# acdha/trivy

Hardware: AMD Instinct MI355X
Metric: secret-scan GB/s (builtin rules) at 1/2/4/8 MI355X; % of HBM peak (higher is better)
Workload: dtype u8

## Files before the change

### include/trivy_secret.h

```cpp
#ifndef TRIVY_SECRET_H
#define TRIVY_SECRET_H

#include <stddef.h>
#include <stdint.h>

#ifdef __cplusplus
extern "C" {
#endif

#define TSG_OK 0
#define TSG_ERR_CONFIG -1
#define TSG_ERR_ARG -2
#define TSG_ERR_GPU -3
#define TSG_ERR_NOMEM -4
#define TSG_ERR_INTERNAL -5

typedef struct tsg_allow_rule_desc {
  const char* id;
  const char* description;
  const char* regex;
  const char* path;
} tsg_allow_rule_desc;

typedef struct tsg_rule_desc {
// ... 16 lines not shown
typedef struct tsg_result tsg_result;
typedef struct tsg_ctx tsg_ctx;

int tsg_ruleset_compile(const tsg_rule_desc* rules, uint32_t n_rules,
                        const tsg_allow_rule_desc* allow_rules, uint32_t n_allow_rules,
                        const char* const* exclude_regexes, uint32_t n_exclude_regexes,
                        tsg_ruleset** out, char* err, size_t err_len);
void tsg_ruleset_destroy(tsg_ruleset* rs);

int tsg_ruleset_allow_path(const tsg_ruleset* rs, const char* path, size_t path_len);

typedef struct tsg_ruleset_info {
  uint32_t n_rules;
  uint32_t n_keywords;
  uint32_t n_groups;
  uint32_t n_hostonly;
  uint32_t kw_states;
  uint32_t max_group_states;
  uint64_t table_bytes;
  uint32_t kw_classes;
  uint32_t k1x_literals;
} tsg_ruleset_info;
int tsg_ruleset_get_info(const tsg_ruleset* rs, tsg_ruleset_info* out);

int tsg_scan_cpu(const tsg_ruleset* rs, const char* path, size_t path_len,
                 const uint8_t* content, size_t len, tsg_result** out);

int tsg_scan_cpu_batch(const tsg_ruleset* rs, const uint8_t* data, const uint64_t* offsets,
                       uint32_t nfiles, const char* paths, const uint64_t* path_offsets,
                       int nthreads, tsg_result** out);

const uint8_t* tsg_result_data(const tsg_result* r, size_t* len);

int tsg_go_sort_perm(const uint8_t* keys, const uint64_t* key_offsets, const int64_t* secondary,
                     uint32_t n, uint32_t* perm);
void tsg_result_free(tsg_result* r);
int tsg_result_summary(const tsg_result* r, uint64_t* nfiles, uint64_t* files_with_findings,
                       uint64_t* findings);

typedef struct tsg_ctx_options {
  uint32_t chunk_bytes;
  uint32_t ext_cap;
  uint32_t cand_capacity;
  int32_t host_threads;
  uint32_t adapt_mib;
  uint32_t flags;
  uint32_t slot_mib;
  uint32_t max_slots;
} tsg_ctx_options;

#define TSG_CTX_EMULATE 1u

int tsg_ctx_create(int device, const tsg_ruleset* rs, const tsg_ctx_options* opt,
                   tsg_ctx** out);
void tsg_ctx_destroy(tsg_ctx* ctx);

typedef struct tsg_slot_view {
  uint32_t id;
  uint8_t* data;
  uint64_t data_cap;
  uint64_t* offsets;
  uint32_t files_cap;
  char* paths;
  uint64_t paths_cap;
  uint64_t* path_offsets;
} tsg_slot_view;
int tsg_slot_acquire(tsg_ctx* ctx, uint64_t data_bytes, uint32_t nfiles, uint64_t path_bytes,
                     tsg_slot_view* out);
int tsg_slot_submit(tsg_ctx* ctx, uint32_t slot_id, uint32_t nfiles, uint64_t* ticket);
int tsg_slot_release(tsg_ctx* ctx, uint32_t slot_id);

int tsg_batch_upload(tsg_ctx* ctx, const uint8_t* data, const uint64_t* offsets,
                     uint32_t nfiles, const char* paths, const uint64_t* path_offsets,
                     uint32_t* slot_id);
int tsg_batch_collect(tsg_ctx* ctx, uint64_t ticket, tsg_result** out);
int tsg_batch_pending(const tsg_ctx* ctx);
int tsg_scan_batch(tsg_ctx* ctx, const uint8_t* data, const uint64_t* offsets, uint32_t nfiles,
                   const char* paths, const uint64_t* path_offsets, tsg_result** out);
int tsg_batch_kernels(tsg_ctx* ctx, uint32_t slot_id, uint32_t nfiles, uint32_t* kw,
                      size_t kw_len, uint32_t* ev, size_t ev_len);
int tsg_batch_items(tsg_ctx* ctx, uint32_t slot_id, uint32_t* entries, size_t entries_cap,
                    uint32_t* dentries, size_t dentries_cap, uint32_t* items, size_t items_cap,
                    uint8_t* gskip, size_t gskip_len, uint64_t* n);
int tsg_batch_candidates(tsg_ctx* ctx, uint32_t slot_id, uint32_t* records, size_t records_cap,
                         uint8_t* flags, size_t flags_len, uint32_t* kw, size_t kw_len, uint64_t* n);

typedef struct tsg_adaptation_info {
  uint32_t adapted;
  uint32_t k1_filter;
  uint32_t hot_states;
  uint32_t ev_hot;
  uint64_t sample_bytes;
  uint32_t n_keywords;
  uint32_t n_groups;
  uint32_t n_literals;
  uint32_t reserved;
} tsg_adaptation_info;
int tsg_test_adaptation(tsg_ctx* ctx, tsg_adaptation_info* info, uint8_t* kw_unknown,
                        size_t kw_unknown_len, uint8_t* gate_open, size_t gate_open_len,
                        uint8_t* event_everywhere, size_t event_everywhere_len, uint32_t* hits,
                        size_t hits_len, uint8_t* quiet, size_t quiet_len);

typedef struct tsg_stats {
  double k1_ms;
  double k2_ms;
  double aux_ms;
  double resolve_ms;
  uint64_t bytes;
  uint64_t k2_bytes;
  uint64_t candidates;
  uint64_t files_resolved;
  uint32_t k2_launches;
  uint32_t overflow;
  double gate_ms;
  uint64_t k2_items;
  uint32_t k1_hot_states;
  double h2d_ms;
  uint32_t groups_skipped;
  uint64_t batches;
  uint64_t sum_bytes;
  double sum_k1_ms, sum_gate_ms, sum_k2_ms, sum_h2d_ms, sum_d2h_ms, sum_resolve_ms;
  double wait_ms;
  uint32_t k2_tail_bytes, k2_tail_max, k2_long_tails, k2_replays;
  double prep_ms, meta_ms, sum_prep_ms, sum_meta_ms;
  uint32_t k1x_records, k1x_inline;
  uint32_t k1f_listed, k1f_arrivals;
  uint32_t event_chunks;
  uint32_t k1_filter;
  double k1_clock_ms, chain_clock_ms, post_k1_clock_ms;
  double sum_k1_clock_ms, sum_chain_clock_ms, sum_post_k1_clock_ms;
  uint32_t k2_dense_entries;
  uint32_t k2_rich;
  uint32_t k1x_img_bytes;
} tsg_stats;
int tsg_ctx_get_stats(const tsg_ctx* ctx, tsg_stats* out);

int tsg_device_submit(tsg_ctx* ctx, const void* d_data, const uint64_t* offsets, uint32_t nfiles,
                      const char* paths, const uint64_t* path_offsets, uint64_t* ticket);
int tsg_scan_device(tsg_ctx* ctx, const void* d_data, const uint64_t* offsets, uint32_t nfiles,
                    const char* paths, const uint64_t* path_offsets, tsg_result** out);
typedef struct tsg_device_input_stats {
  double stage_ms;
  double fetch_ms;
  uint64_t fetched_files;
  uint64_t fetched_bytes;
  uint64_t batches, sum_bytes, sum_fetched_bytes;
  double sum_stage_ms, sum_fetch_ms;
  uint32_t whole_batch_copy;
} tsg_device_input_stats;
int tsg_ctx_get_device_input_stats(const tsg_ctx* ctx, tsg_device_input_stats* out);
int tsg_test_device_mirror(tsg_ctx* ctx, uint8_t* data, uint64_t data_cap, uint64_t* segs,
                           size_t segs_cap, uint64_t* n);

#define TSG_SPANS_BINARY_GATE 1u
int tsg_device_spans_submit(tsg_ctx* ctx, const void* d_base, uint64_t base_bytes,
                            const uint64_t* starts, const uint64_t* lengths, uint32_t nfiles,
                            const char* paths, const uint64_t* path_offsets, uint32_t flags,
                            uint8_t* kept, uint64_t* ticket);
int tsg_scan_device_spans(tsg_ctx* ctx, const void* d_base, uint64_t base_bytes,
                          const uint64_t* starts, const uint64_t* lengths, uint32_t nfiles,
                          const char* paths, const uint64_t* path_offsets, uint32_t flags,
                          uint8_t* kept, tsg_result** out);
typedef struct tsg_device_spans_stats {
  double gate_ms;
  double gather_ms;
  double wait_ms;
  uint64_t files_in, files_kept, files_dropped;
  uint64_t bytes_in, bytes_kept;
  uint64_t batches, sum_files_in, sum_files_kept, sum_files_dropped, sum_bytes_in, sum_bytes_kept;
  double sum_gate_ms, sum_gather_ms, sum_wait_ms;
} tsg_device_spans_stats;
int tsg_ctx_get_device_spans_stats(const tsg_ctx* ctx, tsg_device_spans_stats* out);

typedef struct tsg_queue tsg_queue;
int tsg_queue_create(tsg_ctx* ctx, uint32_t flush_us, tsg_queue** out);
int tsg_queue_scan(tsg_queue* q, const char* path, size_t path_len, const uint8_t* content,
                   size_t len, tsg_result** out);
int tsg_queue_flush(tsg_queue* q);
void tsg_queue_destroy(tsg_queue* q);

typedef struct tsg_multi tsg_multi;
int tsg_multi_create(const int* devices, uint32_t n, const tsg_ruleset* rs,
                     const tsg_ctx_options* opt, tsg_multi** out);
int tsg_multi_size(const tsg_multi* m);
int tsg_multi_ctx(tsg_multi* m, uint32_t i, tsg_ctx** out);
int tsg_multi_scan_batch(tsg_multi* m, const uint8_t* data, const uint64_t* offsets,
                         uint32_t nfiles, const char* paths, const uint64_t* path_offsets,
                         tsg_result** out);
int tsg_multi_get_stats(const tsg_multi* m, uint32_t i, tsg_stats* out);
void tsg_multi_destroy(tsg_multi* m);

const char* tsg_last_error(void);

int tsg_test_knob(const char* name, const char* value);

typedef struct tsg_regex tsg_regex;
int tsg_regex_compile(const char* src, tsg_regex** out, char* err, size_t err_len);
void tsg_regex_free(tsg_regex* re);
int tsg_regex_num_slots(const tsg_regex* re);
int tsg_regex_match(const tsg_regex* re, const uint8_t* text, size_t len);
int64_t tsg_regex_find_all(const tsg_regex* re, const uint8_t* text, size_t len, int submatch,
                           int64_t* out, size_t cap);
int64_t tsg_regex_find_all_engine(const tsg_regex* re, const uint8_t* text, size_t len,
                                  int submatch, int engine, int64_t* out, size_t cap);
int64_t tsg_regex_dfa_ends(const tsg_regex* re, const uint8_t* text, size_t len, uint32_t chunk,
                           int64_t* out, size_t cap);

int tsg_emulate_candidate_stats(const tsg_ruleset* rs, const uint8_t* data,
                                const uint64_t* offsets, uint32_t nfiles, uint32_t chunk,
                                uint64_t* cand_per_rule, uint64_t* gated_bytes_per_group);

int tsg_emulate_items(const tsg_ruleset* rs, const uint8_t* data, const uint64_t* offsets,
                      uint32_t nfiles, uint32_t chunk, uint32_t max_back, uint32_t* triples,
                      size_t triples_cap, uint64_t* counts, uint64_t* n_items);

int tsg_emulate_candidates(const tsg_ruleset* rs, const uint8_t* data, const uint64_t* offsets,
                           uint32_t nfiles, uint32_t chunk, uint32_t ext_cap, uint64_t items_cap,
                           uint32_t max_dense, uint32_t word_recs, uint32_t* records,
                           size_t records_cap, uint64_t* n_records);

int tsg_emulate_item_candidates(const tsg_ruleset* rs, const uint8_t* data, const uint64_t* offsets,
                                uint32_t nfiles, uint32_t chunk, uint32_t ext_cap, uint32_t* triples,
                                size_t triples_cap, uint64_t* n_triples);

int tsg_expand_candidates(const tsg_ruleset* rs, const uint8_t* data, const uint64_t* offsets,
                          uint32_t nfiles, const uint32_t* records, size_t n_records,
                          uint32_t* triples, size_t triples_cap, uint64_t* n_triples);

int tsg_layout_reference(const uint64_t* counts, uint32_t n_groups, uint64_t nchunks,
                         uint64_t items_cap, uint32_t max_dense, uint8_t* kind, uint64_t* totals);

int tsg_emulate_k1(const tsg_ruleset* rs, const uint8_t* data, const uint64_t* offsets,
                   uint32_t nfiles, uint32_t chunk, uint32_t* kw, size_t kw_len, uint32_t* ev,
                   size_t ev_len);

int tsg_emulate_k1f(const tsg_ruleset* rs, const uint8_t* data, const uint64_t* offsets,
                    uint32_t nfiles, uint32_t chunk, const uint32_t* quiet_ids, uint32_t nquiet,
                    uint32_t sample_kib, uint32_t* kw, size_t kw_len, uint32_t* ev, size_t ev_len,
                    uint64_t* stats);

int tsg_ruleset_rule_plan(const tsg_ruleset* rs, uint32_t rule, int32_t* group, int32_t* relax,
                          int64_t* max_len);

int tsg_ruleset_rule_program(const tsg_ruleset* rs, uint32_t rule, int32_t* first_atom,
                             int32_t* rule_atoms, int64_t* winback, int32_t* has_rev);

int tsg_ruleset_rule_anchor(const tsg_ruleset* rs, uint32_t rule, uint32_t* event, int64_t* evdist,
                            char* desc, size_t desc_len);

int tsg_ruleset_k1_literal(const tsg_ruleset* rs, uint32_t i, uint8_t* buf, uint32_t cap,
                           uint32_t* len, uint32_t* event);

int tsg_scan_batch_emulated(const tsg_ruleset* rs, const uint8_t* data, const uint64_t* offsets,
                            uint32_t nfiles, const char* paths, const uint64_t* path_offsets,
                            uint32_t chunk, tsg_result** out);

typedef struct tsg_layer tsg_layer;
typedef struct tsg_layer_view {
  const uint8_t* data;
  const uint64_t* offsets;
  uint32_t nfiles;
  const uint8_t* paths;
  const uint64_t* path_offsets;
  const char* opq;
  size_t opq_len;
  const char* wh;
  size_t wh_len;
  uint32_t walked;
} tsg_layer_view;
int tsg_layer_pack(const tsg_ruleset* rs, const uint8_t* tar, uint64_t tar_len,
                   const char* const* skip_files, uint32_t n_skip_files,
                   const char* const* skip_dirs, uint32_t n_skip_dirs, const char* config_path,
                   tsg_layer** out);
int tsg_layer_pack_shard(const tsg_ruleset* rs, const uint8_t* tar, uint64_t tar_len,
                         const char* const* skip_files, uint32_t n_skip_files,
                         const char* const* skip_dirs, uint32_t n_skip_dirs, const char* config_path,
                         uint32_t rank, uint32_t world, tsg_layer** out);
int tsg_layer_get(const tsg_layer* layer, tsg_layer_view* out);
typedef struct tsg_layer_range tsg_layer_range;
int tsg_layer_range_walk(const uint8_t* tar, uint64_t tar_len, uint32_t rank, uint32_t world,
                         tsg_layer_range** out, uint64_t info[4]);
int tsg_layer_range_sync(tsg_layer_range* range, uint64_t pos, uint64_t* end);
int tsg_layer_range_dirs(tsg_layer_range* range, const char* const* skip_dirs, uint32_t n_skip_dirs,
                         const char** out, uint64_t* out_len);
int tsg_layer_range_pack(const tsg_ruleset* rs, const tsg_layer_range* range,
                         const char* const* skip_files, uint32_t n_skip_files,
                         const char* const* skip_dirs, uint32_t n_skip_dirs,
                         const char* const* prior_dirs, uint32_t n_prior_dirs,
                         const char* config_path, tsg_layer** out);
void tsg_layer_range_free(tsg_layer_range* range);
int tsg_fs_pack(const tsg_ruleset* rs, const char* root, const char* const* skip_files,
                uint32_t n_skip_files, const char* const* skip_dirs, uint32_t n_skip_dirs,
                const char* config_path, tsg_layer** out);
int tsg_fs_pack_shard(const tsg_ruleset* rs, const char* root, const char* const* skip_files,
                      uint32_t n_skip_files, const char* const* skip_dirs, uint32_t n_skip_dirs,
                      const char* config_path, uint32_t rank, uint32_t world, tsg_layer** out);
int tsg_layer_pack_slot(tsg_ctx* ctx, const uint8_t* tar, uint64_t tar_len,
                        const char* const* skip_files, uint32_t n_skip_files,
                        const char* const* skip_dirs, uint32_t n_skip_dirs, const char* config_path,
                        uint32_t* slot_id, tsg_layer** out);
int tsg_layer_range_pack_slot(tsg_ctx* ctx, const tsg_layer_range* range,
                              const char* const* skip_files, uint32_t n_skip_files,
                              const char* const* skip_dirs, uint32_t n_skip_dirs,
                              const char* const* prior_dirs, uint32_t n_prior_dirs,
                              const char* config_path, uint32_t* slot_id, tsg_layer** out);
int tsg_fs_pack_slot(tsg_ctx* ctx, const char* root, const char* const* skip_files,
                     uint32_t n_skip_files, const char* const* skip_dirs, uint32_t n_skip_dirs,
                     const char* config_path, uint32_t* slot_id, tsg_layer** out);
int tsg_layer_scan(tsg_ctx* ctx, const uint8_t* tar, uint64_t tar_len,
                   const char* const* skip_files, uint32_t n_skip_files,
                   const char* const* skip_dirs, uint32_t n_skip_dirs, const char* config_path,
                   tsg_layer** layer, tsg_result** out);
int tsg_fs_scan(tsg_ctx* ctx, const char* root, const char* const* skip_files, uint32_t n_skip_files,
                const char* const* skip_dirs, uint32_t n_skip_dirs, const char* config_path,
                tsg_layer** layer, tsg_result** out);
void tsg_layer_free(tsg_layer* layer);

int tsg_device_layer_scan(tsg_ctx* ctx, const void* d_tar, uint64_t tar_len,
                          const char* const* skip_files, uint32_t n_skip_files,
                          const char* const* skip_dirs, uint32_t n_skip_dirs,
                          const char* config_path, tsg_layer** layer, tsg_result** out);
typedef struct tsg_device_layer_stats {
  double mark_ms;
  uint64_t tar_bytes;
  uint64_t blocks;
  uint64_t marked_blocks;
  uint64_t chain_entries;
  uint64_t header_bytes;
  uint64_t payloads;
  uint64_t payload_bytes;
  uint64_t payload_rounds;
// ... 18 lines not shown
```

### trivy_amd/_native.py

```python
import ctypes as C
import os

LIB_PATH = os.path.join(os.path.dirname(os.path.abspath(__file__)), "libtrivy_secret.so")
if os.environ.get("TSG_LIB_VARIANT"):
    LIB_PATH = os.path.join(os.path.dirname(os.path.abspath(__file__)),
                            "libtrivy_secret_%s.so" % os.environ["TSG_LIB_VARIANT"])

TSG_OK = 0
TSG_ERR_CONFIG = -1
TSG_ERR_ARG = -2
TSG_ERR_GPU = -3
TSG_ERR_NOMEM = -4
TSG_ERR_INTERNAL = -5


class AllowRuleDesc(C.Structure):
    _fields_ = [("id", C.c_char_p), ("description", C.c_char_p), ("regex", C.c_char_p),
                ("path", C.c_char_p)]


class RuleDesc(C.Structure):
    _fields_ = [("id", C.c_char_p), ("category", C.c_char_p), ("title", C.c_char_p),
                ("severity", C.c_char_p), ("regex", C.c_char_p),
                ("keywords", C.POINTER(C.c_char_p)), ("n_keywords", C.c_uint32),
# ... 153 lines not shown
    ("tsg_queue_destroy", None, [_P]),
    ("tsg_multi_create", C.c_int, [C.POINTER(C.c_int), C.c_uint32, _P, C.POINTER(CtxOptions),
                                   C.POINTER(_P)]),
    ("tsg_multi_size", C.c_int, [_P]),
    ("tsg_multi_ctx", C.c_int, [_P, C.c_uint32, C.POINTER(_P)]),
    ("tsg_multi_scan_batch", C.c_int, [_P, _P, _U64P, C.c_uint32, _P, _U64P, C.POINTER(_P)]),
    ("tsg_multi_get_stats", C.c_int, [_P, C.c_uint32, C.POINTER(Stats)]),
    ("tsg_multi_destroy", None, [_P]),
    ("tsg_last_error", C.c_char_p, []),
    ("tsg_test_knob", C.c_int, [C.c_char_p, C.c_char_p]),
    ("tsg_regex_compile", C.c_int, [C.c_char_p, C.POINTER(_P), C.c_char_p, C.c_size_t]),
    ("tsg_regex_free", None, [_P]),
    ("tsg_regex_num_slots", C.c_int, [_P]),
    ("tsg_regex_match", C.c_int, [_P, C.c_char_p, C.c_size_t]),
    ("tsg_regex_find_all", C.c_int64, [_P, C.c_char_p, C.c_size_t, C.c_int, _I64P, C.c_size_t]),
    ("tsg_regex_find_all_engine", C.c_int64, [_P, C.c_char_p, C.c_size_t, C.c_int, C.c_int, _I64P, C.c_size_t]),
    ("tsg_regex_dfa_ends", C.c_int64, [_P, C.c_char_p, C.c_size_t, C.c_uint32, _I64P,
                                       C.c_size_t]),
    ("tsg_scan_batch_emulated", C.c_int, [_P, _P, _U64P, C.c_uint32, _P, _U64P, C.c_uint32,
                                          C.POINTER(_P)]),
    ("tsg_emulate_candidate_stats", C.c_int, [_P, _P, _U64P, C.c_uint32, C.c_uint32, _U64P,
                                              _U64P]),
    ("tsg_emulate_items", C.c_int, [_P, _P, _U64P, C.c_uint32, C.c_uint32, C.c_uint32,
                                    C.POINTER(C.c_uint32), C.c_size_t, _U64P, _U64P]),
    ("tsg_emulate_candidates", C.c_int, [_P, _P, _U64P, C.c_uint32, C.c_uint32, C.c_uint32, C.c_uint64,
                                         C.c_uint32, C.c_uint32, C.POINTER(C.c_uint32), C.c_size_t, _U64P]),
    ("tsg_emulate_item_candidates", C.c_int, [_P, _P, _U64P, C.c_uint32, C.c_uint32, C.c_uint32,
                                              C.POINTER(C.c_uint32), C.c_size_t, _U64P]),
    ("tsg_expand_candidates", C.c_int, [_P, _P, _U64P, C.c_uint32, C.POINTER(C.c_uint32), C.c_size_t,
                                        C.POINTER(C.c_uint32), C.c_size_t, _U64P]),
    ("tsg_layout_reference", C.c_int, [_U64P, C.c_uint32, C.c_uint64, C.c_uint64, C.c_uint32,
                                       _U8P, _U64P]),
    ("tsg_ruleset_rule_plan", C.c_int, [_P, C.c_uint32, C.POINTER(C.c_int32),
                                        C.POINTER(C.c_int32), C.POINTER(C.c_int64)]),
    ("tsg_ruleset_rule_program", C.c_int, [_P, C.c_uint32, C.POINTER(C.c_int32), C.POINTER(C.c_int32),
                                           C.POINTER(C.c_int64), C.POINTER(C.c_int32)]),
    ("tsg_emulate_k1", C.c_int, [_P, _P, _U64P, C.c_uint32, C.c_uint32, C.POINTER(C.c_uint32),
                                 C.c_size_t, C.POINTER(C.c_uint32), C.c_size_t]),
    ("tsg_layer_pack", C.c_int, [_P, _P, C.c_uint64, C.POINTER(C.c_char_p), C.c_uint32,
                                 C.POINTER(C.c_char_p), C.c_uint32, C.c_char_p, C.POINTER(_P)]),
    ("tsg_layer_pack_shard", C.c_int, [_P, _P, C.c_uint64, C.POINTER(C.c_char_p), C.c_uint32,
                                       C.POINTER(C.c_char_p), C.c_uint32, C.c_char_p, C.c_uint32,
                                       C.c_uint32, C.POINTER(_P)]),
    ("tsg_layer_get", C.c_int, [_P, C.POINTER(LayerView)]),
    ("tsg_layer_range_walk", C.c_int, [_P, C.c_uint64, C.c_uint32, C.c_uint32, C.POINTER(_P),
                                       _U64P]),
    ("tsg_layer_range_sync", C.c_int, [_P, C.c_uint64, _U64P]),
    ("tsg_layer_range_dirs", C.c_int, [_P, C.POINTER(C.c_char_p), C.c_uint32,
                                       C.POINTER(C.c_void_p), _U64P]),
    ("tsg_layer_range_pack", C.c_int, [_P, _P, C.POINTER(C.c_char_p), C.c_uint32,
                                       C.POINTER(C.c_char_p), C.c_uint32, C.POINTER(C.c_char_p),
                                       C.c_uint32, C.c_char_p, C.POINTER(_P)]),
    ("tsg_layer_range_free", None, [_P]),
    ("tsg_fs_pack", C.c_int, [_P, C.c_char_p, C.POINTER(C.c_char_p), C.c_uint32,
                              C.POINTER(C.c_char_p), C.c_uint32, C.c_char_p, C.POINTER(_P)]),
    ("tsg_fs_pack_shard", C.c_int, [_P, C.c_char_p, C.POINTER(C.c_char_p), C.c_uint32,
                                    C.POINTER(C.c_char_p), C.c_uint32, C.c_char_p, C.c_uint32,
                                    C.c_uint32, C.POINTER(_P)]),
    ("tsg_layer_pack_slot", C.c_int, [_P, _P, C.c_uint64, C.POINTER(C.c_char_p), C.c_uint32,
                                      C.POINTER(C.c_char_p), C.c_uint32, C.c_char_p,
                                      C.POINTER(C.c_uint32), C.POINTER(_P)]),
    ("tsg_layer_range_pack_slot", C.c_int, [_P, _P, C.POINTER(C.c_char_p), C.c_uint32,
                                            C.POINTER(C.c_char_p), C.c_uint32,
                                            C.POINTER(C.c_char_p), C.c_uint32, C.c_char_p,
                                            C.POINTER(C.c_uint32), C.POINTER(_P)]),
    ("tsg_fs_pack_slot", C.c_int, [_P, C.c_char_p, C.POINTER(C.c_char_p), C.c_uint32,
                                   C.POINTER(C.c_char_p), C.c_uint32, C.c_char_p,
                                   C.POINTER(C.c_uint32), C.POINTER(_P)]),
    ("tsg_layer_scan", C.c_int, [_P, _P, C.c_uint64, C.POINTER(C.c_char_p), C.c_uint32,
                                 C.POINTER(C.c_char_p), C.c_uint32, C.c_char_p, C.POINTER(_P),
                                 C.POINTER(_P)]),
    ("tsg_fs_scan", C.c_int, [_P, C.c_char_p, C.POINTER(C.c_char_p), C.c_uint32,
                              C.POINTER(C.c_char_p), C.c_uint32, C.c_char_p, C.POINTER(_P),
                              C.POINTER(_P)]),
    ("tsg_layer_free", None, [_P]),
    ("tsg_go_sort_perm", C.c_int, [_P, _U64P, _I64P, C.c_uint32, C.POINTER(C.c_uint32)]),
    ("tsg_ruleset_rule_anchor", C.c_int, [_P, C.c_uint32, C.POINTER(C.c_uint32),
                                          C.POINTER(C.c_int64), C.c_char_p, C.c_size_t]),
    ("tsg_emulate_k1f", C.c_int, [_P, _P, _U64P, C.c_uint32, C.c_uint32, C.POINTER(C.c_uint32),
                                  C.c_uint32, C.c_uint32, C.POINTER(C.c_uint32), C.c_size_t,
                                  C.POINTER(C.c_uint32), C.c_size_t, C.POINTER(C.c_uint64)]),
    ("tsg_ruleset_k1_literal", C.c_int, [_P, C.c_uint32, C.c_char_p, C.c_uint32,
                                         C.POINTER(C.c_uint32), C.POINTER(C.c_uint32)]),
]

_lib = None


def lib():
    global _lib
    if _lib is None:
        if not os.path.exists(LIB_PATH):
            raise ImportError("libtrivy_secret.so is not built; run `python -m trivy_amd.build` "
                              "(expected at %s)" % LIB_PATH)
        L = C.CDLL(LIB_PATH)
        for name, res, args in SIGNATURES:
            fn = getattr(L, name)
            fn.restype = res
            fn.argtypes = args
        _lib = L
    return _lib


class NativeError(RuntimeError):
    def __init__(self, code, msg):
        super().__init__("%s (code %d)" % (msg, code))
        self.code = code


def knob(name, value=None):
    check(lib().tsg_test_knob(name.encode(), None if value is None else str(value).encode()))


def check(rc):
    if rc != TSG_OK:
        raise NativeError(rc, lib().tsg_last_error().decode("utf-8", "replace"))
    return rc
```

### trivy_amd/csrc/capi.cpp

```cpp
#include <chrono>
#include <cstdio>
#include <cstdlib>
#include <cstring>
#include <exception>
#include <thread>

#include "internal.hpp"
#include "k1f.hpp"

namespace tsg {

static thread_local std::string g_last_error;

void set_error(const std::string& msg) { g_last_error = msg; }
int fail(int code, const std::string& msg) {
  g_last_error = msg;
  return code;
}

static void copy_err(const std::string& m, char* err, size_t len) {
  if (!err || len == 0) return;
  size_t n = std::min(len - 1, m.size());
  std::memcpy(err, m.data(), n);
  err[n] = 0;
// ... 363 lines not shown
  try {
    std::vector<uint64_t> poff(nfiles + 1, 0);
    BatchView b{data, offsets, nfiles, "", poff.data()};
    std::vector<uint32_t> k, e;
    k1_reference(*rs->plan, b, chunk, &k, &e);
    if (kw) std::memcpy(kw, k.data(), sizeof(uint32_t) * std::min(kw_len, k.size()));
    if (ev) std::memcpy(ev, e.data(), sizeof(uint32_t) * std::min(ev_len, e.size()));
    return TSG_OK;
  } catch (const std::bad_alloc&) {
    return fail(TSG_ERR_NOMEM, "out of memory");
  } catch (const std::exception& ex) {
    return fail(TSG_ERR_INTERNAL, ex.what());
  }
}

int tsg_emulate_k1f(const tsg_ruleset* rs, const uint8_t* data, const uint64_t* offsets,
                    uint32_t nfiles, uint32_t chunk, const uint32_t* quiet_ids, uint32_t nquiet,
                    uint32_t sample_kib, uint32_t* kw, size_t kw_len, uint32_t* ev, size_t ev_len,
                    uint64_t* stats) {
  if (!rs || !offsets || chunk == 0 || (nquiet && !quiet_ids)) return fail(TSG_ERR_ARG, "bad argument");
  try {
    const Plan& p = *rs->plan;
    std::vector<uint8_t> quiet(p.n_lit, 0);
    for (uint32_t i = 0; i < nquiet; i++) {
      if (quiet_ids[i] >= (uint32_t)p.n_lit) return fail(TSG_ERR_ARG, "no such K1 literal");
      quiet[quiet_ids[i]] = 1;
    }
    K1FTables t;
    std::string why;
    const size_t smp = std::min<uint64_t>((uint64_t)sample_kib << 10, offsets[nfiles]);
    if (!k1f_build(p, quiet, &t, &why, smp ? data : nullptr, smp)) return fail(TSG_ERR_CONFIG, "K1F does not apply: " + why);
    std::vector<uint64_t> poff(nfiles + 1, 0);
    BatchView b{data, offsets, nfiles, "", poff.data()};
    std::vector<uint32_t> k, e;
    uint64_t st[2];
    k1f_emulate(p, t, b, chunk, &k, &e, st);
    if (kw) std::memcpy(kw, k.data(), sizeof(uint32_t) * std::min(kw_len, k.size()));
    if (ev) std::memcpy(ev, e.data(), sizeof(uint32_t) * std::min(ev_len, e.size()));
    if (stats) {
      stats[0] = st[0];
      stats[1] = st[1];
      stats[2] = t.nlit;
      stats[3] = 0;
    }
    return TSG_OK;
  } catch (const std::bad_alloc&) {
    return fail(TSG_ERR_NOMEM, "out of memory");
  } catch (const std::exception& ex) {
    return fail(TSG_ERR_INTERNAL, ex.what());
  }
}

int tsg_ruleset_rule_plan(const tsg_ruleset* rs, uint32_t rule, int32_t* group, int32_t* relax,
                          int64_t* max_len) {
  if (!rs || rule >= rs->rs.rules.size()) return fail(TSG_ERR_ARG, "bad argument");
  const Plan& p = *rs->plan;
  if (group) *group = p.rule_hostonly[rule] ? -1 : p.rule_group[rule];
  if (relax) *relax = p.rule_relax[rule];
  if (max_len) *max_len = p.rule_maxlen[rule];
  return TSG_OK;
}

int tsg_ruleset_rule_program(const tsg_ruleset* rs, uint32_t rule, int32_t* first_atom, int32_t* rule_atoms,
                             int64_t* winback, int32_t* has_rev) {
  if (!rs || rule >= rs->rs.rules.size()) return fail(TSG_ERR_ARG, "bad argument");
  const Plan& p = *rs->plan;
  if (first_atom) *first_atom = p.rule_first_atom[rule];
  if (rule_atoms) *rule_atoms = p.rule_atoms[rule];
  if (winback) *winback = p.rule_winback[rule];
  if (has_rev) *has_rev = p.rule_rev[rule] ? 1 : 0;
  return TSG_OK;
}

int tsg_ruleset_rule_anchor(const tsg_ruleset* rs, uint32_t rule, uint32_t* event, int64_t* evdist,
                            char* desc, size_t desc_len) {
  if (!rs || rule >= rs->rs.rules.size()) return fail(TSG_ERR_ARG, "bad argument");
  const Plan& p = *rs->plan;
  if (event) *event = p.rule_event[rule];
  if (evdist) *evdist = p.rule_evdist[rule];
  copy_err(p.rule_anchor[rule], desc, desc_len);
  return TSG_OK;
}

int tsg_ruleset_k1_literal(const tsg_ruleset* rs, uint32_t i, uint8_t* buf, uint32_t cap,
                           uint32_t* len, uint32_t* event) {
  if (!rs || (!buf && cap)) return fail(TSG_ERR_ARG, "bad argument");
  const Plan& p = *rs->plan;
  if (i >= p.k1_lits.size()) return fail(TSG_ERR_ARG, "no such K1 literal");
  const std::string& s = p.k1_lits[i];
  if (buf) std::memcpy(buf, s.data(), std::min<size_t>(cap, s.size()));
  if (len) *len = (uint32_t)s.size();
  if (event) *event = p.lit_event[i];
  return TSG_OK;
}

int tsg_go_sort_perm(const uint8_t* keys, const uint64_t* key_offsets, const int64_t* secondary,
                     uint32_t n, uint32_t* perm) {
  if ((n && (!keys || !key_offsets || !perm))) return fail(TSG_ERR_ARG, "bad argument");
  try {
    go_sort_perm(keys, key_offsets, secondary, n, perm);
    return TSG_OK;
  } catch (const std::bad_alloc&) {
    return fail(TSG_ERR_NOMEM, "out of memory");
  }
}

const uint8_t* tsg_result_data(const tsg_result* r, size_t* len) {
  if (!r) {
    if (len) *len = 0;
    return nullptr;
  }
  if (len) *len = r->buf.size();
  return (const uint8_t*)r->buf.data();
}

void tsg_result_free(tsg_result* r) { delete r; }

int tsg_result_summary(const tsg_result* r, uint64_t* nfiles, uint64_t* files_with_findings,
                       uint64_t* findings) {
  if (!r) return fail(TSG_ERR_ARG, "bad argument");
  try {
    std::vector<size_t> rec;
    result_record_spans(r->buf, &rec);
    uint64_t ff = 0, nf = 0;
    for (size_t i = 0; i + 1 < rec.size(); i++) {
      uint32_t k;
      std::memcpy(&k, r->buf.data() + rec[i] + 1, 4);
      ff += k > 0;
      nf += k;
    }
    if (nfiles) *nfiles = rec.size() - 1;
    if (files_with_findings) *files_with_findings = ff;
    if (findings) *findings = nf;
    return TSG_OK;
  } catch (const std::exception& ex) {
    return fail(TSG_ERR_ARG, ex.what());
  }
}

struct tsg_regex {
  std::shared_ptr<Regexp> re;
};

int tsg_regex_compile(const char* src, tsg_regex** out, char* err, size_t err_len) {
  if (!src || !out) return fail(TSG_ERR_ARG, "bad argument");
  std::string e;
  auto re = Regexp::Compile(src, &e);
  if (!re) {
    copy_err(e, err, err_len);
    return fail(TSG_ERR_CONFIG, e);
  }
  *out = new tsg_regex{re};
  return TSG_OK;
}

void tsg_regex_free(tsg_regex* re) { delete re; }

int tsg_regex_num_slots(const tsg_regex* re) { return re ? re->re->NumSlots() : TSG_ERR_ARG; }

int tsg_regex_match(const tsg_regex* re, const uint8_t* text, size_t len) {
  if (!re) return fail(TSG_ERR_ARG, "bad argument");
  return re->re->Match(text, len) ? 1 : 0;
}

int64_t tsg_regex_find_all(const tsg_regex* re, const uint8_t* text, size_t len, int submatch,
                           int64_t* out, size_t cap) {
// ... 51 lines not shown
```

### trivy_amd/csrc/device.hpp

```cpp
#pragma once
#include <hip/hip_runtime_api.h>

#include <cstdint>
#include <memory>
#include <vector>

#include "plan.hpp"

namespace tsg {

struct DeviceRules;

enum BatchEvent : int { kEvH2D = 0, kEvMeta, kEvPrep, kEvWait, kEvK1, kEvGates, kEvK2, kEvOut, kEvDone };

struct HostOut {
  uint8_t* blk = nullptr;
  uint8_t* blk_dev = nullptr;
  uint32_t* kw = nullptr;
  uint8_t* ovf = nullptr;
  uint8_t* gskip = nullptr;
  Candidate* cand = nullptr;
  Candidate* cand_dev = nullptr;
  uint32_t* counts = nullptr;
  uint32_t files_cap = 0, cand_cap = 0, groups = 0, kw_words = 0;
// ... 17 lines not shown
  kCntK1FSample = 24,
  kCntClk = 32,
  kCounts = 48,
};
enum LayoutStat : uint32_t { kLayItems = 1, kLayEntries = 2, kLaySkipped = 3 };
enum ClkStamp : uint32_t { kClkK1FStart = 0, kClkK1FEnd = 1, kClkGatesStart = 2, kClkK2End = 3, kClkStamps = 4 };
static_assert(kCntDenseEntries < kCntLayout && kCntLayout + kLayItems == kCntItems &&
                  kCntLayout + kLayEntries == kCntEntries && kCntLayout + kLaySkipped == kCntSkipped,
              "the layout's stats are slots 5..7");
static_assert(kCntSkipped < kCntK2Diag && kCntK2Diag + 4 <= kCntK2Claim && kCntK2Claim + 2 <= kCntK1X &&
                  kCntK1X + 2 <= kCntK1F && kCntK1F + 2 <= kCntK1FSample && kCntK1FSample + 2 <= kCntClk,
              "counter ranges overlap");
static_assert(kCntClk % 2 == 0 && kCntClk + 2 * kClkStamps <= kCounts, "clock stamps: 8-byte aligned, inside the block");

struct K2Diag {
  unsigned long long tail_bytes, tail_max, long_tails, replays;
};

struct GatherSeg {
  uint64_t src, dst, len;
};

enum class ScanSource {
  kHostSlot,
  kPackedHbm,
  kHbmSpans,
};

struct ScanInput {
  ScanSource kind;
  const uint64_t* off;
  uint32_t nfiles;
  uint64_t total;
  const uint8_t* data = nullptr;
  uint8_t* room = nullptr;
  uint64_t room_bytes = 0;
  const uint8_t* dev_src = nullptr;
  uint64_t src_bytes = 0;
  const GatherSeg* gather = nullptr;
  const GatherSeg* gather_dev = nullptr;
  uint32_t ngather = 0;
};

inline uint64_t slot_room_bytes(uint32_t files_cap) { return (128u << 10) + 8ull * ((uint64_t)files_cap + 1) + 64; }

struct ScanTimes {
  float h2d = 0, meta = 0, wait = 0, prep = 0, k1 = 0, gates = 0, k2 = 0, out = 0;
  float k1_clk = 0, chain_clk = 0, post_k1_clk = 0;
};

struct LaneState;

int device_rules_create(int device, const Plan& plan, uint32_t chunk, uint32_t ext_cap,
                        uint32_t adapt_mib, DeviceRules** out);
void device_rules_destroy(DeviceRules* d);
std::shared_ptr<const std::vector<uint8_t>> device_rules_kw_unknown(const DeviceRules* d);
uint32_t device_rules_hot_states(const DeviceRules* d);
struct AdaptationView {
  bool adapted = false, k1_filter = false;
  uint32_t hot_states = 0, ev_hot = 0;
  uint64_t sample_bytes = 0;
  std::vector<uint8_t> kw_unknown;
  std::vector<uint8_t> gate_open;
  std::vector<uint8_t> event_everywhere;
  std::vector<uint32_t> hits;
  std::vector<uint8_t> quiet;
};
int device_rules_adaptation(const DeviceRules* d, AdaptationView* out);
bool device_rules_k1_filter(const DeviceRules* d);
bool device_rules_k2_rich(const DeviceRules* d);
uint32_t device_rules_k1x_img_bytes(const DeviceRules* d);

int lane_create(DeviceRules* d, LaneState** out);
void lane_destroy(LaneState* l);
hipStream_t lane_stream(LaneState* l);

int host_out_alloc(const DeviceRules* d, uint32_t files_cap, uint32_t cand_cap, HostOut* out);
void host_out_free(HostOut* o);

int enqueue_scan(DeviceRules* d, LaneState* l, const ScanInput& in, HostOut* out);
int batch_times(const HostOut* out, ScanTimes* t);
int lane_kw(LaneState* l, uint32_t* kw, size_t n);
int lane_events(LaneState* l, uint32_t* ev, size_t n);
struct LaneItems {
  std::vector<uint32_t> entries, dentries, items;
  std::vector<uint8_t> gskip;
  uint64_t extent = 0;
};
int lane_items(LaneState* l, LaneItems* out);
int lane_k2_trace(LaneState* l, std::vector<unsigned long long>* out);
int lane_k1f_trace(LaneState* l, std::vector<unsigned long long>* out);

constexpr uint64_t kGatherSegBytes = 64u << 10;
struct DeviceFetch;
int fetch_create(DeviceRules* d, DeviceFetch** out);
void fetch_destroy(DeviceFetch* f);
int fetch_segments(DeviceFetch* f, const uint8_t* d_src, uint64_t total, uint8_t* host_dst,
                   const GatherSeg* segs, size_t nsegs, float* ms);
int gate_spans(DeviceFetch* f, const uint8_t* d_base, uint64_t base_bytes, const uint64_t* starts_dev,
               const uint64_t* lengths_dev, uint8_t* flags_dev, uint32_t nfiles, float* ms);
int fetch_gather(DeviceFetch* f, const uint8_t* d_base, uint64_t base_bytes, uint8_t* host_dst, uint64_t dst_bytes,
                 const GatherSeg* segs, size_t nsegs, float* ms);
int mark_tar(DeviceFetch* f, const uint8_t* d_tar, uint64_t tar_len, uint64_t* marks, float* ms);
int fetch_whole(DeviceFetch* f, const uint8_t* d_src, uint64_t total, uint8_t* host_dst, float* ms);

}
```

### trivy_amd/csrc/internal.hpp

```cpp
#pragma once
#include <algorithm>
#include <atomic>
#include <cstdint>
#include <memory>
#include <mutex>
#include <string>
#include <utility>

#include "../../include/trivy_secret.h"
#include "plan.hpp"
#include "scanner.hpp"

struct tsg_ruleset {
  tsg::Ruleset rs;
  std::unique_ptr<tsg::Plan> plan;
};

struct tsg_result {
  std::string buf;
};

namespace tsg {
void set_error(const std::string& msg);
int fail(int code, const std::string& msg);
const tsg_ruleset* ctx_ruleset(const tsg_ctx* c);
uint64_t ctx_slot_bytes(const tsg_ctx* c);
bool is_binary_head(const uint8_t* p, uint64_t n);


void tar_block_marks(const uint8_t* block, bool* header, bool* zero);
int ctx_tar_marks(tsg_ctx* c, const void* d_tar, uint64_t tar_len, uint64_t* marks, double* ms);
struct PinBuf {
  uint8_t* p = nullptr;
  uint64_t cap = 0;
};
void ctx_pin_give(tsg_ctx* c, PinBuf* b);
int ctx_fetch_ranges(tsg_ctx* c, const void* d_base, uint64_t base_bytes,
                     const std::pair<uint64_t, uint64_t>* ranges, size_t n, PinBuf* dst);
int ctx_collect_device(tsg_ctx* c, uint64_t ticket, tsg_result** out, uint64_t* fetched_bytes);
void ctx_device_layer_done(tsg_ctx* c, const tsg_device_layer_stats& last);

struct Knobs {
  std::atomic<int64_t> tar_range_kib{0}, piece_mib{0}, pike_only{0}, no_k1x{0}, emu_wordrec{0},
      x_step{0}, k1_automaton{0}, group_states{0}, group_table_kib{0}, k1f_grid{0},
      k1f_list{0}, k2_items_cap{0}, k2_max_dense{0}, k2_no_word_recs{0}, device_poison{0}, grid_cap{0};
  std::mutex m;
  std::string emu_kw_unknown;
};
Knobs& knobs();
std::string knob_kw_unknown();

inline int capped_grid(uint64_t grid, int64_t cap) {
  return (int)(cap > 0 ? std::min<uint64_t>(grid, (uint64_t)cap) : grid);
}

inline uint64_t k2_items_cap(uint64_t nchunks) {
  const int64_t k = knobs().k2_items_cap.load();
  return k > 0 ? (uint64_t)k : std::max<uint64_t>(2 * nchunks, 1u << 16);
}
inline uint32_t k2_max_dense() {
  const int64_t k = knobs().k2_max_dense.load();
  return k > 0 ? (uint32_t)k : 16u;
}
}
```

### trivy_amd/csrc/kernels.hip

```cpp
#include <hip/hip_runtime.h>

#include <algorithm>
#include <map>
#include <cstdlib>
#include <cstring>
#include <memory>
#include <vector>

#include "device.hpp"
#include "internal.hpp"
#include "k1f.hpp"

namespace tsg {

#define HIP_TRY(x)                                                                    \
  do {                                                                                \
    hipError_t e_ = (x);                                                              \
    if (e_ != hipSuccess)                                                             \
      return fail(TSG_ERR_GPU, std::string(#x) + ": " + hipGetErrorString(e_));       \
  } while (0)

constexpr int kStreams = 4;
constexpr int kK1Chains = 2;
constexpr int kK1Unroll = 8;
// ... 1301 lines not shown
  if (threadIdx.x == 0) {
    const uint32_t n = *s_n, kept = min(n, slice);
    A.count[blockIdx.x] = kept;
    atomicAdd(&A.stats[0], kept);
    if (n > kept) atomicAdd(&A.stats[1], n - kept);
  }
}

static const void* k1x_fn(uint32_t step) {
  if (step == 4) return (const void*)k1x_kernel<4>;
  if (step == 2) return (const void*)k1x_kernel<2>;
  return (const void*)k1x_kernel<1>;
}

constexpr int kXVerifyBlock = 1024;
template <bool LDS>
__global__ void __launch_bounds__(kXVerifyBlock) k1x_verify_kernel(DevK1X x, K1XArgs A, uint32_t nblocks) {
  extern __shared__ __attribute__((aligned(16))) uint8_t x_img[];
  const uint32_t b = blockIdx.x;
  const uint32_t n = A.count[b];
  if (n == 0) return;
  DevK1X y = x;
  if constexpr (LDS) {
    stage16(x_img, x.img, x.img_bytes / 16 * 16);
    __syncthreads();
    auto rebase = [&](auto* p) { return (decltype(p))(x_img + ((const uint8_t*)p - x.img)); };
    y.slots = rebase(x.slots);
    y.lits = rebase(x.lits);
    y.off = rebase(x.off);
    y.len = rebase(x.len);
    y.kwid = rebase(x.kwid);
    y.ev = rebase(x.ev);
    y.bytes = rebase(x.bytes);
  }
  const uint32_t slice = A.cap / nblocks;
  for (uint32_t j = threadIdx.x; j < n; j += blockDim.x) {
    const uint2 r = A.list[(size_t)b * slice + j];
    const uint64_t p0 = (uint64_t)r.x * 16;
    for (uint32_t t = r.y; t; t &= t - 1) {
      const uint64_t p = p0 + __builtin_ctz(t);
      const uint32_t w = x_low_byte(A.data[p]) | x_low_byte(A.data[p + 1]) << 8 | x_low_byte(A.data[p + 2]) << 16 |
                         x_low_byte(A.data[p + 3]) << 24;
      k1x_verify_at(y, A, p, w);
    }
  }
}

__device__ __forceinline__ bool group_gated(const uint32_t* __restrict__ kwf, const uint32_t* __restrict__ gm,
                                            uint32_t W, uint32_t always) {
  if (always) return true;
  for (uint32_t w = 0; w < W; w++)
    if (kwf[w] & gm[w]) return true;
  return false;
}

__device__ __forceinline__ void ggate_file(uint32_t f, const uint32_t* __restrict__ kw, uint32_t F, uint32_t W,
                                           const unsigned long long* __restrict__ kwg,
                                           const unsigned long long* __restrict__ galw, uint32_t GW,
                                           unsigned long long* __restrict__ ggate) {
  if (f >= F) return;
  const uint32_t* kwf = kw + (size_t)f * W;
  for (uint32_t w0 = 0; w0 < GW; w0 += 8) {
    const uint32_t n = min(8u, GW - w0);
    unsigned long long acc[8];
#pragma unroll
    for (uint32_t j = 0; j < 8; j++) acc[j] = j < n ? galw[w0 + j] : 0ull;
    for (uint32_t i = 0; i < W; i++)
      for (uint32_t bits = kwf[i]; bits; bits &= bits - 1) {
        const unsigned long long* row = kwg + (size_t)(i * 32 + __builtin_ctz(bits)) * GW + w0;
#pragma unroll
        for (uint32_t j = 0; j < 8; j++)
          if (j < n) acc[j] |= row[j];
      }
#pragma unroll
    for (uint32_t j = 0; j < 8; j++)
      if (j < n) ggate[(size_t)f * GW + w0 + j] = acc[j];
  }
}

struct ItemArgs {
  const uint64_t* off;
  const uint32_t* cf;
  const uint32_t* ev;
  const uint32_t* evlist;
  const uint32_t* nev;
  uint32_t evcap;
  const unsigned long long* ggate;
  const unsigned long long* gofbit;
  const uint32_t* gevents;
  const uint32_t* gback;
  uint64_t nchunks;
  uint32_t F, G, GW, chunk, maxback;
  uint32_t* count;
  uint32_t* bcount;
  uint32_t* cursor;
  uint2* items;
  const uint32_t* kw;
  uint32_t W;
  const unsigned long long* kwg;
  const unsigned long long* galw;
  unsigned long long* clk;
  uint32_t kwg_lds;
};

constexpr uint32_t kEvPer = 32;
__device__ __forceinline__ void ev_compact_block(const uint32_t* __restrict__ ev, uint64_t nchunks,
                                                 uint32_t* __restrict__ list, uint32_t* __restrict__ count,
                                                 uint32_t bid, uint32_t nblocks) {
  __shared__ uint32_t s_wave[kBlock / 64];
  __shared__ uint32_t s_base;
  const uint32_t lane = threadIdx.x & 63, wave = threadIdx.x >> 6;
  constexpr uint64_t kPer = (uint64_t)kEvPer * kBlock;
  for (uint64_t c0 = (uint64_t)bid * kPer; c0 < nchunks; c0 += (uint64_t)nblocks * kPer) {
    const uint64_t c = c0 + (uint64_t)threadIdx.x * kEvPer;
    uint32_t has = 0;
    if (c + kEvPer <= nchunks) {
      uint4 v[kEvPer / 4];
#pragma unroll
      for (uint32_t i = 0; i < kEvPer / 4; i++) v[i] = *(const uint4*)(ev + c + 4 * i);
#pragma unroll
      for (uint32_t i = 0; i < kEvPer / 4; i++)
        has |= ((v[i].x & ~kEvAlways) != 0 ? 1u : 0u) << (4 * i) | ((v[i].y & ~kEvAlways) != 0 ? 2u : 0u) << (4 * i) |
               ((v[i].z & ~kEvAlways) != 0 ? 4u : 0u) << (4 * i) | ((v[i].w & ~kEvAlways) != 0 ? 8u : 0u) << (4 * i);
    } else {
      for (uint32_t i = 0; i < kEvPer && c + i < nchunks; i++) has |= ((ev[c + i] & ~kEvAlways) != 0 ? 1u : 0u) << i;
    }
    const uint32_t n = __popc(has);
    uint32_t inc = n;
#pragma unroll
    for (int o = 1; o < 64; o <<= 1) {
      const uint32_t t = __shfl_up(inc, o);
      if (lane >= (uint32_t)o) inc += t;
    }
    if (lane == 63) s_wave[wave] = inc;
    __syncthreads();
    if (threadIdx.x == 0) {
      uint32_t tot = 0;
      for (uint32_t w = 0; w < kBlock / 64; w++) tot += s_wave[w];
      s_base = tot ? atomicAdd(count, tot) : 0;
    }
    __syncthreads();
    uint32_t at = s_base + inc - n;
    for (uint32_t w = 0; w < wave; w++) at += s_wave[w];
    for (uint32_t t = has; t; t &= t - 1) list[at++] = (uint32_t)(c + __builtin_ctz(t));
    __syncthreads();
  }
}

struct GateArgs {
  const uint32_t* ev;
  uint64_t nchunks;
  uint32_t* evlist;
  uint32_t* nev;
  uint32_t ev_blocks;
  const uint32_t* kw;
  uint32_t F, W, GW;
  const unsigned long long* kwg;
  const unsigned long long* galw;
  unsigned long long* ggate;
  unsigned long long* clk;
  uint32_t kwg_lds;
};
constexpr uint32_t kKwgLdsMax = 48 * 1024;
__global__ void __launch_bounds__(kBlock) gates_kernel(GateArgs A) {
  extern __shared__ __attribute__((aligned(16))) uint8_t smem[];
  if (threadIdx.x == 0 && blockIdx.x < kStampBlocks)
    atomicMax(&A.clk[kClkGatesStart], ~(unsigned long long)wall_clock64());
  if (blockIdx.x < A.ev_blocks) {
    ev_compact_block(A.ev, A.nchunks, A.evlist, A.nev, blockIdx.x, A.ev_blocks);
  } else {
    const unsigned long long* kwg = A.kwg;
    if (A.kwg_lds) {
      stage16(smem, A.kwg, A.kwg_lds);
      __syncthreads();
      kwg = (const unsigned long long*)smem;
    }
    ggate_file((blockIdx.x - A.ev_blocks) * blockDim.x + threadIdx.x, A.kw, A.F, A.W, kwg, A.galw, A.GW, A.ggate);
  }
}

static inline size_t item_lds_host(uint32_t G, uint32_t GW) { return 256 * (size_t)GW + 8 * (size_t)G; }
constexpr uint32_t kItemKwgLdsMax = 16 * 1024;
struct ItemLds {
  const unsigned long long* gofbit;
  const uint32_t* gback;
  const uint32_t* gevents;
  const unsigned long long* kwg;
};
__device__ __forceinline__ uint32_t item_lds_bytes(const ItemArgs& A) { return 256 * A.GW + 8 * A.G + A.kwg_lds; }
__device__ __forceinline__ ItemLds item_lds_load(const ItemArgs& A, uint8_t* smem) {
  unsigned long long* gofbit = (unsigned long long*)smem;
  uint32_t* gback = (uint32_t*)(gofbit + 32 * A.GW);
  uint32_t* gevents = gback + A.G;
  for (uint32_t i = threadIdx.x; i < 32 * A.GW; i += blockDim.x) gofbit[i] = A.gofbit[i];
  for (uint32_t i = threadIdx.x; i < A.G; i += blockDim.x) {
    gback[i] = A.gback[i];
    gevents[i] = A.gevents[i];
  }
  const unsigned long long* kwg = A.kwg;
  if (A.kwg_lds) {
    unsigned long long* k = (unsigned long long*)(gevents + A.G);
    for (uint32_t i = threadIdx.x; i < A.kwg_lds / 8; i += blockDim.x) k[i] = A.kwg[i];
    kwg = k;
  }
  return ItemLds{gofbit, gback, gevents, kwg};
}

__device__ __forceinline__ unsigned long long file_gate(const ItemArgs& A, const ItemLds& T, uint32_t f, uint32_t w) {
  if (A.ggate) return A.ggate[(size_t)f * A.GW + w];
  const uint32_t* kwf = A.kw + (size_t)f * A.W;
  unsigned long long acc = A.galw[w];
  for (uint32_t i = 0; i < A.W; i++)
    for (uint32_t bits = kwf[i]; bits; bits &= bits - 1) acc |= T.kwg[(size_t)(i * 32 + __builtin_ctz(bits)) * A.GW + w];
  return acc;
}

template <class V>
__device__ __forceinline__ void gen_items(const ItemArgs& A, const ItemLds& T, uint64_t t, V visit) {
  const uint32_t ev_t = t < A.evcap ? A.evlist[t] : 0u;
  const uint32_t nev = min(*A.nev, A.evcap);
  const uint32_t C = A.chunk;
  if (t < nev) {
    const uint64_t e = ev_t;
    const uint32_t evb = A.ev[e] & ~kEvAlways;
    const uint64_t ce = (e + 1) * C;
    uint32_t pw[kMaxBack];
    if (e >= (uint64_t)kMaxBack) {
      const uint64_t b0 = (e - kMaxBack) & ~3ull;
      const uint32_t sh = (uint32_t)(e - kMaxBack - b0);
      uint32_t x[20];
#pragma unroll
      for (int j = 0; j < 5; j++) {
        const uint4 q = *(const uint4*)(A.ev + b0 + 4 * j);
        x[4 * j] = q.x;
        x[4 * j + 1] = q.y;
        x[4 * j + 2] = q.z;
        x[4 * j + 3] = q.w;
      }
#pragma unroll
      for (int i = 0; i < kMaxBack; i++) {
        const int k = kMaxBack - 1 - i;
        pw[i] = sh == 0 ? x[k] : sh == 1 ? x[k + 1] : sh == 2 ? x[k + 2] : x[k + 3];
      }
    } else {
#pragma unroll
      for (int i = 0; i < kMaxBack; i++) pw[i] = e > (uint64_t)i ? A.ev[e - 1 - i] : 0u;
    }
    for (uint32_t f = file_of(A.cf, A.off, A.F, e * C); f < A.F && A.off[f] < ce; f++) {
      const uint64_t fs = A.off[f], fe = A.off[f + 1];
      if (fe == fs) continue;
      const uint64_t fc0 = fs / C;
      for (uint32_t w = 0; w < A.GW; w++) {
        unsigned long long cand = 0;
        for (uint32_t bits = evb; bits; bits &= bits - 1) cand |= T.gofbit[__builtin_ctz(bits) * A.GW + w];
        cand &= file_gate(A, T, f, w) & ~T.gofbit[31 * A.GW + w];
        while (cand) {
          const uint32_t g = w * 64 + __builtin_ctzll(cand);
          cand &= cand - 1;
          const uint32_t back = T.gback[g], gev = T.gevents[g];
          const uint64_t lo0 = e > fc0 + back ? e - back : fc0;
          const uint32_t lim = (uint32_t)(e - lo0);
          uint32_t m = 0;
#pragma unroll
          for (int i = 0; i < kMaxBack; i++) m |= ((pw[i] & gev) != 0 && (uint32_t)i < lim ? 1u : 0u) << i;
          visit(f, g, m ? e - __builtin_ctz(m) : lo0, e);
        }
      }
    }
  } else if (t < (uint64_t)nev + A.F) {
    const uint32_t f = (uint32_t)(t - nev);
    const uint64_t fs = A.off[f], fe = A.off[f + 1];
    if (fe == fs) return;
    for (uint32_t w = 0; w < A.GW; w++) {
      unsigned long long cand = file_gate(A, T, f, w) & T.gofbit[31 * A.GW + w];
      while (cand) {
        const uint32_t g = w * 64 + __builtin_ctzll(cand);
        cand &= cand - 1;
        visit(f, g, fs / C, (fe - 1) / C);
      }
    }
  }
}

__global__ void __launch_bounds__(kBlock) items_count_kernel(ItemArgs A) {
  extern __shared__ __attribute__((aligned(16))) uint8_t smem[];
  if (!A.ggate && threadIdx.x == 0 && blockIdx.x < kStampBlocks)
    atomicMax(&A.clk[kClkGatesStart], ~(unsigned long long)wall_clock64());
  const ItemLds T = item_lds_load(A, smem);
  uint32_t* s_count = (uint32_t*)(smem + item_lds_bytes(A));
  for (uint32_t g = threadIdx.x; g < A.G; g += blockDim.x) s_count[g] = 0;
  __syncthreads();
  const uint64_t nt = (uint64_t)min(*A.nev, A.evcap) + A.F, stride = (uint64_t)gridDim.x * blockDim.x;
  for (uint64_t t = (uint64_t)blockIdx.x * blockDim.x + threadIdx.x; t < nt; t += stride)
    gen_items(A, T, t, [&](uint32_t, uint32_t g, uint64_t lo, uint64_t hi) { atomicAdd(&s_count[g], (uint32_t)(hi - lo + 1)); });
  __syncthreads();
  for (uint32_t g = threadIdx.x; g < A.G; g += blockDim.x)
    A.bcount[(size_t)blockIdx.x * A.G + g] = s_count[g] ? atomicAdd(&A.count[g], s_count[g]) : 0u;
}

struct LayoutArgs {
  const uint32_t* gcount;
  uint32_t G;
  uint64_t nchunks, items_cap;
  uint32_t max_dense;
  uint4* entries;
  uint32_t* nentries;
  uint4* dentries;
  uint32_t* ndentries;
  uint8_t* gskip;
  uint32_t* stats;
};

constexpr int kK2Block = 256;
constexpr uint32_t kEntryItems = 2 * kK2Block;
constexpr uint32_t kEntryChunks = kStreams * kBlock;
static_assert(kEntryItems == kK2EntryItems && kEntryChunks == kK2EntryChunks, "layout_reference restates these");

template <int N>
__device__ void block_exclusive_scan_n(const unsigned long long (&v)[N], unsigned long long (&out)[N],
                                       unsigned long long (&tot)[N], unsigned long long* s_wave) {
  const uint32_t lane = threadIdx.x & 63, wave = threadIdx.x >> 6, nw = blockDim.x >> 6;
  unsigned long long x[N];
#pragma unroll
  for (int k = 0; k < N; k++) x[k] = v[k];
  for (int o = 1; o < 64; o <<= 1) {
#pragma unroll
    for (int k = 0; k < N; k++) {
      const unsigned long long y = __shfl_up(x[k], o);
      if (lane >= (uint32_t)o) x[k] += y;
    }
  }
  if (lane == 63)
#pragma unroll
    for (int k = 0; k < N; k++) s_wave[k * nw + wave] = x[k];
  __syncthreads();
#pragma unroll
  for (int k = 0; k < N; k++) {
    unsigned long long before = 0, total = 0;
    for (uint32_t w = 0; w < nw; w++) {
      const unsigned long long t = s_wave[k * nw + w];
      before += w < wave ? t : 0;
      total += t;
    }
    out[k] = before + x[k] - v[k];
    tot[k] = total;
  }
  __syncthreads();
// ... 947 lines not shown
  v.ns = (uint32_t)d.nstates;
  v.nmasks = (uint32_t)d.masks.size();
  v.mw = mw;
  v.kw_words = W;
  v.warm = (uint32_t)p.warm;
  v.kU = (uint32_t)p.run_k[0];
  v.kD = v.packed ? (uint32_t)p.run_k[1] : (uint32_t)p.run_k[1] << 8;
  std::vector<uint16_t> kwlen((size_t)W * 32, 0);
  v.kw_maxlen = 1;
  for (int k = 0; k < p.n_kw; k++) {
    kwlen[k] = p.kw_len[k];
    v.kw_maxlen = std::max<uint32_t>(v.kw_maxlen, p.kw_len[k]);
  }
  if ((rc = upload_vec(kwlen, &v.kw_len, allocs))) return rc;
  host->masks = masks;
  const int lc = k1_lds_class(host->tab.size() * 2);
  v.lds_class = (uint32_t)(lc >> 1);
  v.rep = (uint32_t)(lc & 1);
  if (!v.packed && v.lds_class > 2) return fail(TSG_ERR_INTERNAL, "keyword automaton exceeds LDS");
  return TSG_OK;
}

template <class T>
struct DevBuf {
  T* p = nullptr;
  size_t cap = 0;
  DevBuf() = default;
  DevBuf(const DevBuf&) = delete;
  DevBuf& operator=(const DevBuf&) = delete;
  ~DevBuf() { (void)hipFree(p); }
  operator T*() const { return p; }
  int ensure(size_t n, bool exact = false) {
    if (cap >= n && p) return TSG_OK;
    if (p) HIP_TRY(hipFree(p));
    p = nullptr;
    cap = 0;
    const size_t alloc = exact ? n : std::max<size_t>(n + n / 8, 16);
    HIP_TRY(hipMalloc((void**)&p, exact ? alloc * sizeof(T) : (alloc * sizeof(T) + 15) & ~(size_t)15));
    cap = alloc;
    return TSG_OK;
  }
};

struct DeviceRules {
  uint32_t all_kw_rows = 0;
  int device = 0;
  const Plan* plan = nullptr;
  uint32_t chunk = 256, ext_cap = 1u << 16, adapt_mib = 0;
  int grid = 0;
  int cus = 0;
  int k2_grid = 0, k2_dense_grid = 0;
  bool k2_rich = false;
  hipEvent_t kernels_done = nullptr;
  bool kernels_done_valid = false;
  std::vector<void*> tables;
  DevK1 k1{};
  K1Host k1h;
  DevK1X k1x{};
  bool has_k1x = false;
  bool use_k1f = false;
  uint32_t k1f_maxlen = 4;
  DevK1F k1f{};
  K1FTables k1ft;
  DevBuf<uint32_t> d_fhits;
  DevBuf<uint32_t> d_hits;
  bool adapted = false;
  uint32_t hot_states = 0;
  uint32_t ev_hot = 0;
  uint64_t sample_bytes = 0;
  std::vector<uint32_t> lit_hits;
  std::vector<uint8_t> lit_quiet;
  std::shared_ptr<const std::vector<uint8_t>> kw_unknown;
  std::vector<uint32_t> h_galways, h_gevents;
  std::vector<unsigned long long> h_gofbit;
  std::vector<DevDFA> groups;
  DevDFA* d_groups = nullptr;
  uint32_t* d_gmask = nullptr;
  uint32_t* d_galways = nullptr;
  unsigned long long* d_kwg = nullptr;
  unsigned long long* d_galw = nullptr;
  uint32_t* d_gevents = nullptr;
  uint32_t* d_gback = nullptr;
  unsigned long long* d_gofbit = nullptr;
  std::vector<uint32_t> gback;
  uint32_t GW = 1, maxback = 0, max_lds = 0;
  ~DeviceRules() {
    (void)hipSetDevice(device);
    if (kernels_done) (void)hipEventDestroy(kernels_done);
    for (auto* p : tables) (void)hipFree(p);
  }
};

struct LaneState {
  DeviceRules* d = nullptr;
  hipStream_t st = nullptr;
  DevBuf<uint8_t> data_alloc;
  DevBuf<uint8_t> meta;
  const uint64_t* off = nullptr;
  DevBuf<uint32_t> cf;
  DevBuf<uint32_t> ev_bits;
  DevBuf<uint2> xlist;
  DevBuf<uint32_t> xcount;
  DevBuf<uint32_t> evlist;
  DevBuf<uint32_t> zclaim;
  DevBuf<unsigned long long> wtrace;
  size_t wtrace_n = 0;
  DevBuf<uint32_t> kw;
  DevBuf<unsigned long long> ggate;
  DevBuf<uint8_t> ovf;
  DevBuf<uint8_t> hascand;
  DevBuf<uint2> items;
  DevBuf<uint4> entries;
  DevBuf<uint4> dentries;
  DevBuf<DevCand> cand;
  DevBuf<uint32_t> counts;
  DevBuf<uint32_t> gcount;
  DevBuf<uint32_t> bcount;
  DevBuf<uint32_t> cursor;
  DevBuf<uint8_t> gskip;
  DevBuf<unsigned long long> etrace;
  uint64_t nchunks = 0;
  uint8_t* data() const { return data_alloc.p + kPad; }
  ~LaneState() {
    if (!d) return;
    (void)hipSetDevice(d->device);
    if (st) (void)hipStreamSynchronize(st);
    if (st) (void)hipStreamDestroy(st);
  }
};

template <bool PACKED, int LDSK, bool REP, int TPB>
static const void* k1_fn_w(uint32_t kw_words) {
  if (kw_words <= 1) return (const void*)k1_kernel<1, PACKED, LDSK, REP, TPB>;
  if (kw_words <= 2) return (const void*)k1_kernel<2, PACKED, LDSK, REP, TPB>;
  if (kw_words <= 4) return (const void*)k1_kernel<4, PACKED, LDSK, REP, TPB>;
  return (const void*)k1_kernel<8, PACKED, LDSK, REP, TPB>;
}

static const void* k1_fn(const DevK1& k, int* threads, int* per_cu) {
  if (k.packed) {
    *threads = 1024;
    *per_cu = 1;
    return k1_fn_w<true, kK1PLdsK, true, 1024>(k.kw_words);
  }
  const uint32_t lc = std::min<uint32_t>(k.lds_class, 2);
  *threads = k1_threads(kK1Lds[lc]);
  *per_cu = kK1BlocksPerCU[lc];
  switch (lc) {
    case 0: return k1_fn_w<false, kK1Lds[0], true, k1_threads(kK1Lds[0])>(k.kw_words);
    case 1: return k1_fn_w<false, kK1Lds[1], true, k1_threads(kK1Lds[1])>(k.kw_words);
    default:
      return k.rep ? k1_fn_w<false, kK1Lds[2], true, k1_threads(kK1Lds[2])>(k.kw_words)
                   : k1_fn_w<false, kK1Lds[2], false, k1_threads(kK1Lds[2])>(k.kw_words);
  }
}

static int launch_k1(DeviceRules* r, const K1Args& A, int64_t grid_cap, hipStream_t st) {
  int threads = 0, per_cu = 0;
  const void* fn = k1_fn(r->k1, &threads, &per_cu);
  const uint64_t cap = (uint64_t)r->cus * per_cu;
  const int grid = capped_grid(std::min<uint64_t>((A.nitems + threads - 1) / threads, cap), grid_cap);
  DevK1 d = r->k1;
  K1Args a = A;
  void* args[] = {&d, &a};
  HIP_TRY(hipLaunchKernel(fn, dim3(grid), dim3(threads), args, 0, st));
  HIP_TRY(hipGetLastError());
  return TSG_OK;
}

template <class Exact>
static std::vector<uint32_t> hottest_over_budget(const std::vector<uint32_t>& hits, uint64_t sample_bytes, Exact exact) {
  uint64_t tot = 0;
  std::vector<uint32_t> order, drop;
  for (uint32_t i = 0; i < hits.size(); i++)
    if (hits[i]) {
      tot += hits[i];
      order.push_back(i);
    }
  std::sort(order.begin(), order.end(), [&](uint32_t a, uint32_t b) { return hits[a] > hits[b]; });
  const uint64_t budget = sample_bytes / 4096;
  for (uint32_t i : order) {
    if (tot <= budget) break;
    if (exact(i)) continue;
// ... 176 lines not shown
}

int device_rules_create(int device, const Plan& p, uint32_t chunk, uint32_t ext_cap, uint32_t adapt_mib,
                        DeviceRules** out) {
  int ndev = 0;
  HIP_TRY(hipGetDeviceCount(&ndev));
  if (device < 0 || device >= ndev) return fail(TSG_ERR_GPU, "no such HIP device");
  HIP_TRY(hipSetDevice(device));
  auto r = std::make_unique<DeviceRules>();
  r->device = device;
  r->plan = &p;
  r->chunk = chunk;
  r->ext_cap = ext_cap;
  r->adapt_mib = adapt_mib;
  if (p.warm > kPad) return fail(TSG_ERR_CONFIG, "a keyword is longer than the K1 warm-up window");
  int rc;
  if ((rc = make_device_k1(p, &r->k1, &r->tables, &r->k1h))) return rc;
  if ((rc = make_device_k1x(p, &r->k1x, &r->tables))) return rc;
  r->has_k1x = !p.x_lits.empty();
  if (!knobs().k1_automaton.load() && k1f_build(p, {}, &r->k1ft, nullptr)) {
    void* ent = nullptr;
    void* img = nullptr;
    HIP_TRY(hipMalloc(&ent, 256 * 16));
    r->tables.push_back(ent);
    HIP_TRY(hipMalloc(&img, kFImgMax));
    r->tables.push_back(img);
    r->k1f.ent = (const uint4*)ent;
    r->k1f.img = (const uint8_t*)img;
    r->k1f.kw_words = (uint32_t)p.kw_words;
    if ((rc = upload_k1f(r.get()))) return rc;
    if ((rc = r->d_fhits.ensure(std::max(1, p.n_lit), true))) return rc;
    r->use_k1f = true;
  }
  for (uint8_t h : p.rule_hostonly) r->all_kw_rows |= h;
  if (r->has_k1x)
    HIP_TRY(hipFuncSetAttribute(k1x_fn(r->k1x.step), hipFuncAttributeMaxDynamicSharedMemorySize,
                                kXDwords * 4 + 16));
  if (r->has_k1x && r->k1x.img_bytes <= kXImgLds)
    HIP_TRY(hipFuncSetAttribute((const void*)k1x_verify_kernel<true>, hipFuncAttributeMaxDynamicSharedMemorySize,
                                r->k1x.img_bytes));
  if ((rc = r->d_hits.ensure(r->k1.ns, true))) return rc;
  const uint32_t G = (uint32_t)p.groups.size();
  if (G > 0x7FFF) return fail(TSG_ERR_INTERNAL, "more K2 groups than transition records can name");
  r->GW = std::max<uint32_t>(1, (G + 63) / 64);
  std::vector<uint32_t> gmask, galways, gevents;
  std::vector<unsigned long long> gofbit(32 * r->GW, 0);
  for (uint32_t g = 0; g < G; g++) {
    const auto& gp = p.groups[g];
    DevDFA dd{};
    if ((rc = make_device_dfa(*gp.dfa, gp.rules, &dd, &r->tables))) return rc;
    r->max_lds = std::max(r->max_lds, dd.lds_bytes);
    r->groups.push_back(dd);
    gmask.insert(gmask.end(), gp.kwmask.begin(), gp.kwmask.end());
    galways.push_back(gp.always ? 1 : 0);
    gevents.push_back(gp.events);
    uint32_t back = group_back(gp, chunk);
    if (back > (uint32_t)kMaxBack) back = kMaxBack + 1;
    r->gback.push_back(back);
    if (back <= (uint32_t)kMaxBack) r->maxback = std::max(r->maxback, back);
    for (int b = 0; b < 32; b++)
      if (((gp.events >> b) & 1) || back > (uint32_t)kMaxBack) gofbit[b * r->GW + g / 64] |= 1ull << (g % 64);
  }
  r->max_lds = std::max<uint32_t>(r->max_lds, 16);
  {
    const size_t emit_lds = item_lds_host(G, r->GW) + kItemKwgLdsMax + 13 * (size_t)G + 16;
    if (emit_lds > 160 * 1024) return fail(TSG_ERR_INTERNAL, "too many rule groups for the item passes");
    if (emit_lds > 64 * 1024) {
      HIP_TRY(hipFuncSetAttribute((const void*)items_emit_kernel, hipFuncAttributeMaxDynamicSharedMemorySize, (int)emit_lds));
      HIP_TRY(hipFuncSetAttribute((const void*)items_count_kernel, hipFuncAttributeMaxDynamicSharedMemorySize, (int)emit_lds));
    }
  }
  if (r->max_lds > 64 * 1024) {
    HIP_TRY(hipFuncSetAttribute((const void*)k2_kernel, hipFuncAttributeMaxDynamicSharedMemorySize, (int)r->max_lds));
    HIP_TRY(hipFuncSetAttribute((const void*)k2_kernel_rich, hipFuncAttributeMaxDynamicSharedMemorySize, (int)r->max_lds));
    HIP_TRY(hipFuncSetAttribute((const void*)k2_dense_kernel, hipFuncAttributeMaxDynamicSharedMemorySize,
                                (int)r->max_lds));
  }
  if ((rc = upload_vec(gmask, &r->d_gmask, &r->tables))) return rc;
  if ((rc = upload_vec(galways, &r->d_galways, &r->tables))) return rc;
  if ((rc = upload_vec(gevents, &r->d_gevents, &r->tables))) return rc;
  if ((rc = upload_vec(r->gback, &r->d_gback, &r->tables))) return rc;
  if ((rc = upload_vec(gofbit, &r->d_gofbit, &r->tables))) return rc;
  {
    const uint32_t nkw = (uint32_t)p.kw_words * 32;
    std::vector<unsigned long long> kwg((size_t)nkw * r->GW, 0), galw(r->GW, 0);
    for (uint32_t g = 0; g < G; g++) {
      for (uint32_t k = 0; k < nkw; k++)
        if ((gmask[(size_t)g * p.kw_words + k / 32] >> (k % 32)) & 1) kwg[(size_t)k * r->GW + g / 64] |= 1ull << (g % 64);
      if (galways[g]) galw[g / 64] |= 1ull << (g % 64);
    }
    if ((rc = upload_vec(kwg, &r->d_kwg, &r->tables))) return rc;
    if ((rc = upload_vec(galw, &r->d_galw, &r->tables))) return rc;
  }
  r->h_galways = galways;
  r->h_gevents = gevents;
  r->h_gofbit = gofbit;
  if ((rc = upload_vec(r->groups, &r->d_groups, &r->tables))) return rc;
  hipDeviceProp_t prop;
  HIP_TRY(hipGetDeviceProperties(&prop, device));
  r->cus = prop.multiProcessorCount;
  r->grid = prop.multiProcessorCount * 8;
  HIP_TRY(hipEventCreateWithFlags(&r->kernels_done, hipEventDisableTiming | hipEventReleaseToDevice));
  int occ = 0;
  HIP_TRY(hipOccupancyMaxActiveBlocksPerMultiprocessor(&occ, (const void*)k2_kernel, kK2Block, r->max_lds));
  r->k2_grid = r->cus * std::max(occ, 1);
  {
    int occ_rich = 0;
    HIP_TRY(hipOccupancyMaxActiveBlocksPerMultiprocessor(&occ_rich, (const void*)k2_kernel_rich, kK2Block, r->max_lds));
    r->k2_rich = occ_rich >= 1 && occ_rich >= occ;
  }
  HIP_TRY(hipOccupancyMaxActiveBlocksPerMultiprocessor(&occ, (const void*)k2_dense_kernel, kBlock, r->max_lds));
  r->k2_dense_grid = r->cus * std::max(occ, 1);
  *out = r.release();
  return TSG_OK;
}

void device_rules_destroy(DeviceRules* d) { delete d; }

std::shared_ptr<const std::vector<uint8_t>> device_rules_kw_unknown(const DeviceRules* d) { return d->kw_unknown; }
uint32_t device_rules_hot_states(const DeviceRules* d) { return d->hot_states; }
int device_rules_adaptation(const DeviceRules* d, AdaptationView* out) {
  const Plan& p = *d->plan;
  out->adapted = d->adapted;
  out->k1_filter = d->use_k1f;
  out->hot_states = d->hot_states;
  out->ev_hot = d->ev_hot;
  out->sample_bytes = d->sample_bytes;
  if (d->kw_unknown) out->kw_unknown = *d->kw_unknown;
  else out->kw_unknown.assign(p.n_kw, 0);
  const size_t G = d->groups.size();
  std::vector<uint32_t> ga(G), ge(G);
  if (G) {
    HIP_TRY(hipSetDevice(d->device));
    HIP_TRY(hipMemcpy(ga.data(), d->d_galways, sizeof(uint32_t) * G, hipMemcpyDeviceToHost));
    HIP_TRY(hipMemcpy(ge.data(), d->d_gevents, sizeof(uint32_t) * G, hipMemcpyDeviceToHost));
  }
  out->gate_open.assign(G, 0);
  out->event_everywhere.assign(G, 0);
  for (size_t g = 0; g < G; g++) {
    out->gate_open[g] = ga[g] ? 1 : 0;
    out->event_everywhere[g] = (ge[g] & kEvAlways) ? 1 : 0;
  }
  out->hits = d->lit_hits;
  out->quiet = d->lit_quiet;
  return TSG_OK;
}
bool device_rules_k1_filter(const DeviceRules* d) { return d->use_k1f; }
bool device_rules_k2_rich(const DeviceRules* d) { return d->k2_rich; }
uint32_t device_rules_k1x_img_bytes(const DeviceRules* d) { return d->has_k1x ? d->k1x.img_bytes : 0u; }

int lane_create(DeviceRules* d, LaneState** out) {
  HIP_TRY(hipSetDevice(d->device));
  auto l = std::make_unique<LaneState>();
  l->d = d;
  HIP_TRY(hipStreamCreateWithFlags(&l->st, hipStreamNonBlocking));
  const uint32_t G = std::max<uint32_t>(1, (uint32_t)d->groups.size());
  int rc;
  if ((rc = l->counts.ensure(kCounts, true))) return rc;
  if ((rc = l->gcount.ensure(G, true))) return rc;
  if ((rc = l->bcount.ensure(G * (size_t)d->grid, true))) return rc;
  if ((rc = l->cursor.ensure(G, true))) return rc;
  if ((rc = l->gskip.ensure(G, true))) return rc;
  *out = l.release();
  return TSG_OK;
}

void lane_destroy(LaneState* l) { delete l; }
hipStream_t lane_stream(LaneState* l) { return l->st; }

static size_t al256(size_t x) { return (x + 255) & ~(size_t)255; }

void host_out_free(HostOut* o) {
  void* ps[] = {o->blk, o->cand};
  for (void* p : ps)
    if (p) (void)hipHostFree(p);
  for (auto& e : o->ev)
    if (e) (void)hipEventDestroy(e);
  *o = HostOut{};
}

int host_out_alloc(const DeviceRules* d, uint32_t files_cap, uint32_t cand_cap, HostOut* o) {
  HIP_TRY(hipSetDevice(d->device));
  HostOut h;
  h.files_cap = std::max<uint32_t>(files_cap, 1);
  h.cand_cap = std::max<uint32_t>(cand_cap, 1);
  h.groups = std::max<uint32_t>(1, (uint32_t)d->groups.size());
  h.kw_words = (uint32_t)d->plan->kw_words;
  const size_t o_gskip = 256, o_ovf = o_gskip + al256(h.groups), o_kw = o_ovf + al256(h.files_cap),
               bytes = o_kw + al256(sizeof(uint32_t) * (size_t)h.files_cap * h.kw_words);
  auto fail_free = [&](hipError_t e, const char* what) {
    host_out_free(&h);
    return fail(TSG_ERR_GPU, std::string(what) + ": " + hipGetErrorString(e));
  };
  hipError_t e;
  if ((e = hipHostMalloc((void**)&h.blk, bytes, hipHostMallocMapped)) != hipSuccess) return fail_free(e, "hipHostMalloc");
  if ((e = hipHostGetDevicePointer((void**)&h.blk_dev, h.blk, 0)) != hipSuccess) return fail_free(e, "hipHostGetDevicePointer");
  h.counts = (uint32_t*)h.blk;
  {
    int khz = 0;
    if (hipDeviceGetAttribute(&khz, hipDeviceAttributeWallClockRate, d->device) == hipSuccess && khz > 0)
      h.wall_khz = (uint32_t)khz;
  }
  h.gskip = h.blk + o_gskip;
  h.ovf = h.blk + o_ovf;
  h.kw = (uint32_t*)(h.blk + o_kw);
  if ((e = hipHostMalloc((void**)&h.cand, sizeof(Candidate) * (size_t)h.cand_cap, hipHostMallocMapped)) != hipSuccess)
    return fail_free(e, "hipHostMalloc");
  if ((e = hipHostGetDevicePointer((void**)&h.cand_dev, h.cand, 0)) != hipSuccess) return fail_free(e, "hipHostGetDevicePointer");
  for (int k = 0; k <= kEvDone; k++)
    if ((e = k < kEvDone ? hipEventCreateWithFlags(&h.ev[k], hipEventDisableSystemFence) : hipEventCreate(&h.ev[k])) !=
        hipSuccess)
      return fail_free(e, "hipEventCreate");
  *o = h;
  return TSG_OK;
}

struct BatchShape {
  uint32_t W, C, F, G;
  uint64_t total, nchunks, nchunks_pad, ncf;
  size_t tail, o_off, meta_bytes;
  bool one_copy;
  bool k1f;
  uint64_t k1_items;
  uint32_t k1f_tiles;
  uint64_t items_cap;
  uint32_t max_dense;
  uint64_t entries_cap, dentries_cap, zclaim_words;
  bool work;
  uint32_t kwg_bytes;
  int64_t grid_cap;
};

static int batch_shape(const DeviceRules* r, const ScanInput& in, const HostOut* out, BatchShape* s) {
  const uint32_t C = s->C = r->chunk;
  const uint64_t total = s->total = in.total;
  s->W = (uint32_t)r->plan->kw_words;
  s->F = in.nfiles;
  s->G = (uint32_t)r->groups.size();
  if (s->F > out->files_cap) return fail(TSG_ERR_ARG, "batch has more files than its output buffers");
  if (total / C >= (1ull << 32) - 2) return fail(TSG_ERR_ARG, "batch too large for u32 chunk ids");
  const bool spans = in.kind == ScanSource::kHbmSpans;
  for (uint32_t k = 0; spans && k < in.ngather; k++) {
    const GatherSeg& g = in.gather[k];
    if (g.src > in.src_bytes || g.len > in.src_bytes - g.src || g.dst > total || g.len > total - g.dst)
      return fail(TSG_ERR_INTERNAL, "gather segment outside its buffers");
  }
  if (spans && in.ngather && (!in.dev_src || !in.gather_dev)) return fail(TSG_ERR_INTERNAL, "gather without a source");
  s->nchunks = (total + C - 1) / C;
  s->k1f = r->use_k1f && total + (1u << 16) < (1ull << 32);
  s->tail = std::max<size_t>((size_t)kK1Chains * kK1Seg * C + kPad, 8192);
  s->meta_bytes = sizeof(uint64_t) * ((size_t)s->F + 1);
  s->o_off = ((size_t)total + s->tail + 15) & ~(size_t)15;
  s->one_copy = in.kind == ScanSource::kHostSlot && in.room == in.data && in.room_bytes >= s->o_off + s->meta_bytes;
  const uint64_t k1_item_chunks = (uint64_t)kK1Chains * kK1Seg;
  s->k1_items = (s->nchunks + k1_item_chunks - 1) / k1_item_chunks;
  s->nchunks_pad = s->k1_items * k1_item_chunks + 1;
  s->ncf = (total >> kCfShift) + 2;
  s->k1f_tiles = (uint32_t)((total + kFTile - 1) / kFTile);
  s->zclaim_words = s->nchunks_pad / 32 + 2;
  s->items_cap = k2_items_cap(s->nchunks);
  s->max_dense = k2_max_dense();
  s->entries_cap = s->items_cap / kEntryItems + s->G + 1;
  s->dentries_cap = (uint64_t)s->max_dense * ((s->nchunks + kEntryChunks - 1) / kEntryChunks + 1);
  s->work = s->F && s->G && s->nchunks;
  s->kwg_bytes = (uint32_t)(32ull * s->W * r->GW * 8);
  s->grid_cap = knobs().grid_cap.load();
  return TSG_OK;
}

int enqueue_scan(DeviceRules* r, LaneState* l, const ScanInput& in, HostOut* out) {
  const Plan& p = *r->plan;
  HIP_TRY(hipSetDevice(r->device));
  hipStream_t st = l->st;
  BatchShape s;
  int rc;
  if ((rc = batch_shape(r, in, out, &s))) return rc;
  const uint64_t total = s.total;
  l->nchunks = s.nchunks;
  if ((rc = l->data_alloc.ensure(kPad + s.o_off + s.meta_bytes))) return rc;
  uint8_t* data = l->data();
  if (s.one_copy) {
    l->off = (const uint64_t*)(data + s.o_off);
  } else {
    if ((rc = l->meta.ensure(s.meta_bytes))) return rc;
    l->off = (const uint64_t*)l->meta.p;
  }
  if ((rc = l->cf.ensure((size_t)s.ncf))) return rc;
  if ((rc = l->ev_bits.ensure((size_t)s.nchunks_pad + 4))) return rc;
  if (r->has_k1x && (rc = l->xlist.ensure((size_t)(total / 256 + 65536)))) return rc;
  if (r->has_k1x && (rc = l->xcount.ensure((size_t)std::max(r->cus, 1)))) return rc;
  if ((rc = l->evlist.ensure((size_t)s.nchunks_pad))) return rc;
  if (s.k1f && (rc = l->zclaim.ensure((size_t)s.zclaim_words))) return rc;
  if ((rc = l->kw.ensure((size_t)s.F * s.W + 1))) return rc;
  if ((rc = l->ggate.ensure((size_t)s.F * r->GW + 1))) return rc;
  if ((rc = l->ovf.ensure((size_t)s.F + 1))) return rc;
  if ((rc = l->hascand.ensure((size_t)s.F + 1))) return rc;
  if ((rc = l->items.ensure((size_t)s.items_cap))) return rc;
  if ((rc = l->entries.ensure((size_t)s.entries_cap))) return rc;
  if ((rc = l->dentries.ensure((size_t)s.dentries_cap))) return rc;
  if ((rc = l->cand.ensure(out->cand_cap, true))) return rc;
  HIP_TRY(hipEventRecord(out->ev[kEvH2D], st));
  if (s.one_copy) {
    std::memset(in.room + total, 0, s.o_off - total);
    std::memcpy(in.room + s.o_off, in.off, s.meta_bytes);
    HIP_TRY(hipMemcpyAsync(data, in.room, s.o_off + s.meta_bytes, hipMemcpyHostToDevice, st));
    HIP_TRY(hipEventRecord(out->ev[kEvMeta], st));
  } else {
    switch (in.kind) {
      case ScanSource::kHbmSpans:
        if (in.ngather) {
          GatherArgs GA{in.dev_src, in.src_bytes, data, total, in.gather_dev, in.ngather};
          const int ggrid = capped_grid(std::min<uint64_t>(in.ngather, (uint64_t)std::max(r->grid, 1)), s.grid_cap);
          gather_kernel<true><<<ggrid, 256, 0, st>>>(GA);
          HIP_TRY(hipGetLastError());
        }
        break;
      case ScanSource::kPackedHbm:
        if (total) {
          const uint64_t words = (total + 15) / 16;
          const int sgrid =
              capped_grid(std::max<uint64_t>(1, std::min<uint64_t>((words + 255) / 256, (uint64_t)r->grid)), s.grid_cap);
          stage_kernel<<<sgrid, 256, 0, st>>>(data, in.dev_src, total);
          HIP_TRY(hipGetLastError());
        }
        break;
      case ScanSource::kHostSlot:
        if (total) HIP_TRY(hipMemcpyAsync(data, in.data, total, hipMemcpyHostToDevice, st));
        break;
    }
    HIP_TRY(hipEventRecord(out->ev[kEvMeta], st));
    HIP_TRY(hipMemcpyAsync(l->meta, in.off, s.meta_bytes, hipMemcpyHostToDevice, st));
  }
  HIP_TRY(hipEventRecord(out->ev[kEvPrep], st));
  {
    PrepArgs PA{};
    PA.off = l->off;
    PA.nfiles = s.F;
    PA.ncf = s.F ? s.ncf : 0;
    PA.cf = l->cf;
    bool too_many = false;
    auto zero = [&](void* ptr, uint64_t n) {
      if (!n) return;
      if (PA.nz == (uint32_t)kPrepZeros) {
        too_many = true;
        return;
      }
      PA.zp[PA.nz] = (uint8_t*)ptr;
      PA.zn[PA.nz++] = n;
    };
    zero(l->data_alloc, kPad);
    if (!s.one_copy) zero(data + total, s.tail);
    zero(l->kw, sizeof(uint32_t) * (uint64_t)s.F * s.W);
    zero(l->ovf, s.F);
    zero(l->hascand, s.F);
    zero(l->counts, sizeof(uint32_t) * kCounts);
    if (s.k1f) zero(l->ev_bits, sizeof(uint32_t) * s.nchunks_pad);
    if (s.k1f) zero(l->zclaim, sizeof(uint32_t) * s.zclaim_words);
    zero(l->gcount, sizeof(uint32_t) * s.G);
    zero(l->cursor, sizeof(uint32_t) * s.G);
    zero(l->gskip, s.G);
    if (too_many) return fail(TSG_ERR_INTERNAL, "more zero fills than the prep kernel takes");
    const uint64_t work = std::max<uint64_t>(
        {PA.ncf, (uint64_t)s.F * s.W / 4, s.one_copy ? 1 : s.tail / 16, s.k1f ? s.nchunks_pad / 4 : 1, 1});
    const int pgrid = capped_grid(std::min<uint64_t>((work + 255) / 256, (uint64_t)r->grid), s.grid_cap);
    prep_kernel<<<pgrid, 256, 0, st>>>(PA);
    HIP_TRY(hipGetLastError());
  }
  HIP_TRY(hipEventRecord(out->ev[kEvWait], st));
  if (r->kernels_done_valid) HIP_TRY(hipStreamWaitEvent(st, r->kernels_done, 0));
  HIP_TRY(hipEventRecord(out->ev[kEvK1], st));

  const uint64_t adapt_bytes = r->adapt_mib == 0xFFFFFFFFu ? ~0ull : (uint64_t)(r->adapt_mib ? r->adapt_mib : 16) << 20;
  const bool k1f_list = s.k1f && total && !r->has_k1x && knobs().k1f_list.load() && k1f_lists(r, s.k1f_tiles, s.C, s.grid_cap);
  if (s.k1f) {
    K1FArgs A{data, l->off, l->cf, (uint32_t)total, s.C, s.F, s.k1f_tiles, s.F ? (uint32_t)s.ncf : 0u,
              l->kw, l->ev_bits, nullptr, l->counts + kCntK1F, (unsigned long long*)(l->counts + kCntClk),
              nullptr, nullptr, r->k1f_maxlen, 0, nullptr, nullptr};
    if (!r->adapted && total >= adapt_bytes &&
        (rc = adapt_k1f(r, l, A, in.data, sizeof(uint32_t) * (uint64_t)s.F * s.W, sizeof(uint32_t) * s.nchunks_pad,
                        s.grid_cap)))
      return rc;
    if (k1f_list) {
      A.evlist = l->evlist;
      A.nev = l->counts + kCntEvChunks;
      A.evcap = (uint32_t)std::min<size_t>(l->evlist.cap, 0xFFFFFFFFu);
      A.zone = r->k1f_maxlen;
      A.claim = l->zclaim;
    }
    static const bool wtrace = getenv("TSG_K1F_TRACE") != nullptr;
    if (wtrace && total) {
      const size_t nw = (size_t)k1f_grid(r, s.k1f_tiles, s.grid_cap) * (kFThreads / 64);
      if ((rc = l->wtrace.ensure(4 * nw))) return rc;
      HIP_TRY(hipMemsetAsync(l->wtrace, 0, sizeof(unsigned long long) * 4 * nw, st));
      A.wtrace = l->wtrace;
      l->wtrace_n = 4 * nw;
    }
    if (total && (rc = launch_k1f(r, A, s.grid_cap, st))) return rc;
  } else if (!r->adapted && s.k1_items >= 64 && total >= adapt_bytes) {
    if ((rc = adapt_k1(r, l, total, s.F, s.nchunks, s.k1_items, s.grid_cap))) return rc;
  }
  if (!s.k1f && s.k1_items) {
    K1Args A{data, l->off, l->cf, total, s.nchunks, s.k1_items, 1, s.C, s.F, l->kw, l->ev_bits, nullptr, (uint32_t)kK1Seg};
    if ((rc = launch_k1(r, A, s.grid_cap, st))) return rc;
  }
  if (r->has_k1x && total) {
    const int xg = capped_grid(
        std::max<uint64_t>(1, std::min<uint64_t>((total / 16 + kK1XBlock - 1) / kK1XBlock, (uint64_t)r->cus)), s.grid_cap);
    K1XArgs X{data, l->off, l->cf, total, s.C, s.F, l->kw, l->ev_bits, l->xlist, l->xcount,
              (uint32_t)std::min<size_t>(l->xlist.cap, 0xFFFFFFFFu), l->counts + kCntK1X};
    void* xa[] = {(void*)&r->k1x, (void*)&X};
    HIP_TRY(hipLaunchKernel(k1x_fn(r->k1x.step), dim3(xg), dim3(kK1XBlock), xa, kXDwords * 4 + 16, st));
    if (r->k1x.img_bytes <= kXImgLds)
      k1x_verify_kernel<true><<<xg, kXVerifyBlock, r->k1x.img_bytes, st>>>(r->k1x, X, (uint32_t)xg);
    else
      k1x_verify_kernel<false><<<xg, kXVerifyBlock, 0, st>>>(r->k1x, X, (uint32_t)xg);
    HIP_TRY(hipGetLastError());
  }
  HIP_TRY(hipEventRecord(out->ev[kEvGates], st));

  ItemArgs IA{};
  IA.off = l->off;
  IA.cf = l->cf;
  IA.ev = l->ev_bits;
  IA.ggate = l->ggate;
  IA.gofbit = r->d_gofbit;
  IA.gevents = r->d_gevents;
  IA.gback = r->d_gback;
  IA.nchunks = s.nchunks;
  IA.F = s.F;
  IA.G = s.G;
  IA.GW = r->GW;
  IA.chunk = s.C;
  IA.maxback = r->maxback;
  IA.count = l->gcount;
  IA.bcount = l->bcount;
  IA.cursor = l->cursor;
  IA.evlist = l->evlist;
  IA.nev = l->counts + kCntEvChunks;
  IA.evcap = (uint32_t)std::min<size_t>(l->evlist.cap, 0xFFFFFFFFu);
  IA.items = l->items;
  IA.kw = l->kw;
  IA.W = s.W;
  IA.kwg = r->d_kwg;
  IA.galw = r->d_galw;
  IA.clk = (unsigned long long*)(l->counts + kCntClk);
  if (s.work && k1f_list) {
    IA.ggate = nullptr;
  } else if (s.work) {
    const uint32_t cgrid = (uint32_t)capped_grid(
        std::min<uint64_t>((s.nchunks + kEvPer * kBlock - 1) / (kEvPer * kBlock), (uint64_t)r->grid), s.grid_cap);
    GateArgs GA{l->ev_bits, s.nchunks, l->evlist, l->counts + kCntEvChunks, cgrid, l->kw, s.F, s.W, r->GW, r->d_kwg, r->d_galw, l->ggate,
                (unsigned long long*)(l->counts + kCntClk), s.kwg_bytes <= kKwgLdsMax ? s.kwg_bytes : 0u};
    gates_kernel<<<cgrid + (s.F + kBlock - 1) / kBlock, kBlock, GA.kwg_lds, st>>>(GA);
    HIP_TRY(hipGetLastError());
  }
  if (s.work) {
    const int igrid = capped_grid((uint64_t)std::min(r->grid, r->cus * kItemsBpc), s.grid_cap);
    IA.kwg_lds = !IA.ggate && s.kwg_bytes <= kItemKwgLdsMax ? s.kwg_bytes : 0u;
    const size_t ilds = item_lds_host(s.G, r->GW) + IA.kwg_lds;
    hipLaunchKernelGGL(items_count_kernel, dim3(igrid), dim3(kBlock), ilds + s.G * sizeof(uint32_t) + 16, st, IA);
    HIP_TRY(hipGetLastError());
    LayoutArgs LA{l->gcount, s.G, s.nchunks, s.items_cap, s.max_dense, l->entries, l->counts + kCntListEntries,
                  l->dentries, l->counts + kCntDenseEntries, l->gskip, l->counts + kCntLayout};
    hipLaunchKernelGGL(items_emit_kernel, dim3(igrid), dim3(kBlock), ilds + 3 * s.G * sizeof(uint32_t) + s.G + 16, st, IA, LA);
    HIP_TRY(hipGetLastError());
  }
  HIP_TRY(hipEventRecord(out->ev[kEvK2], st));

  if (s.work) {
    K2Args A{};
    A.data = data;
    A.off = l->off;
    A.cf = l->cf;
    A.total = total;
    A.nchunks = s.nchunks;
    A.chunk = s.C;
    A.ext_cap = r->ext_cap;
    A.nfiles = s.F;
    A.kw = l->kw;
    A.kw_words = s.W;
    A.gmask = r->d_gmask;
    A.galways = r->d_galways;
    A.items = l->items;
    A.entries = l->entries;
    A.nentries = l->counts + kCntListEntries;
    A.dentries = l->dentries;
    A.ndentries = l->counts + kCntDenseEntries;
    A.cand = l->cand;
    A.cand_count = l->counts + kCntCand;
    A.cand_cap = out->cand_cap;
    A.ovf = l->ovf;
    A.hascand = l->hascand;
    static const bool diag = getenv("TSG_K2_DIAG") != nullptr;
    A.diag = diag ? l->counts + kCntK2Diag : nullptr;
    A.claim = l->counts + kCntK2Claim;
    A.word_recs = s.G <= 0x3FFF && !knobs().k2_no_word_recs.load();
    static const bool trace = getenv("TSG_K2_TRACE") != nullptr;
    if (trace && (rc = l->etrace.ensure((size_t)s.entries_cap * kTraceW))) return rc;
    if (trace) HIP_TRY(hipMemsetAsync(l->etrace, 0, sizeof(unsigned long long) * s.entries_cap * kTraceW, st));
    A.etrace = trace ? l->etrace.p : nullptr;
    A.clk = (unsigned long long*)(l->counts + kCntClk);
    const int k2g = capped_grid((uint64_t)r->k2_grid, s.grid_cap), k2dg = capped_grid((uint64_t)r->k2_dense_grid, s.grid_cap);
    if (r->k2_rich)
      hipLaunchKernelGGL(k2_kernel_rich, dim3(k2g), dim3(kK2Block), r->max_lds, st, (const DevDFA*)r->d_groups, A);
    else
      hipLaunchKernelGGL(k2_kernel, dim3(k2g), dim3(kK2Block), r->max_lds, st, (const DevDFA*)r->d_groups, A);
    HIP_TRY(hipGetLastError());
    hipLaunchKernelGGL(k2_dense_kernel, dim3(k2dg), dim3(kBlock), r->max_lds, st,
                       (const DevDFA*)r->d_groups, A);
    HIP_TRY(hipGetLastError());
  }
  HIP_TRY(hipEventRecord(out->ev[kEvOut], st));
  HIP_TRY(hipEventRecord(r->kernels_done, st));
  r->kernels_done_valid = true;

  {
    OutArgs OA{};
    OA.count = l->counts;
    OA.cand_cap = out->cand_cap;
    OA.cand = (const uint8_t*)l->cand.p;
    OA.cand_host = (uint8_t*)out->cand_dev;
    auto copy = [&](void* host, const void* dev, uint64_t n) {
      if (n) {
        OA.dst[OA.nc] = out->blk_dev + ((uint8_t*)host - out->blk);
        OA.src[OA.nc] = (const uint8_t*)dev;
        OA.n[OA.nc++] = n;
      }
    };
    copy(out->counts, l->counts, sizeof(uint32_t) * kCounts);
    copy(out->gskip, l->gskip, s.G);
    OA.kw = l->kw;
    OA.kw_host = (uint32_t*)(out->blk_dev + ((uint8_t*)out->kw - out->blk));
    OA.ovf = l->ovf;
    OA.hascand = l->hascand;
    OA.flags_host = out->blk_dev + (out->ovf - out->blk);
    OA.F = s.F;
    OA.W = s.W;
    OA.fb_lo = (uint32_t)p.fb_kw0;
    OA.fb_hi = (uint32_t)p.n_kw;
    OA.all_rows = r->all_kw_rows;
    outputs_kernel<<<capped_grid(128, s.grid_cap), 256, 0, st>>>(OA);
    HIP_TRY(hipGetLastError());
  }
  HIP_TRY(hipEventRecord(out->ev[kEvDone], st));
  return TSG_OK;
}

int batch_times(const HostOut* o, ScanTimes* t) {
  auto between = [&](BatchEvent a, BatchEvent b, float* ms) { return hipEventElapsedTime(ms, o->ev[a], o->ev[b]); };
  HIP_TRY(between(kEvH2D, kEvMeta, &t->h2d));
  HIP_TRY(between(kEvMeta, kEvPrep, &t->meta));
  HIP_TRY(between(kEvPrep, kEvWait, &t->prep));
  HIP_TRY(between(kEvWait, kEvK1, &t->wait));
  HIP_TRY(between(kEvK1, kEvGates, &t->k1));
  HIP_TRY(between(kEvGates, kEvK2, &t->gates));
  HIP_TRY(between(kEvK2, kEvOut, &t->k2));
  HIP_TRY(between(kEvOut, kEvDone, &t->out));
  const unsigned long long* c = (const unsigned long long*)(o->counts + kCntClk);
  const double per_ms = o->wall_khz ? (double)o->wall_khz : 100000.0;
  const unsigned long long k1s = ~c[kClkK1FStart], k1e = c[kClkK1FEnd], gs = ~c[kClkGatesStart], k2e = c[kClkK2End];
  t->k1_clk = c[kClkK1FStart] && k1e > k1s ? (float)((k1e - k1s) / per_ms) : 0.f;
  t->chain_clk = c[kClkK1FStart] && k2e > k1s ? (float)((k2e - k1s) / per_ms) : 0.f;
  t->post_k1_clk = c[kClkGatesStart] && k2e > gs ? (float)((k2e - gs) / per_ms) : 0.f;
  return TSG_OK;
}

static int lane_sync(LaneState* l) {
  HIP_TRY(hipSetDevice(l->d->device));
  HIP_TRY(hipStreamSynchronize(l->st));
  return TSG_OK;
}

int lane_k2_trace(LaneState* l, std::vector<unsigned long long>* out) {
  if (int rc = lane_sync(l)) return rc;
  out->clear();
  if (!l->etrace) return TSG_OK;
  uint32_t nent = 0;
  HIP_TRY(hipMemcpy(&nent, l->counts + kCntListEntries, sizeof(nent), hipMemcpyDeviceToHost));
  const size_t n = std::min<size_t>((size_t)nent * kTraceW, l->etrace.cap);
  out->resize(n);
  if (n) HIP_TRY(hipMemcpy(out->data(), l->etrace, n * sizeof(unsigned long long), hipMemcpyDeviceToHost));
  return TSG_OK;
}

int lane_k1f_trace(LaneState* l, std::vector<unsigned long long>* out) {
  if (int rc = lane_sync(l)) return rc;
  out->assign(l->wtrace ? l->wtrace_n : 0, 0);
  if (!out->empty()) HIP_TRY(hipMemcpy(out->data(), l->wtrace, out->size() * sizeof(unsigned long long), hipMemcpyDeviceToHost));
  return TSG_OK;
}

int lane_kw(LaneState* l, uint32_t* kw, size_t n) {
  if (int rc = lane_sync(l)) return rc;
  if (n) HIP_TRY(hipMemcpy(kw, l->kw, sizeof(uint32_t) * n, hipMemcpyDeviceToHost));
  return TSG_OK;
}

int lane_items(LaneState* l, LaneItems* out) {
  if (int rc = lane_sync(l)) return rc;
  uint32_t nent = 0, ndent = 0, nitems = 0;
  HIP_TRY(hipMemcpy(&nent, l->counts + kCntListEntries, sizeof(nent), hipMemcpyDeviceToHost));
  HIP_TRY(hipMemcpy(&ndent, l->counts + kCntDenseEntries, sizeof(ndent), hipMemcpyDeviceToHost));
  HIP_TRY(hipMemcpy(&nitems, l->counts + kCntItems, sizeof(nitems), hipMemcpyDeviceToHost));
  const size_t ne = std::min<size_t>(nent, l->entries.cap), nd = std::min<size_t>(ndent, l->dentries.cap),
               ni = std::min<size_t>(nitems, l->items.cap), G = l->d->groups.size();
  out->entries.assign(4 * ne, 0);
  out->dentries.assign(4 * nd, 0);
  out->items.assign(2 * ni, 0);
  out->gskip.assign(G, 0);
  out->extent = nitems;
  if (ne) HIP_TRY(hipMemcpy(out->entries.data(), l->entries, sizeof(uint4) * ne, hipMemcpyDeviceToHost));
  if (nd) HIP_TRY(hipMemcpy(out->dentries.data(), l->dentries, sizeof(uint4) * nd, hipMemcpyDeviceToHost));
  if (ni) HIP_TRY(hipMemcpy(out->items.data(), l->items, sizeof(uint2) * ni, hipMemcpyDeviceToHost));
  if (G) HIP_TRY(hipMemcpy(out->gskip.data(), l->gskip, G, hipMemcpyDeviceToHost));
  return TSG_OK;
}

int lane_events(LaneState* l, uint32_t* ev, size_t n) {
  if (int rc = lane_sync(l)) return rc;
  if (n && l->nchunks)
    HIP_TRY(hipMemcpy(ev, l->ev_bits, sizeof(uint32_t) * std::min<uint64_t>(n, l->nchunks), hipMemcpyDeviceToHost));
  return TSG_OK;
}

struct DeviceFetch {
  DeviceRules* d = nullptr;
  std::mutex m;
  hipStream_t st = nullptr;
  hipEvent_t ev[2] = {};
  FetchSeg* segs = nullptr;
  FetchSeg* segs_dev = nullptr;
  size_t segs_cap = 0;
  GatherSeg* gsegs = nullptr;
  GatherSeg* gsegs_dev = nullptr;
  size_t gsegs_cap = 0;
  uint64_t* marks = nullptr;
  uint64_t marks_cap = 0;
  ~DeviceFetch() {
    if (!d) return;
    (void)hipSetDevice(d->device);
    if (st) (void)hipStreamSynchronize(st);
    if (segs) (void)hipHostFree(segs);
    if (gsegs) (void)hipHostFree(gsegs);
    if (marks) (void)hipFree(marks);
    for (auto& e : ev)
      if (e) (void)hipEventDestroy(e);
    if (st) (void)hipStreamDestroy(st);
  }
};

int fetch_create(DeviceRules* d, DeviceFetch** out) {
  HIP_TRY(hipSetDevice(d->device));
  auto f = std::make_unique<DeviceFetch>();
  f->d = d;
  HIP_TRY(hipStreamCreateWithFlags(&f->st, hipStreamNonBlocking));
  for (auto& e : f->ev) HIP_TRY(hipEventCreate(&e));
  *out = f.release();
  return TSG_OK;
}

void fetch_destroy(DeviceFetch* f) { delete f; }

struct FetchCall {
  std::lock_guard<std::mutex> g;
  int rc;
  explicit FetchCall(DeviceFetch* f)
      : g(f->m), rc(hipSetDevice(f->d->device) == hipSuccess ? TSG_OK : fail(TSG_ERR_GPU, "hipSetDevice failed")) {}
};

template <class Work, class Behind>
int fetch_run(DeviceFetch* f, float* ms, Work work, Behind behind) {
  HIP_TRY(hipEventRecord(f->ev[0], f->st));
  if (int rc = work()) return rc;
  HIP_TRY(hipEventRecord(f->ev[1], f->st));
  if (int rc = behind()) return rc;
  HIP_TRY(hipEventSynchronize(f->ev[1]));
  HIP_TRY(hipEventElapsedTime(ms, f->ev[0], f->ev[1]));
  return TSG_OK;
}
template <class Work>
int fetch_run(DeviceFetch* f, float* ms, Work work) {
  return fetch_run(f, ms, work, [] { return (int)TSG_OK; });
}

int fetch_segments(DeviceFetch* f, const uint8_t* d_src, uint64_t total, uint8_t* host_dst, const GatherSeg* segs,
                   size_t nsegs, float* ms) {
  *ms = 0;
  if (!nsegs) return TSG_OK;
  if (nsegs > 0xFFFFFFFFu) return fail(TSG_ERR_INTERNAL, "too many fetch segments");
  for (size_t k = 0; k < nsegs; k++)
    if (segs[k].src != segs[k].dst || segs[k].dst > total || segs[k].len > total - segs[k].dst)
      return fail(TSG_ERR_INTERNAL, "fetch segment outside the batch");
  FetchCall call(f);
  if (call.rc) return call.rc;
  if (f->segs_cap < nsegs) {
    if (f->segs) HIP_TRY(hipHostFree(f->segs));
    f->segs = nullptr;
    f->segs_cap = 0;
    const size_t cap = nsegs + nsegs / 2 + 1024;
    HIP_TRY(hipHostMalloc((void**)&f->segs, sizeof(FetchSeg) * cap, hipHostMallocMapped));
// ... 106 lines not shown
```

### trivy_amd/csrc/knobs.cpp

```cpp
#include <cstdlib>
#include <cstring>
#include <mutex>
#include <string>

#include "internal.hpp"

namespace tsg {

Knobs& knobs() {
  static Knobs k;
  return k;
}

std::string knob_kw_unknown() {
  Knobs& k = knobs();
  std::lock_guard<std::mutex> g(k.m);
  return k.emu_kw_unknown;
}

}

extern "C" int tsg_test_knob(const char* name, const char* value) {
  using namespace tsg;
  if (!name) return fail(TSG_ERR_ARG, "bad argument");
  const std::string v = value ? value : "";
  const long long x = v.empty() ? 0 : strtoll(v.c_str(), nullptr, 10);
  Knobs& k = knobs();
  if (!strcmp(name, "tar_range_kib")) k.tar_range_kib = x;
  else if (!strcmp(name, "piece_mib")) k.piece_mib = x;
  else if (!strcmp(name, "pike_only")) k.pike_only = x;
  else if (!strcmp(name, "no_k1x")) k.no_k1x = x;
  else if (!strcmp(name, "emu_wordrec")) k.emu_wordrec = x;
  else if (!strcmp(name, "k1_automaton")) k.k1_automaton = x;
  else if (!strcmp(name, "group_states")) k.group_states = x;
  else if (!strcmp(name, "k1f_list")) k.k1f_list = x;
  else if (!strcmp(name, "k1f_grid")) {
    if (x < 0) return fail(TSG_ERR_ARG, "k1f_grid must be >= 0");
    k.k1f_grid = x;
  }
  else if (!strcmp(name, "grid_cap")) {
    if (x < 0) return fail(TSG_ERR_ARG, "grid_cap must be >= 0");
    k.grid_cap = x;
  }
  else if (!strcmp(name, "device_poison")) k.device_poison = x;
  else if (!strcmp(name, "k2_no_word_recs")) k.k2_no_word_recs = x;
  else if (!strcmp(name, "k2_items_cap")) {
    if (x < 0 || x > 0x7FFFFFFF) return fail(TSG_ERR_ARG, "k2_items_cap must be 0..2^31-1");
    k.k2_items_cap = x;
  }
  else if (!strcmp(name, "k2_max_dense")) {
    if (x < 0 || x > 16) return fail(TSG_ERR_ARG, "k2_max_dense must be 0..16");
    k.k2_max_dense = x;
  }
  else if (!strcmp(name, "group_table_kib")) {
    if (x < 0 || x > 64) return fail(TSG_ERR_ARG, "group_table_kib must be 0..64");
    k.group_table_kib = x;
  }
  else if (!strcmp(name, "x_step")) {
    if (x != 0 && x != 1 && x != 2 && x != 4) return fail(TSG_ERR_ARG, "x_step must be 0, 1, 2 or 4");
    k.x_step = x;
  }
  else if (!strcmp(name, "emu_kw_unknown")) {
    std::lock_guard<std::mutex> g(k.m);
    k.emu_kw_unknown = v;
  } else {
    return fail(TSG_ERR_ARG, std::string("unknown knob: ") + name);
  }
  return TSG_OK;
}
```

### trivy_amd/csrc/pipeline.cpp

```cpp
#include <hip/hip_runtime_api.h>
#include <malloc.h>

#include <algorithm>
#include <chrono>
#include <condition_variable>
#include <cstdio>
#include <cstdlib>
#include <cstring>
#include <deque>
#include <functional>
#include <map>
#include <set>
#include <memory>
#include <mutex>
#include <thread>
#include <vector>

#include "device.hpp"
#include "internal.hpp"

namespace tsg {

#define HIP_TRY(x)                                                                    \
  do {                                                                                \
// ... 1247 lines not shown
  if (!c) return fail(TSG_ERR_ARG, "bad argument");
  return guard([&]() -> int {
    std::lock_guard<std::mutex> g(c->m);
    if (slot_id >= c->slots.size() || c->slots[slot_id]->owner != kCaller) return fail(TSG_ERR_ARG, "not an acquired slot");
    Slot& s = *c->slots[slot_id];
    int rc = check_layout(s, nfiles);
    if (rc) return rc;
    const size_t W = (size_t)c->rs->plan->kw_words;
    BatchView view{s.data, s.off, nfiles, s.paths, s.poff};
    if (c->emulate) {
      std::vector<uint32_t> kwv, evv;
      k1_reference(*c->rs->plan, view, c->opt.chunk_bytes, &kwv, &evv);
      if (kw) std::memcpy(kw, kwv.data(), sizeof(uint32_t) * std::min(kw_len, kwv.size()));
      if (ev) std::memcpy(ev, evv.data(), sizeof(uint32_t) * std::min(ev_len, evv.size()));
      return TSG_OK;
    }
    int oi;
    if ((rc = out_take(c, nfiles, &oi))) return rc;
    LaneState* l = c->lanes[c->seq++ % c->lanes.size()];
    const ScanInput in = slot_input(s, nfiles);
    if ((rc = enqueue_scan(c->dr, l, in, &c->outs[oi]))) {
      c->out_busy[oi] = 0;
      return rc;
    }
    HostOut ho = c->outs[oi];
    hipError_t e = hipEventSynchronize(ho.ev[kEvDone]);
    if (e == hipSuccess) {
      Batch b;
      (void)batch_times(&ho, &b.t);
      std::memcpy(b.counts, ho.counts, sizeof(b.counts));
      b.bytes = s.off[nfiles];
      b.cand_cap = ho.cand_cap;
      update_stats(c, b);
      c->kernels_lane = l;
      c->kernels_slot = slot_id;
      c->kernels_seq = c->seq;
      c->kernels_out = oi;
      c->kernels_nfiles = nfiles;
      if (kw) rc = lane_kw(l, kw, std::min(kw_len, W * nfiles));
      if (ev && !rc) rc = lane_events(l, ev, ev_len);
      if (const char* tp = getenv("TSG_K1F_TRACE")) {
        std::vector<unsigned long long> tr;
        if (!rc) rc = lane_k1f_trace(l, &tr);
        if (FILE* f = tr.empty() ? nullptr : fopen(tp, "ab")) {
          fwrite(tr.data(), sizeof(unsigned long long), tr.size(), f);
          fclose(f);
        }
      }
      if (const char* tp = getenv("TSG_K2_TRACE")) {
        std::vector<unsigned long long> tr;
        if (!rc) rc = lane_k2_trace(l, &tr);
        if (FILE* f = tr.empty() ? nullptr : fopen(tp, "ab")) {
          fwrite(tr.data(), sizeof(unsigned long long), tr.size(), f);
          fclose(f);
        }
      }
    }
    c->out_busy[oi] = 0;
    if (e != hipSuccess) return fail(TSG_ERR_GPU, std::string("tsg_batch_kernels: ") + hipGetErrorString(e));
    return rc;
  });
}

int tsg_batch_items(tsg_ctx* c, uint32_t slot_id, uint32_t* entries, size_t entries_cap, uint32_t* dentries,
                    size_t dentries_cap, uint32_t* items, size_t items_cap, uint8_t* gskip, size_t gskip_len,
                    uint64_t* n) {
  if (!c || !n) return fail(TSG_ERR_ARG, "bad argument");
  return guard([&]() -> int {
    std::lock_guard<std::mutex> g(c->m);
    if (c->emulate) return fail(TSG_ERR_ARG, "an emulated context has no device work lists");
    if (!c->kernels_lane || c->kernels_slot != slot_id || c->kernels_seq != c->seq)
      return fail(TSG_ERR_ARG, "tsg_batch_items follows tsg_batch_kernels on the same slot");
    LaneItems li;
    int rc = lane_items(c->kernels_lane, &li);
    if (rc) return rc;
    n[0] = li.entries.size() / 4;
    n[1] = li.dentries.size() / 4;
    n[2] = li.extent;
    if (entries) std::memcpy(entries, li.entries.data(), 16 * std::min<size_t>(entries_cap, n[0]));
    if (dentries) std::memcpy(dentries, li.dentries.data(), 16 * std::min<size_t>(dentries_cap, n[1]));
    if (items) std::memcpy(items, li.items.data(), 8 * std::min<size_t>(items_cap, li.items.size() / 2));
    if (gskip) std::memcpy(gskip, li.gskip.data(), std::min(gskip_len, li.gskip.size()));
    return TSG_OK;
  });
}

int tsg_batch_candidates(tsg_ctx* c, uint32_t slot_id, uint32_t* records, size_t records_cap, uint8_t* flags,
                         size_t flags_len, uint32_t* kw, size_t kw_len, uint64_t* n) {
  if (!c || !n) return fail(TSG_ERR_ARG, "bad argument");
  return guard([&]() -> int {
    std::lock_guard<std::mutex> g(c->m);
    if (c->emulate) return fail(TSG_ERR_ARG, "an emulated context has no device output block");
    if (!c->kernels_lane || c->kernels_slot != slot_id || c->kernels_seq != c->seq || c->kernels_out < 0)
      return fail(TSG_ERR_ARG, "tsg_batch_candidates follows tsg_batch_kernels on the same slot");
    const HostOut& ho = c->outs[c->kernels_out];
    const uint32_t F = c->kernels_nfiles;
    if (!ho.blk || ho.files_cap < F) return fail(TSG_ERR_INTERNAL, "the output block of the last tsg_batch_kernels is gone");
    const size_t W = ho.kw_words;
    const uint32_t nrec = std::min<uint32_t>(ho.counts[kCntCand], ho.cand_cap);
    n[0] = ho.counts[kCntCand];
    n[1] = nrec;
    n[2] = F;
    n[3] = ho.cand_cap;
    if (records) std::memcpy(records, ho.cand, sizeof(Candidate) * std::min<size_t>(records_cap, nrec));
    if (flags) std::memcpy(flags, ho.ovf, std::min<size_t>(flags_len, F));
    if (kw)
      for (uint32_t f = 0; f < F && (size_t)(f + 1) * W <= kw_len; f++) {
        if (ho.ovf[f] & 4) std::memcpy(kw + (size_t)f * W, ho.kw + (size_t)f * W, sizeof(uint32_t) * W);
        else std::memset(kw + (size_t)f * W, 0, sizeof(uint32_t) * W);
      }
    return TSG_OK;
  });
}

int tsg_test_adaptation(tsg_ctx* c, tsg_adaptation_info* info, uint8_t* kw_unknown, size_t kw_unknown_len,
                        uint8_t* gate_open, size_t gate_open_len, uint8_t* event_everywhere,
                        size_t event_everywhere_len, uint32_t* hits, size_t hits_len, uint8_t* quiet, size_t quiet_len) {
  if (!c || !info) return fail(TSG_ERR_ARG, "bad argument");
  return guard([&]() -> int {
    std::lock_guard<std::mutex> g(c->m);
    const Plan& p = *c->rs->plan;
    AdaptationView v;
    if (c->emulate || !c->dr) {
      v.kw_unknown.assign(p.n_kw, 0);
      for (const auto& gp : p.groups) {
        v.gate_open.push_back(gp.always ? 1 : 0);
        v.event_everywhere.push_back((gp.events & kEvAlways) ? 1 : 0);
      }
    } else if (int rc = device_rules_adaptation(c->dr, &v)) {
      return rc;
    }
    std::memset(info, 0, sizeof(*info));
    info->adapted = v.adapted;
    info->k1_filter = v.k1_filter;
    info->hot_states = v.hot_states;
    info->ev_hot = v.ev_hot;
    info->sample_bytes = v.sample_bytes;
    info->n_keywords = (uint32_t)v.kw_unknown.size();
    info->n_groups = (uint32_t)v.gate_open.size();
    info->n_literals = (uint32_t)v.hits.size();
    auto give = [](auto* dst, size_t cap, const auto& src) {
      if (dst && !src.empty()) std::memcpy(dst, src.data(), sizeof(src[0]) * std::min(cap, src.size()));
    };
    give(kw_unknown, kw_unknown_len, v.kw_unknown);
    give(gate_open, gate_open_len, v.gate_open);
    give(event_everywhere, event_everywhere_len, v.event_everywhere);
    give(hits, hits_len, v.hits);
    give(quiet, quiet_len, v.quiet);
    return TSG_OK;
  });
}

int tsg_ctx_get_stats(const tsg_ctx* c, tsg_stats* out) {
  if (!c || !out) return fail(TSG_ERR_ARG, "bad argument");
  std::lock_guard<std::mutex> g(c->m);
  *out = c->stats;
  return TSG_OK;
}

int tsg_queue_create(tsg_ctx* c, uint32_t flush_us, tsg_queue** out) {
  if (!c || !out) return fail(TSG_ERR_ARG, "bad argument");
  return guard([&]() -> int {
    auto q = std::make_unique<tsg_queue>();
    q->c = c;
    q->flush_us = flush_us ? flush_us : 2000;
    q->slot_bytes = (uint64_t)(c->opt.slot_mib ? c->opt.slot_mib : 256) << 20;
// ... 128 lines not shown
```

### trivy_amd/csrc/plan.cpp

```cpp
#include "plan.hpp"
#include "internal.hpp"
#include <deque>
#include <condition_variable>
#include <mutex>
#include <functional>

#include <algorithm>
#include <chrono>
#include <cstdio>
#include <cstdlib>
#include <atomic>
#include <map>
#include <unordered_map>
#include <unordered_set>
#include <set>
#include <thread>
#include <x86intrin.h>

namespace tsg {

static std::string ascii_lower(std::string s) {
  for (char& c : s)
    if (c >= 'A' && c <= 'Z') c = (char)(c + 32);
  return s;
}

static bool is_ascii(const std::string& s) {
  for (unsigned char c : s)
    if (c >= 0x80) return false;
  return true;
}

static const std::unordered_set<uint32_t>& common4() {
  static const std::unordered_set<uint32_t> set = [] {
    static const char kCommon4[][5] = {
#include "common4.inc"
    };
    std::unordered_set<uint32_t> s;
    for (const auto& g : kCommon4) s.insert(x_prefix4((const uint8_t*)g));
    return s;
  }();
  return set;
}

static void x_place_windows(Plan* p, int step) {
  std::unordered_map<uint32_t, uint32_t> mult;
  for (const auto& l : p->x_lits) {
    std::unordered_set<uint32_t> mine;
    for (size_t j = 0; j + 4 <= l.size(); j++) mine.insert(x_prefix4((const uint8_t*)l.data() + j));
    for (uint32_t g : mine) mult[g]++;
  }
  p->x_j0.assign(p->x_lits.size(), 0);
  for (size_t i = 0; i < p->x_lits.size(); i++) {
    const std::string& l = p->x_lits[i];
    const size_t last = std::min(l.size() - 3 - (size_t)step, (size_t)256 - (size_t)step);
    uint64_t best = UINT64_MAX;
    for (size_t j = 0; j <= last; j++) {
      uint64_t c = 0;
      for (size_t t = j; t < j + (size_t)step; t++) {
        const uint32_t g = x_prefix4((const uint8_t*)l.data() + t);
        c += (common4().count(g) ? 1000000u : 0u) + mult[g];
      }
      if (c < best) {
        best = c;
        p->x_j0[i] = (uint8_t)j;
      }
    }
  }
}

static int x_pick(const std::string& l, int step, uint32_t* j0) {
  if (l.size() < (size_t)step + 3) return -1;
  const size_t last = std::min(l.size() - 3 - (size_t)step, (size_t)256 - (size_t)step);
  int best = -1;
  for (size_t j = 0; j <= last && best != 0; j++) {
    int c = 0;
    for (size_t t = j; t < j + (size_t)step; t++) c += common4().count(x_prefix4((const uint8_t*)l.data() + t)) ? 1 : 0;
    if (best < 0 || c < best) {
      best = c;
      *j0 = (uint32_t)j;
    }
  }
  return best;
}

namespace {

bool in_set(const uint64_t* set, const uint8_t* cls, int bit) {
  for (int c = 0; c < 128; c++)
    if (((set[c >> 6] >> (c & 63)) & 1) && !((cls[c] >> bit) & 1)) return false;
  return true;
}

struct Anchor {
  uint32_t kind = kEvAlways;
  std::string lit;
  int first_atom = 0;
  int64_t evdist = 0;
  std::string desc = "none";
};

Anchor choose_anchor(const Regexp& re, const Plan& p, bool literal_first) {
  const std::vector<AtomInfo> at = re.Atoms();
  const int n = (int)at.size();
  std::vector<int64_t> B(n + 1, 0);
  for (int i = 0; i < n; i++)
    B[i + 1] = (B[i] < 0 || at[i].max_bytes < 0) ? -1 : B[i] + at[i].max_bytes;
  Anchor best;
  auto take = [&](uint32_t kind, int t, int64_t len, const std::string& lit, const char* what) {
    Anchor a;
    a.kind = kind;
    a.lit = lit;
    if (B[t] >= 0) {
      a.first_atom = 0;
      a.evdist = B[t] + len - 1;
    } else {
      a.first_atom = t;
      a.evdist = len - 1;
    }
    a.desc = std::string(what) + (lit.empty() ? "" : " '" + lit + "'") + " at atom " +
             std::to_string(t) + (a.first_atom ? " (suffix)" : "");
    return a;
  };
  double best_score = 0;
  auto best_literal = [&]() {
    for (int i = 0; i < n;) {
      if (at[i].lit < 0) {
        i++;
        continue;
      }
      int j = i;
      std::string s;
      double score = 0;
      while (j < n && at[j].lit >= 0) {
        int c = at[j].lit;
        if (s.size() < 24) {
          s.push_back((char)c);
          score += (c >= 'a' && c <= 'z') ? 1.0 : (c >= '0' && c <= '9') ? 1.3 : 1.6;
        }
        j++;
      }
      if (score >= 3.0 && score > best_score) {
        best_score = score;
        best = take(1u << kEvLit0, i, (int64_t)s.size(), s, "literal");
      }
      i = j;
    }
  };
  if (literal_first) {
    best_literal();
    if (best_score >= 6.0) return best;
    best = Anchor();
    best_score = 0;
  }
  for (int bit = 0; bit < 2; bit++) {
    const int k = p.run_k[bit];
    for (int i = 0; i < n;) {
      if (!(at[i].ascii_only && in_set(at[i].set, p.run_cls, bit))) {
        i++;
        continue;
      }
      int j = i;
      int64_t run = 0;
      while (j < n && at[j].ascii_only && in_set(at[j].set, p.run_cls, bit)) run += at[j++].min_bytes;
      if (run >= k) return take(bit == 0 ? kEvRunU : kEvRunD, i, k, "", bit == 0 ? "run U" : "run D");
      i = j;
    }
  }
  best_literal();
  return best;
}

size_t product_states(const DFA& a, const DFA& b, size_t cap) {
  std::vector<uint8_t> seen((size_t)a.nstates * b.nstates, 0);
  std::vector<std::pair<uint32_t, uint32_t>> stack;
  uint16_t pcls[256][2];
  int np = 0;
  {
    std::map<std::pair<int, int>, int> idx;
    for (int c = 0; c < 256; c++) {
      auto k = std::make_pair((int)a.cls[c], (int)b.cls[c]);
      if (!idx.count(k)) idx[k] = np++;
      pcls[c][0] = (uint16_t)a.cls[c];
      pcls[c][1] = (uint16_t)b.cls[c];
    }
  }
  std::vector<int> rep;
  {
    std::set<std::pair<int, int>> done;
    for (int c = 0; c < 256; c++)
      if (done.insert({pcls[c][0], pcls[c][1]}).second) rep.push_back(c);
  }
  size_t n = 0;
  auto push = [&](uint32_t x, uint32_t y) {
    uint8_t& v = seen[(size_t)x * b.nstates + y];
    if (v) return;
    v = 1;
    n++;
    stack.push_back({x, y});
  };
  for (int c = 0; c < 4; c++) push(a.start[c], b.start[c]);
  while (!stack.empty() && n <= cap) {
    auto [x, y] = stack.back();
    stack.pop_back();
    for (int c : rep) push(a.next[(size_t)x * a.nclasses + pcls[c][0]], b.next[(size_t)y * b.nclasses + pcls[c][1]]);
  }
  return n;
}

}

std::unique_ptr<Plan> build_plan(const Ruleset& rs, const PlanOptions& opt, std::string* err) {
  auto p = std::make_unique<Plan>();
  const size_t R = rs.rules.size();
  p->rule_kw_mode.assign(R, kKwAlways);
  p->rule_kws.assign(R, {});
  p->rule_group.assign(R, -1);
  p->rule_hostonly.assign(R, 0);
  p->rule_maxlen.assign(R, -1);
  p->rule_event.assign(R, kEvAlways);
  p->rule_evdist.assign(R, 0);
  p->rule_first_atom.assign(R, 0);
  p->rule_anchor.assign(R, "none");
  for (int c = 0; c < 256; c++) {
    bool u = (c >= 'A' && c <= 'Z') || (c >= 'a' && c <= 'z') || (c >= '0' && c <= '9') ||
             c == '+' || c == '/' || c == '=' || c == '_' || c == '.' || c == '-';
    bool d = (c >= '0' && c <= '9') || c == '-';
    p->run_cls[c] = (uint8_t)((u ? 1 : 0) | (d ? 2 : 0));
  }

  std::map<std::string, uint32_t> kwid;
  std::vector<std::string> kws;
  for (size_t r = 0; r < R; r++) {
    const RuleC& rule = rs.rules[r];
    if (rule.kw_lower.empty()) continue;
    bool ascii = true;
    for (const auto& k : rule.kw_lower) ascii &= is_ascii(k);
    if (!ascii) {
      p->rule_kw_mode[r] = kKwUnknown;
      continue;
    }
    p->rule_kw_mode[r] = kKwBits;
    for (const auto& k : rule.kw_lower) {
      auto it = kwid.find(k);
      uint32_t id;
      if (it == kwid.end()) {
        id = (uint32_t)kws.size();
        kwid[k] = id;
        kws.push_back(k);
      } else {
        id = it->second;
      }
      p->rule_kws[r].push_back(id);
    }
  }
  p->fb_kw0 = (int)kws.size();
  kws.push_back("\xc4\xb0");
  kws.push_back("\xe2\x84\xaa");
  kws.push_back("\xc5\xbf");
  p->n_kw = (int)kws.size();
  p->kw_words = (p->n_kw + 31) / 32;
  for (const auto& k : kws) p->kw_len.push_back((uint16_t)std::min<size_t>(k.size(), 0xFFFF));

  DFAOptions one;
  one.max_states = opt.max_group_states;
  auto fits = [&](const DFA& d, size_t nrules) {
    return d.nstates <= opt.max_group_states &&
           (size_t)d.nstates * d.nclasses * 2 <= (size_t)opt.max_group_table_bytes &&
           (int)nrules <= opt.max_rules_per_group;
  };
  p->rule_relax.assign(R, -1);
  p->rule_atoms.assign(R, -1);
  p->rule_winback.assign(R, -1);
  p->rule_prog.assign(R, Prog{});
  std::vector<std::unique_ptr<DFA>> single(R);
  const auto t_rules0 = std::chrono::steady_clock::now();
  std::vector<Anchor> anchor(R);
  const int plan_threads = (int)std::max(1u, std::min(16u, std::thread::hardware_concurrency()));
  pool_for(R, plan_threads, [&](size_t r) {
    const RuleC& rule = rs.rules[r];
    if (!rule.regex) return;
    p->rule_maxlen[r] = max_match_len(rule.regex->prog());
    if (opt.anchors) anchor[r] = choose_anchor(*rule.regex, *p, rule.kw_lower.empty());
    const int fa = anchor[r].first_atom;
    for (int k : {-1, 32, 16, 8, 4, 2, 1, 0}) {
      Prog pr = (k < 0 && fa == 0) ? rule.regex->prog() : rule.regex->RelaxedProg(k, -1, fa);
      std::string e;
      auto d = build_dfa({&pr}, one, &e);
      if (d && fits(*d, 1)) {
        single[r] = std::move(d);
        p->rule_relax[r] = k;
        p->rule_prog[r] = std::move(pr);
        break;
      }
    }
    for (int t = rule.regex->NumAtoms() - fa - 1; !single[r] && t >= 1; t--) {
      for (int k : {8, 2, 0}) {
        Prog pr = rule.regex->RelaxedProg(k, t, fa);
        std::string e;
        auto d = build_dfa({&pr}, one, &e);
        if (d && fits(*d, 1)) {
          single[r] = std::move(d);
          p->rule_relax[r] = k;
          p->rule_atoms[r] = t;
          p->rule_prog[r] = std::move(pr);
          break;
        }
      }
    }
    if (!single[r]) {
      p->rule_hostonly[r] = 1;
      return;
    }
    if (fa > 0) {
      p->rule_winback[r] = -1;
    } else if (p->rule_atoms[r] >= 0) {
      p->rule_winback[r] = max_match_len(rule.regex->RelaxedProg(-1, p->rule_atoms[r]));
    } else {
      p->rule_winback[r] = p->rule_maxlen[r];
    }
    p->rule_event[r] = anchor[r].kind;
    p->rule_evdist[r] = anchor[r].evdist;
    p->rule_first_atom[r] = fa;
    p->rule_anchor[r] = anchor[r].desc;
  }, 1);

  const bool tprof = getenv("TSG_PROF") != nullptr;
  auto tnow = [] { return std::chrono::steady_clock::now(); };
  auto tms = [](std::chrono::steady_clock::time_point a) {
    return std::chrono::duration<double, std::milli>(std::chrono::steady_clock::now() - a).count();
  };
  auto tp = tnow();
  if (tprof) fprintf(stderr, "plan: per-rule DFAs %.1f ms\n", tms(t_rules0));
  auto group_kwmask = [&](GroupPlan& g) {
    g.kwmask.assign(p->kw_words, 0);
    for (uint32_t r : g.rules) {
      if (p->rule_kw_mode[r] != kKwBits) {
        g.always = true;
        continue;
      }
      for (uint32_t k : p->rule_kws[r]) g.kwmask[k / 32] |= 1u << (k % 32);
    }
  };
  for (uint32_t kind : {kEvRunU, kEvRunD, 1u << kEvLit0, kEvAlways}) {
    std::vector<uint32_t> cur;
    std::unique_ptr<DFA> cur_dfa;
    auto flush = [&]() {
      if (cur.empty()) return;
      GroupPlan g;
      g.dfa = std::move(cur_dfa);
      g.rules = cur;
      group_kwmask(g);
      g.events = kind;
      g.evdist = 0;
      for (uint32_t r : cur) {
        p->rule_group[r] = (int)p->groups.size();
        g.evdist = std::max(g.evdist, p->rule_evdist[r]);
      }
      p->groups.push_back(std::move(g));
      cur.clear();
    };
    for (size_t r = 0; r < R; r++) {
      if (!single[r] || p->rule_event[r] != kind) continue;
      if (cur.empty()) {
        cur.push_back((uint32_t)r);
        cur_dfa = std::move(single[r]);
        continue;
      }
      if (cur_dfa->nstates + single[r]->nstates > opt.max_group_states ||
          product_states(*cur_dfa, *single[r], opt.max_group_states) > (size_t)opt.max_group_states) {
        flush();
        cur.push_back((uint32_t)r);
        cur_dfa = std::move(single[r]);
        continue;
      }
      std::vector<const Prog*> progs;
      for (uint32_t q : cur) progs.push_back(&p->rule_prog[q]);
      progs.push_back(&p->rule_prog[r]);
      std::string e;
      auto merged = build_dfa(progs, one, &e);
      if (getenv("TSG_PROF2"))
        fprintf(stderr, "merge %d+%d (nc %d,%d) -> %d %s\n", cur_dfa->nstates, single[r]->nstates,
                cur_dfa->nclasses, single[r]->nclasses, merged ? merged->nstates : -1,
                merged && fits(*merged, cur.size() + 1) ? "ok" : "FAIL");
      if (merged && fits(*merged, cur.size() + 1)) {
        cur.push_back((uint32_t)r);
        cur_dfa = std::move(merged);
      } else {
        flush();
        cur.push_back((uint32_t)r);
        cur_dfa = std::move(single[r]);
      }
    }
    flush();
  }

  if (tprof) {
    fprintf(stderr, "plan: grouping %.1f ms (%zu groups)\n", tms(tp), p->groups.size());
    for (size_t g = 0; g < p->groups.size(); g++)
      fprintf(stderr, "plan: group %zu: %zu rules, %d states x %d classes (%zu table bytes), events %#x\n", g,
              p->groups[g].rules.size(), p->groups[g].dfa->nstates, p->groups[g].dfa->nclasses,
              (size_t)p->groups[g].dfa->nstates * p->groups[g].dfa->nclasses * 2, p->groups[g].events);
  }
  tp = tnow();
  std::vector<char> litg(p->groups.size(), 0);
  for (size_t g = 0; g < p->groups.size(); g++) litg[g] = p->groups[g].events == (1u << kEvLit0);
  std::vector<char> kw_dropped(kws.size(), 0);
  std::vector<char> kw_hashed(kws.size(), 0), anchor_hashed(R, 0);
  auto build_k1 = [&](bool with_anchors) -> bool {
    std::vector<std::string> lits = kws;
    for (size_t k = 0; k < lits.size(); k++)
      if (kw_dropped[k] || kw_hashed[k]) lits[k] = never_literal();
    std::map<std::string, std::pair<int32_t, uint32_t>> xl;
    for (size_t k = 0; k < kws.size(); k++)
      if (kw_hashed[k]) xl[ascii_lower(kws[k])] = {(int32_t)k, 0u};
    std::vector<uint32_t> lit_event(lits.size(), 0);
    std::map<std::string, uint32_t> lid;
    for (size_t i = 0; i < lits.size(); i++) lid.emplace(lits[i], (uint32_t)i);
    int nlitgroups = 0;
    for (size_t gi = 0; gi < p->groups.size(); gi++) {
      GroupPlan& g = p->groups[gi];
      if (!litg[gi]) continue;
      if (!with_anchors) {
        g.events = kEvAlways;
        for (uint32_t r : g.rules) p->rule_event[r] = kEvAlways;
        continue;
      }
      const uint32_t bit = 1u << (kEvLit0 + (nlitgroups++ % kEvLitBits));
      g.events = bit;
      for (uint32_t r : g.rules) {
        p->rule_event[r] = bit;
        const std::string& s = anchor[r].lit;
        if (anchor_hashed[r]) {
          auto xi = xl.find(ascii_lower(s));
          if (xi == xl.end()) xl[ascii_lower(s)] = {-1, bit};
          else xi->second.second |= bit;
          continue;
        }
        auto it = lid.find(s);
        uint32_t id;
// ... 877 lines not shown
    (*ev)[p / chunk] |= e;
  }
  k1x_reference(plan, bv, chunk, kw, ev);
}

void k1x_reference(const Plan& plan, const BatchView& bv, uint32_t chunk, std::vector<uint32_t>* kw,
                   std::vector<uint32_t>* ev) {
  if (plan.x_lits.empty()) return;
  const uint64_t total = bv.offsets[bv.nfiles];
  std::unordered_map<uint32_t, std::vector<uint32_t>> by4;
  for (size_t i = 0; i < plan.x_lits.size(); i++) by4[x_prefix4((const uint8_t*)plan.x_lits[i].data())].push_back((uint32_t)i);
  auto low = [](uint8_t c) -> uint8_t { return (c >= 'A' && c <= 'Z') ? (uint8_t)(c + 32) : c; };
  for (uint64_t p = 0; p + 4 <= total; p++) {
    const uint8_t b4[4] = {low(bv.data[p]), low(bv.data[p + 1]), low(bv.data[p + 2]), low(bv.data[p + 3])};
    auto it = by4.find(x_prefix4(b4));
    if (it == by4.end()) continue;
    for (uint32_t i : it->second) {
      const std::string& L = plan.x_lits[i];
      if (p + L.size() > total) continue;
      size_t t = 4;
      while (t < L.size() && low(bv.data[p + t]) == (uint8_t)L[t]) t++;
      if (t < L.size()) continue;
      const uint64_t q = p + L.size() - 1;
      (*ev)[q / chunk] |= plan.x_event[i];
      if (plan.x_kw[i] >= 0) {
        const uint32_t f = (uint32_t)(std::upper_bound(bv.offsets, bv.offsets + bv.nfiles + 1, q) - bv.offsets) - 1;
        if (p >= bv.offsets[f]) (*kw)[(size_t)f * plan.kw_words + plan.x_kw[i] / 32] |= 1u << (plan.x_kw[i] % 32);
      }
    }
  }
}

static void emulate_records(const DFA& d, uint32_t gi, const std::vector<uint32_t>& rules, const uint8_t* data,
                            uint32_t f, uint64_t fs, uint64_t fe, uint64_t a, uint64_t b, uint32_t ext_cap,
                            bool body_words, bool tail_words, std::vector<Candidate>* out) {
  const uint32_t nc = (uint32_t)d.nclasses, ncd = std::max<uint32_t>(2, nc);
  auto eot = [&](uint32_t s) {
    if (!d.eot_acc[s]) return;
    const auto& m = d.masks[d.eot_acc[s]];
    for (size_t k = 0; k < rules.size(); k++)
      if ((m[k / 64] >> (k % 64)) & 1) out->push_back({f, rules[k], (uint32_t)(fe - fs)});
  };
  auto step = [&](uint32_t& s, uint64_t p, uint64_t e, bool words) {
    const uint32_t s0 = s;
    const uint64_t p0 = p;
    bool acc = false;
    for (; p < e; p++) {
      const uint32_t c = d.cls[data[p]];
      const size_t x = (size_t)s * nc + c;
      if (d.acc[x] && !words) out->push_back({f, kCandTrans | (gi << 16) | (s * ncd + c), (uint32_t)(p - fs)});
      acc |= d.acc[x] != 0;
      s = d.next[x];
    }
    if (acc && words) out->push_back({f, kCandTrans | kCandWord | (gi << 16) | (s0 * ncd), (uint32_t)(p0 - fs)});
  };
  uint32_t s = (a == fs) ? d.start[kCtxBOT] : d.start[DFA::ctx_of(data[a - 1], d)];
  for (uint64_t p = a; p < b;) {
    const uint64_t e = std::min<uint64_t>(b, (p | 15) + 1);
    step(s, p, e, body_words);
    p = e;
  }
  if (b >= fe) {
    eot(s);
    return;
  }
  s = d.to_noinject[s];
  uint64_t q = b;
  while (q < fe && !d.dead[s]) {
    if (q - b >= ext_cap || (s < d.immortal.size() && d.immortal[s])) {
      for (uint32_t r : rules) out->push_back({f, r, kCandWhole});
      return;
    }
    const uint64_t e = std::min<uint64_t>(fe, (q | 15) + 1);
    step(s, q, e, tail_words);
    q = e;
  }
  if (q >= fe && !d.dead[s]) eot(s);
}

void emulate_items(const Plan& plan, const BatchView& bv, uint32_t chunk, const uint32_t* kwbits,
                   const std::vector<uint32_t>& ev, uint32_t max_back,
                   const std::function<void(uint32_t g, uint32_t f, uint64_t c)>& visit) {
  const uint32_t F = bv.nfiles;
  for (size_t gi = 0; gi < plan.groups.size(); gi++) {
    const GroupPlan& g = plan.groups[gi];
    const uint32_t back = group_back(g, chunk);
    const bool every = (g.events & kEvAlways) != 0 || back > max_back;
    for (uint32_t f = 0; f < F; f++) {
      const uint64_t fs = bv.offsets[f], fe = bv.offsets[f + 1];
      if (fe == fs) continue;
      const uint32_t* kw = kwbits + (size_t)f * plan.kw_words;
      bool gate = g.always;
      for (int w = 0; w < plan.kw_words && !gate; w++) gate = (kw[w] & g.kwmask[w]) != 0;
      if (!gate) continue;
      const uint64_t c0 = fs / chunk, c1 = (fe - 1) / chunk;
      for (uint64_t c = c0; c <= c1; c++) {
        bool need = every;
        for (uint64_t q = c; q <= std::min<uint64_t>(c + back, c1) && !need; q++) need = (ev[q] & g.events) != 0;
        if (need) visit((uint32_t)gi, f, c);
      }
    }
  }
}

void layout_reference(const uint64_t* counts, uint32_t ngroups, uint64_t nchunks, uint64_t items_cap,
                      uint32_t max_dense, uint8_t* kind, LayoutTotals* totals) {
  LayoutTotals t;
  const uint64_t dense_all = (nchunks + kK2EntryChunks - 1) / kK2EntryChunks;
  uint64_t dense_wanted = 0;
  for (uint32_t g = 0; g < ngroups; g++) {
    const uint64_t cnt = counts[g];
    uint8_t k = kGroupNone;
    if (cnt * 2 > nchunks) {
      k = dense_wanted++ < max_dense ? kGroupDense : kGroupSkip;
      if (k == kGroupDense) t.dense_entries += dense_all;
    } else if (cnt) {
      k = t.extent + cnt <= items_cap ? kGroupList : kGroupSkip;
      if (k == kGroupList) t.entries += (cnt + kK2EntryItems - 1) / kK2EntryItems;
      t.extent += cnt;
    }
    t.skipped += k == kGroupSkip;
    if (kind) kind[g] = k;
  }
  if (totals) *totals = t;
}

void emulate_kernels(const Plan& plan, const BatchView& bv, uint32_t chunk, uint32_t ext_cap,
                     KernelOutput* ko, std::vector<uint64_t>* group_item_bytes, const EmuOptions* opt,
                     EmuStats* st) {
  const uint32_t F = bv.nfiles;
  const size_t G = plan.groups.size();
  const bool word_recs = knobs().emu_wordrec.load() && !knobs().k2_no_word_recs.load() && G <= 0x3FFF;
  const uint32_t max_back = opt ? opt->max_back : 0xFFFFFFFFu;
  std::vector<uint32_t> ev;
  k1_reference(plan, bv, chunk, &ko->kw, &ev);
  ko->cand.clear();
  ko->overflow.assign(F, 0);
  ko->group_skipped.clear();
  if (group_item_bytes) group_item_bytes->assign(G, 0);
  std::vector<uint8_t> kind;
  EmuStats es;
  if (opt && opt->layout) {
    std::vector<uint64_t> counts(G, 0);
    emulate_items(plan, bv, chunk, ko->kw.data(), ev, max_back, [&](uint32_t g, uint32_t, uint64_t) { counts[g]++; });
    kind.resize(G);
    layout_reference(counts.data(), (uint32_t)G, ev.size(), opt->items_cap, opt->max_dense, kind.data(), &es.layout);
    if (es.layout.skipped) {
      ko->group_skipped.assign(G, 0);
      for (size_t g = 0; g < G; g++) ko->group_skipped[g] = kind[g] == kGroupSkip;
    }
  }
  emulate_items(plan, bv, chunk, ko->kw.data(), ev, max_back, [&](uint32_t gi, uint32_t f, uint64_t c) {
    if (!kind.empty() && kind[gi] == kGroupSkip) return;
    const GroupPlan& g = plan.groups[gi];
    const DFA& d = *g.dfa;
    const uint64_t fs = bv.offsets[f], fe = bv.offsets[f + 1];
    const uint64_t a = std::max<uint64_t>(fs, c * chunk), b = std::min<uint64_t>(fe, (c + 1) * chunk);
    if (group_item_bytes) (*group_item_bytes)[gi] += b - a;
    if (word_recs) {
      emulate_records(d, gi, g.rules, bv.data, f, fs, fe, a, b, ext_cap, true, true, &ko->cand);
      return;
    }
    bool o = run_segment(d, bv.data, fs, fe, a, b, ext_cap, [&](uint32_t mi, uint64_t pos) {
      const auto& m = d.masks[mi];
      for (size_t k = 0; k < g.rules.size(); k++)
        if ((m[k / 64] >> (k % 64)) & 1) ko->cand.push_back({f, g.rules[k], (uint32_t)pos});
    });
    if (o)
      for (uint32_t r : g.rules) ko->cand.push_back({f, r, kCandWhole});
  });
  es.candidates = ko->cand.size();
  if (opt && ko->cand.size() > opt->cand_cap) {
    for (size_t i = (size_t)opt->cand_cap; i < ko->cand.size(); i++) ko->overflow[ko->cand[i].file] = 1;
    ko->cand.resize((size_t)opt->cand_cap);
  }
  if (st) *st = es;
}

void emulate_candidates(const Plan& plan, const BatchView& bv, uint32_t chunk, uint32_t ext_cap, uint64_t items_cap,
                        uint32_t max_dense, bool word_recs, std::vector<Candidate>* out) {
  const uint32_t F = bv.nfiles;
  const size_t G = plan.groups.size();
  const uint64_t total = bv.offsets[F];
  const bool words = word_recs && G <= 0x3FFF;
// ... 51 lines not shown
```

### trivy_amd/csrc/plan.hpp

```cpp
#pragma once
#include <cstdint>
#include <functional>
#include <memory>
#include <string>
#include <vector>

#include "dfa.hpp"
#include "scanner.hpp"

namespace tsg {

enum KwMode : uint8_t { kKwAlways = 0, kKwBits = 1, kKwUnknown = 2 };

constexpr uint32_t kEvRunU = 1u;
constexpr uint32_t kEvRunD = 2u;
constexpr int kEvLit0 = 2;
constexpr int kEvLitBits = 29;
constexpr uint32_t kEvAlways = 1u << 31;

struct GroupPlan {
  std::unique_ptr<DFA> dfa;
  std::vector<uint32_t> rules;
  std::vector<uint32_t> kwmask;
  bool always = false;
  uint32_t events = kEvAlways;
  int64_t evdist = 0;
};

struct Plan {
  std::unique_ptr<DFA> kw_dfa;
  int n_kw = 0;
  int n_lit = 0;
  int kw_words = 1;
  int fb_kw0 = 0;
  std::vector<uint32_t> kw_mask_events;
  std::vector<uint32_t> lit_event;
  std::vector<std::string> k1_lits;
  std::vector<uint16_t> kw_len;
  std::vector<std::string> x_lits;
  std::vector<int32_t> x_kw;
  std::vector<uint32_t> x_event;
  int x_step = 1;
  std::vector<uint8_t> x_j0;
  uint8_t run_cls[256] = {0};
  int run_k[2] = {32, 12};
  int warm = 32;
  std::vector<uint32_t> rule_event;
  std::vector<int64_t> rule_evdist;
  std::vector<int> rule_first_atom;
  std::vector<std::string> rule_anchor;
  std::vector<uint8_t> rule_kw_mode;
  std::vector<std::vector<uint32_t>> rule_kws;
  std::vector<GroupPlan> groups;
  std::vector<int> rule_group;
  std::vector<uint8_t> rule_hostonly;
  std::vector<int64_t> rule_maxlen;
  std::vector<int> rule_relax;
  std::vector<int> rule_atoms;
  std::vector<int64_t> rule_winback;
  std::vector<Prog> rule_prog;
  std::vector<std::unique_ptr<DFA>> rule_rev;
  std::vector<std::unique_ptr<DFA>> rule_fold_dfa;
  std::unique_ptr<DFA> fold_all_dfa;
  std::vector<uint32_t> fold_rules;
  std::unique_ptr<DFA> allow_path_dfa;
};

struct PlanOptions {
  int max_group_states = 1024;
  int max_group_table_bytes = 48 * 1024;
  int max_rules_per_group = 64;
  int max_kw_table_bytes = 96 * 1024;
  bool anchors = true;
};

std::unique_ptr<Plan> build_plan(const Ruleset& rs, const PlanOptions& opt, std::string* err);

constexpr uint32_t kCandWhole = 0xFFFFFFFFu;
constexpr uint32_t kCandTrans = 0x80000000u;
constexpr uint32_t kCandWord = 0x40000000u;
struct Candidate {
  uint32_t file;
  uint32_t rule;
  uint32_t end;
};

struct KernelOutputView {
  const uint32_t* kw = nullptr;
  const Candidate* cand = nullptr;
  size_t ncand = 0;
  const uint8_t* overflow = nullptr;
  bool sparse_kw = false;
  const uint8_t* kw_unknown = nullptr;
  const uint8_t* path_ok = nullptr;
  const uint8_t* group_skipped = nullptr;
};

enum : uint8_t { kGroupNone = 0, kGroupList = 1, kGroupDense = 2, kGroupSkip = 3 };
constexpr uint32_t kMaxBackChunks = 16;
constexpr uint32_t kK2EntryItems = 512;
constexpr uint32_t kK2EntryChunks = 1024;

struct LayoutTotals {
  uint64_t extent = 0;
  uint64_t entries = 0;
  uint64_t dense_entries = 0;
  uint64_t skipped = 0;
};
void layout_reference(const uint64_t* counts, uint32_t ngroups, uint64_t nchunks, uint64_t items_cap,
                      uint32_t max_dense, uint8_t* kind, LayoutTotals* totals);

struct KernelOutput {
  std::vector<uint32_t> kw;
  std::vector<Candidate> cand;
  std::vector<uint8_t> overflow;
  std::vector<uint8_t> kw_unknown;
  std::vector<uint8_t> path_ok;
  std::vector<uint8_t> group_skipped;
  KernelOutputView view() const {
    KernelOutputView v;
    v.kw = kw.data();
    v.cand = cand.data();
    v.ncand = cand.size();
    v.overflow = overflow.empty() ? nullptr : overflow.data();
    v.kw_unknown = kw_unknown.empty() ? nullptr : kw_unknown.data();
    v.path_ok = path_ok.empty() ? nullptr : path_ok.data();
    v.group_skipped = group_skipped.empty() ? nullptr : group_skipped.data();
    return v;
  }
};

struct BatchView {
  const uint8_t* data;
  const uint64_t* offsets;
  uint32_t nfiles;
  const char* paths;
  const uint64_t* path_offsets;
};

std::vector<uint32_t> host_rules(const Plan& plan, const KernelOutputView& ko);

inline bool file_needs_scan(const Plan& plan, const KernelOutputView& ko, uint32_t f, bool has_cand, bool empty,
                            bool any_host) {
  if (has_cand || empty || (ko.overflow && (ko.overflow[f] & 1)) || any_host) return true;
  if (ko.sparse_kw) return (ko.overflow[f] & 2) != 0;
  const uint32_t* kw = ko.kw + (size_t)f * plan.kw_words;
  for (int k = plan.fb_kw0; k < plan.n_kw; k++)
    if ((kw[k / 32] >> (k % 32)) & 1) return true;
  return false;
}

void fold_rune_positions(const uint8_t* s, int64_t n, uint32_t which, std::vector<int64_t>* out);

void resolve_batch(const Ruleset& rs, const Plan& plan, const BatchView& b,
                   const KernelOutputView& ko, int nthreads, BatchResult* out);

void scan_batch_cpu(const Ruleset& rs, const BatchView& b, int nthreads,
                    std::vector<FileResult>* out);

struct EmuOptions {
  uint32_t max_back = 0xFFFFFFFFu;
  bool layout = false;
  uint64_t items_cap = 0;
  uint32_t max_dense = 0;
  uint64_t cand_cap = ~0ull;
};
struct EmuStats {
  uint64_t candidates = 0;
  LayoutTotals layout;
};
void emulate_kernels(const Plan& plan, const BatchView& b, uint32_t chunk, uint32_t ext_cap,
                     KernelOutput* ko, std::vector<uint64_t>* group_item_bytes = nullptr,
                     const EmuOptions* opt = nullptr, EmuStats* st = nullptr);

void emulate_candidates(const Plan& plan, const BatchView& b, uint32_t chunk, uint32_t ext_cap, uint64_t items_cap,
                        uint32_t max_dense, bool word_recs, std::vector<Candidate>* out);

void expand_candidate(const Plan& plan, const BatchView& b, const Candidate& c, std::vector<Candidate>* out);

void emulate_items(const Plan& plan, const BatchView& b, uint32_t chunk, const uint32_t* kw,
                   const std::vector<uint32_t>& ev, uint32_t max_back,
                   const std::function<void(uint32_t g, uint32_t f, uint64_t c)>& visit);

void k1_reference(const Plan& plan, const BatchView& b, uint32_t chunk,
                  std::vector<uint32_t>* kw, std::vector<uint32_t>* ev);
void k1x_reference(const Plan& plan, const BatchView& b, uint32_t chunk,
                   std::vector<uint32_t>* kw, std::vector<uint32_t>* ev);

inline uint32_t x_prefix4(const uint8_t* b) {
  return (uint32_t)b[0] | (uint32_t)b[1] << 8 | (uint32_t)b[2] << 16 | (uint32_t)b[3] << 24;
}
constexpr int kXDwordBits = 15;
constexpr uint32_t kXDwords = 1u << kXDwordBits;
constexpr uint32_t kXFold = 0x20202020u;
inline uint32_t x_fold(uint32_t w) { return w | kXFold; }
inline uint32_t x_hash(uint32_t w) { return w * 2654435761u; }
inline uint32_t x_dword(uint32_t h) { return h >> (32 - kXDwordBits); }
inline uint32_t x_bits(uint32_t h) { return 1u << ((h >> 12) & 31) | 1u << ((h >> 7) & 31); }

inline uint32_t group_back(const GroupPlan& g, uint32_t chunk) {
  return (uint32_t)((g.evdist + chunk - 1) / chunk);
}

}
```

### trivy_amd/secret.py

```python
import ctypes as C
import json
import os
import struct
from dataclasses import dataclass, field
from typing import List, Optional

import numpy as np
import yaml

from . import _native as N

_RULES_JSON = os.path.join(os.path.dirname(os.path.abspath(__file__)), "rules",
                           "builtin_rules.json")


class ConfigError(ValueError):
    """secrets config decode / regexp compile error (scanner.go:74-77, 286-288)."""


def _check_regex(src):
    h = C.c_void_p()
    err = C.create_string_buffer(512)
    rc = N.lib().tsg_regex_compile(src.encode("utf-8", "surrogateescape"), C.byref(h), err, 512)
    if rc != N.TSG_OK:
# ... 239 lines not shown
        import numpy as np
        W = (self.info()["n_keywords"] + 31) // 32
        kw = np.zeros(batch.nfiles * W, dtype=np.uint32)
        ev = np.zeros((int(batch.offsets[-1]) + chunk - 1) // chunk, dtype=np.uint32)
        u32p = C.POINTER(C.c_uint32)
        N.check(N.lib().tsg_emulate_k1(self.handle, C.c_void_p(batch.data.ctypes.data),
                                       batch.offsets.ctypes.data_as(C.POINTER(C.c_uint64)),
                                       batch.nfiles, chunk, kw.ctypes.data_as(u32p), kw.size,
                                       ev.ctypes.data_as(u32p), ev.size))
        return kw.reshape(batch.nfiles, W), ev

    def emulate_items(self, batch, chunk, max_back=16):
        G = self.info()["n_groups"]
        counts = np.zeros(max(G, 1), dtype=np.uint64)
        n = C.c_uint64()
        u64p = C.POINTER(C.c_uint64)
        args = (self.handle, C.c_void_p(batch.data.ctypes.data), batch.offsets.ctypes.data_as(u64p),
                batch.nfiles, chunk, max_back)
        N.check(N.lib().tsg_emulate_items(*args, None, 0, counts.ctypes.data_as(u64p), C.byref(n)))
        tri = np.zeros((max(n.value, 1), 3), dtype=np.uint32)
        N.check(N.lib().tsg_emulate_items(*args, tri.ctypes.data_as(C.POINTER(C.c_uint32)), n.value,
                                          None, None))
        return tri[:n.value], counts[:G]

    def emulate_candidates(self, batch, chunk, ext_cap=DEFAULT_EXT_CAP, items_cap=None, max_dense=16,
                           word_recs=True):
        if items_cap is None:
            items_cap = default_items_cap((int(batch.offsets[-1]) + chunk - 1) // chunk)
        u64p, u32p = C.POINTER(C.c_uint64), C.POINTER(C.c_uint32)
        args = (self.handle, C.c_void_p(batch.data.ctypes.data), batch.offsets.ctypes.data_as(u64p),
                batch.nfiles, chunk, int(ext_cap), int(items_cap), int(max_dense), 1 if word_recs else 0)
        n = C.c_uint64()
        N.check(N.lib().tsg_emulate_candidates(*args, None, 0, C.byref(n)))
        rec = np.zeros((max(n.value, 1), 3), dtype=np.uint32)
        N.check(N.lib().tsg_emulate_candidates(*args, rec.ctypes.data_as(u32p), n.value, None))
        return rec[:n.value]

    def emulate_item_candidates(self, batch, chunk, ext_cap=DEFAULT_EXT_CAP):
        u64p, u32p = C.POINTER(C.c_uint64), C.POINTER(C.c_uint32)
        args = (self.handle, C.c_void_p(batch.data.ctypes.data), batch.offsets.ctypes.data_as(u64p),
                batch.nfiles, chunk, int(ext_cap))
        n = C.c_uint64()
        N.check(N.lib().tsg_emulate_item_candidates(*args, None, 0, C.byref(n)))
        tri = np.zeros((max(n.value, 1), 3), dtype=np.uint32)
        N.check(N.lib().tsg_emulate_item_candidates(*args, tri.ctypes.data_as(u32p), n.value, None))
        return tri[:n.value]

    def expand_candidates(self, batch, records):
        rec = np.ascontiguousarray(records, dtype=np.uint32).reshape(-1, 3)
        u64p, u32p = C.POINTER(C.c_uint64), C.POINTER(C.c_uint32)
        args = (self.handle, C.c_void_p(batch.data.ctypes.data), batch.offsets.ctypes.data_as(u64p),
                batch.nfiles, rec.ctypes.data_as(u32p), len(rec))
        n = C.c_uint64()
        N.check(N.lib().tsg_expand_candidates(*args, None, 0, C.byref(n)))
        tri = np.zeros((max(n.value, 1), 3), dtype=np.uint32)
        N.check(N.lib().tsg_expand_candidates(*args, tri.ctypes.data_as(u32p), n.value, None))
        return tri[:n.value]

    def candidate_stats(self, batch, chunk):
        per_rule = np.zeros(max(len(self.Rules), 1), dtype=np.uint64)
        per_group = np.zeros(max(self.info()["n_groups"], 1), dtype=np.uint64)
        u64p = C.POINTER(C.c_uint64)
        N.check(N.lib().tsg_emulate_candidate_stats(
            self.handle, C.c_void_p(batch.data.ctypes.data), batch.offsets.ctypes.data_as(u64p),
            batch.nfiles, chunk, per_rule.ctypes.data_as(u64p), per_group.ctypes.data_as(u64p)))
        return per_rule[:len(self.Rules)], per_group[:self.info()["n_groups"]]

    def rule_group(self, rule):
        g, relax, ml = C.c_int32(), C.c_int32(), C.c_int64()
        N.check(N.lib().tsg_ruleset_rule_plan(self.handle, rule, C.byref(g), C.byref(relax), C.byref(ml)))
        return g.value

    def rule_plan(self, rule):
        g, relax, ml = C.c_int32(), C.c_int32(), C.c_int64()
        N.check(N.lib().tsg_ruleset_rule_plan(self.handle, rule, C.byref(g), C.byref(relax), C.byref(ml)))
        return {"group": g.value, "relax": relax.value, "maxlen": ml.value}

    def rule_program(self, rule):
        fa, at, wb, rev = C.c_int32(), C.c_int32(), C.c_int64(), C.c_int32()
        N.check(N.lib().tsg_ruleset_rule_program(self.handle, rule, C.byref(fa), C.byref(at), C.byref(wb),
                                                 C.byref(rev)))
        return {"first_atom": fa.value, "rule_atoms": at.value, "rule_winback": wb.value,
                "rule_rev": bool(rev.value)}

    def k1_literals(self):
        out = []
        buf = C.create_string_buffer(1 << 16)
        n, ev = C.c_uint32(), C.c_uint32()
        while N.lib().tsg_ruleset_k1_literal(self._h, len(out), buf, len(buf), C.byref(n), C.byref(ev)) == 0:
            out.append((buf.raw[:n.value], ev.value))
        return out

    def k1f_emulate(self, batch, chunk, quiet=(), sample_kib=0):
        import numpy as np
        W = (self.info()["n_keywords"] + 31) // 32
        kw = np.zeros(batch.nfiles * W, dtype=np.uint32)
        ev = np.zeros((int(batch.offsets[-1]) + chunk - 1) // chunk, dtype=np.uint32)
        q = np.array(list(quiet) or [0], dtype=np.uint32)
        st = np.zeros(4, dtype=np.uint64)
        u32p = C.POINTER(C.c_uint32)
        N.check(N.lib().tsg_emulate_k1f(self.handle, C.c_void_p(batch.data.ctypes.data),
                                        batch.offsets.ctypes.data_as(C.POINTER(C.c_uint64)),
                                        batch.nfiles, chunk, q.ctypes.data_as(u32p), len(quiet),
                                        sample_kib, kw.ctypes.data_as(u32p), kw.size, ev.ctypes.data_as(u32p),
                                        ev.size, st.ctypes.data_as(C.POINTER(C.c_uint64))))
        return kw.reshape(batch.nfiles, W), ev, {"groups": int(st[0]), "arrivals": int(st[1]),
                                                 "records": int(st[2])}

    def AllowPath(self, path):
        b = _b(path)
        rc = N.lib().tsg_ruleset_allow_path(self._h, b, len(b))
        if rc < 0:
            N.check(rc)
        return rc == 1

    def Scan(self, args):
        p = _b(args.FilePath)
        out = C.c_void_p()
        N.check(N.lib().tsg_scan_cpu(self._h, p, len(p), bytes(args.Content), len(args.Content),
                                     C.byref(out)))
        return self.decode(out, [args.FilePath])[0]

    def ScanBatch(self, args, device=None, ctx=None, emulate_chunk=0, nthreads=0):
        batch = args if isinstance(args, Batch) else Batch.from_args(args)
        paths = [batch.path(i) for i in range(batch.nfiles)]
        out = C.c_void_p()
        L = N.lib()
        if device is not None or ctx is not None:
            own = ctx is None
            if own:
                ctx = GpuContext(self, device)
            try:
                N.check(L.tsg_scan_batch(ctx.handle, *batch.ptrs(), C.byref(out)))
            finally:
                if own:
                    ctx.close()
        elif emulate_chunk:
            N.check(L.tsg_scan_batch_emulated(self._h, *batch.ptrs(), emulate_chunk, C.byref(out)))
        else:
            N.check(L.tsg_scan_cpu_batch(self._h, *batch.ptrs(), nthreads, C.byref(out)))
        return self.decode(out, paths)

    def decode(self, out, paths):
        L = N.lib()
        n = C.c_size_t()
        ptr = L.tsg_result_data(out, C.byref(n))
        buf = C.string_at(ptr, n.value)
        L.tsg_result_free(out)
        return decode_results(buf, paths, self.Rules)


GROUP_NONE, GROUP_LIST, GROUP_DENSE, GROUP_SKIP = 0, 1, 2, 3
ENTRY_ITEMS, ENTRY_CHUNKS = 512, 1024
BLOCK_THREADS, EV_PER, K1X_BLOCK, K1X_WORDS, K1X_IMG_LDS, OUT_BLOCKS = 256, 32, 1024, 4, 128 << 10, 128


def default_items_cap(nchunks):
    return max(2 * nchunks, 1 << 16)


def layout_reference(counts, nchunks, items_cap, max_dense=16):
    counts = np.ascontiguousarray(counts, dtype=np.uint64)
    kind = np.zeros(max(len(counts), 1), dtype=np.uint8)
    tot = np.zeros(4, dtype=np.uint64)
    u64p = C.POINTER(C.c_uint64)
    N.check(N.lib().tsg_layout_reference(counts.ctypes.data_as(u64p), len(counts), int(nchunks),
# ... 46 lines not shown

class GpuContext:

    def __init__(self, scanner, device=0, chunk_bytes=0, ext_cap=0, cand_capacity=0,
                 host_threads=0, adapt_mib=0, emulate=False, slot_mib=0, max_slots=0):
        import threading
        self._h = None
        self._owned = True
        self.scanner = scanner
        self.chunk = chunk_bytes or 256
        opt = N.CtxOptions(chunk_bytes, ext_cap, cand_capacity, host_threads, adapt_mib,
                           N.TSG_CTX_EMULATE if emulate else 0, slot_mib, max_slots)
        h = C.c_void_p()
        N.check(N.lib().tsg_ctx_create(int(device), scanner.handle, C.byref(opt), C.byref(h)))
        self._h = h
        self._upload = None
        self._k1 = None
        self._lock = threading.Lock()
        self._fifo = []
        self._paths = {}
        self._tensors = {}
        self._kept = {}
        self._device = int(device)
        self._emulate = bool(emulate)

    @classmethod
    def borrowed(cls, scanner, handle, chunk_bytes=0):
        import threading
        self = cls.__new__(cls)
        self._h = handle
        self._owned = False
        self.scanner = scanner
        self.chunk = chunk_bytes or 256
        self._upload = None
        self._k1 = None
        self._lock = threading.Lock()
        self._fifo = []
        self._paths = {}
        self._tensors = {}
        self._kept = {}
        self._device = None
        self._emulate = False
        return self

    @property
    def handle(self):
        return self._h

    def upload(self, batch):
        sid = C.c_uint32()
        N.check(N.lib().tsg_batch_upload(self._h, *batch.ptrs(), C.byref(sid)))
        with self._lock:
            prev, self._upload = self._upload, (sid.value, batch)
        if prev is not None:
            N.check(N.lib().tsg_slot_release(self._h, prev[0]))

    def kernels(self):
        sid, b = self._upload
        W = (self.scanner.info()["n_keywords"] + 31) // 32
        kw = np.zeros(b.nfiles * W, dtype=np.uint32)
        ev = np.zeros((int(b.offsets[-1]) + self.chunk - 1) // self.chunk, dtype=np.uint32)
        u32p = C.POINTER(C.c_uint32)
        N.check(N.lib().tsg_batch_kernels(self._h, sid, b.nfiles, kw.ctypes.data_as(u32p), kw.size,
                                          ev.ctypes.data_as(u32p), ev.size))
        self._k1 = (kw.reshape(b.nfiles, W), ev)

    def batch_items(self):
        sid, _ = self._upload
        G = self.scanner.info()["n_groups"]
        n = (C.c_uint64 * 3)()
        u32p, u8p = C.POINTER(C.c_uint32), C.POINTER(C.c_uint8)
        N.check(N.lib().tsg_batch_items(self._h, sid, None, 0, None, 0, None, 0, None, 0, n))
        ent = np.zeros((max(n[0], 1), 4), dtype=np.uint32)
        dent = np.zeros((max(n[1], 1), 4), dtype=np.uint32)
        items = np.zeros((max(n[2], 1), 2), dtype=np.uint32)
        gskip = np.zeros(max(G, 1), dtype=np.uint8)
        m = (C.c_uint64 * 3)()
        N.check(N.lib().tsg_batch_items(self._h, sid, ent.ctypes.data_as(u32p), n[0],
                                        dent.ctypes.data_as(u32p), n[1], items.ctypes.data_as(u32p), n[2],
                                        gskip.ctypes.data_as(u8p), G, m))
        assert list(m) == list(n)
        return ent[:n[0]], dent[:n[1]], items[:n[2]], gskip[:G]

    def batch_candidates(self):
        sid, b = self._upload
        W = (self.scanner.info()["n_keywords"] + 31) // 32
        n = (C.c_uint64 * 4)()
        u32p, u8p = C.POINTER(C.c_uint32), C.POINTER(C.c_uint8)
        N.check(N.lib().tsg_batch_candidates(self._h, sid, None, 0, None, 0, None, 0, n))
        assert n[2] == b.nfiles
        rec = np.zeros((max(n[1], 1), 3), dtype=np.uint32)
        flags = np.zeros(max(b.nfiles, 1), dtype=np.uint8)
        kw = np.zeros(max(b.nfiles * W, 1), dtype=np.uint32)
        m = (C.c_uint64 * 4)()
        N.check(N.lib().tsg_batch_candidates(self._h, sid, rec.ctypes.data_as(u32p), n[1],
                                             flags.ctypes.data_as(u8p), b.nfiles,
                                             kw.ctypes.data_as(u32p), b.nfiles * W, m))
        assert list(m) == list(n)
        return {"count": int(n[0]), "cand_cap": int(n[3]), "records": rec[:n[1]],
                "flags": flags[:b.nfiles], "kw": kw[:b.nfiles * W].reshape(b.nfiles, W)}

    def adaptation(self):
        info = N.AdaptationInfo()
        u8p, u32p = C.POINTER(C.c_uint8), C.POINTER(C.c_uint32)
        N.check(N.lib().tsg_test_adaptation(self._h, C.byref(info), None, 0, None, 0, None, 0, None, 0, None, 0))
        nk, ng, nl = info.n_keywords, info.n_groups, info.n_literals
        kwu = np.zeros(max(nk, 1), dtype=np.uint8)
        gate = np.zeros(max(ng, 1), dtype=np.uint8)
        evw = np.zeros(max(ng, 1), dtype=np.uint8)
        hits = np.zeros(max(nl, 1), dtype=np.uint32)
        quiet = np.zeros(max(nl, 1), dtype=np.uint8)
        N.check(N.lib().tsg_test_adaptation(self._h, C.byref(info), kwu.ctypes.data_as(u8p), nk,
                                            gate.ctypes.data_as(u8p), ng, evw.ctypes.data_as(u8p), ng,
                                            hits.ctypes.data_as(u32p), nl, quiet.ctypes.data_as(u8p), nl))
        assert (info.n_keywords, info.n_groups, info.n_literals) == (nk, ng, nl)
        return {"adapted": int(info.adapted), "k1_filter": int(info.k1_filter),
                "hot_states": int(info.hot_states), "ev_hot": int(info.ev_hot),
                "sample_bytes": int(info.sample_bytes), "kw_unknown": kwu[:nk], "gate_open": gate[:ng],
                "event_everywhere": evw[:ng], "hits": hits[:nl] if nl else None,
                "quiet": quiet[:nl] if nl else None}

    def k1_output(self, chunk):
        assert chunk == self.chunk, "the context's chunk is %d" % self.chunk
        return self._k1

    @staticmethod
    def _paths_of(batch):
        if isinstance(batch, Batch):
            return [batch.path(i) for i in range(batch.nfiles)]
        return list(batch)

    def _track(self, ticket, paths_of):
        with self._lock:
            self._fifo.append(ticket)
            self._paths[ticket] = paths_of
        return ticket

    def submit(self):
        sid, b = self._upload
        t = C.c_uint64()
        N.check(N.lib().tsg_slot_submit(self._h, sid, b.nfiles, C.byref(t)))
        return self._track(t.value, b)

    def submit_slot(self, slot_id, nfiles, paths_of):
        if paths_of is None:
            raise ValueError("submit_slot needs the submitted files' paths (a Batch or a list)")
        t = C.c_uint64()
        N.check(N.lib().tsg_slot_submit(self._h, int(slot_id), int(nfiles), C.byref(t)))
        return self._track(t.value, paths_of)

    def acquire_slot(self, data_bytes, nfiles, path_bytes):
        v = N.SlotView()
        N.check(N.lib().tsg_slot_acquire(self._h, int(data_bytes), int(nfiles),
                                         int(path_bytes), C.byref(v)))
        data = np.ctypeslib.as_array((C.c_uint8 * v.data_cap).from_address(v.data))
        offs = np.ctypeslib.as_array(v.offsets, shape=(v.files_cap + 1,))
        paths = np.ctypeslib.as_array((C.c_uint8 * v.paths_cap).from_address(v.paths))
        poffs = np.ctypeslib.as_array(v.path_offsets, shape=(v.files_cap + 1,))
        return v.id, data, offs, paths, poffs

    def release_slot(self, slot_id):
        N.check(N.lib().tsg_slot_release(self._h, int(slot_id)))

    def _take(self, ticket):
        with self._lock:
            if ticket is None:
# ... 277 lines not shown
```

Before: 56.75.

## Refine run-U events into per-rule character-class runs to prune group items

Adds a refine pass that, for chunks flagged with the generic uppercase-run event, re-scans the chunk bytes against up to 32 per-rule character classes and records which class actually has a 32-byte run. Groups whose run-U anchor maps to a class then trigger only on the refined bits instead of the coarse run event, so fewer (file, group, chunk) items reach the expensive regex/DFA stage. The cost is an extra kernel that re-reads data for run-U chunks, plus extra ev_ref loads in the item builder and more LDS per block. It is enabled by default through a new knob, and a host reference plus test hooks are included.

```diff
diff --git a/include/trivy_secret.h b/include/trivy_secret.h
--- a/include/trivy_secret.h
+++ b/include/trivy_secret.h
@@ -122,6 +122,7 @@
 int tsg_batch_items(tsg_ctx* ctx, uint32_t slot_id, uint32_t* entries, size_t entries_cap,
                     uint32_t* dentries, size_t dentries_cap, uint32_t* items, size_t items_cap,
                     uint8_t* gskip, size_t gskip_len, uint64_t* n);
+int tsg_batch_run_refine(tsg_ctx* ctx, uint32_t slot_id, uint32_t* ref, size_t ref_len);
 int tsg_batch_candidates(tsg_ctx* ctx, uint32_t slot_id, uint32_t* records, size_t records_cap,
                          uint8_t* flags, size_t flags_len, uint32_t* kw, size_t kw_len, uint64_t* n);
 
@@ -287,6 +288,12 @@
 
 int tsg_ruleset_rule_anchor(const tsg_ruleset* rs, uint32_t rule, uint32_t* event, int64_t* evdist,
                             char* desc, size_t desc_len);
+
+int tsg_ruleset_rule_class(const tsg_ruleset* rs, uint32_t rule, uint64_t* cls, int32_t* cls_id,
+                           uint32_t* group_mask);
+
+int tsg_emulate_run_refine(const tsg_ruleset* rs, const uint8_t* data, const uint64_t* offsets,
+                           uint32_t nfiles, uint32_t chunk, uint32_t* ref, size_t ref_len);
 
 int tsg_ruleset_k1_literal(const tsg_ruleset* rs, uint32_t i, uint8_t* buf, uint32_t cap,
                            uint32_t* len, uint32_t* event);
diff --git a/trivy_amd/_native.py b/trivy_amd/_native.py
--- a/trivy_amd/_native.py
+++ b/trivy_amd/_native.py
@@ -259,6 +259,11 @@
                                   C.POINTER(C.c_uint32), C.c_size_t, C.POINTER(C.c_uint64)]),
     ("tsg_ruleset_k1_literal", C.c_int, [_P, C.c_uint32, C.c_char_p, C.c_uint32,
                                          C.POINTER(C.c_uint32), C.POINTER(C.c_uint32)]),
+    ("tsg_ruleset_rule_class", C.c_int, [_P, C.c_uint32, _U64P, C.POINTER(C.c_int32),
+                                         C.POINTER(C.c_uint32)]),
+    ("tsg_emulate_run_refine", C.c_int, [_P, _P, _U64P, C.c_uint32, C.c_uint32, C.POINTER(C.c_uint32),
+                                         C.c_size_t]),
+    ("tsg_batch_run_refine", C.c_int, [_P, C.c_uint32, C.POINTER(C.c_uint32), C.c_size_t]),
 ]
 
 _lib = None
diff --git a/trivy_amd/csrc/capi.cpp b/trivy_amd/csrc/capi.cpp
--- a/trivy_amd/csrc/capi.cpp
+++ b/trivy_amd/csrc/capi.cpp
@@ -469,6 +469,38 @@
   return TSG_OK;
 }
 
+int tsg_ruleset_rule_class(const tsg_ruleset* rs, uint32_t rule, uint64_t* cls, int32_t* cls_id,
+                           uint32_t* group_mask) {
+  if (!rs || rule >= rs->rs.rules.size()) return fail(TSG_ERR_ARG, "bad argument");
+  const Plan& p = *rs->plan;
+  const int id = p.rule_cls_id[rule];
+  if (cls) {
+    cls[0] = p.rule_cls[rule][0];
+    cls[1] = p.rule_cls[rule][1];
+  }
+  if (cls_id) *cls_id = id;
+  if (group_mask) *group_mask = id >= 0 && p.rule_group[rule] >= 0 ? p.groups[p.rule_group[rule]].gref : 0u;
+  return TSG_OK;
+}
+
+int tsg_emulate_run_refine(const tsg_ruleset* rs, const uint8_t* data, const uint64_t* offsets,
+                           uint32_t nfiles, uint32_t chunk, uint32_t* ref, size_t ref_len) {
+  if (!rs || !offsets || chunk == 0 || (!ref && ref_len)) return fail(TSG_ERR_ARG, "bad argument");
+  try {
+    std::vector<uint64_t> poff(nfiles + 1, 0);
+    BatchView b{data, offsets, nfiles, "", poff.data()};
+    std::vector<uint32_t> kw, ev, rf;
+    k1_reference(*rs->plan, b, chunk, &kw, &ev);
+    refined_events(*rs->plan, b, chunk, ev, &rf);
+    if (ref) std::memcpy(ref, rf.data(), sizeof(uint32_t) * std::min(ref_len, rf.size()));
+    return TSG_OK;
+  } catch (const std::bad_alloc&) {
+    return fail(TSG_ERR_NOMEM, "out of memory");
+  } catch (const std::exception& ex) {
+    return fail(TSG_ERR_INTERNAL, ex.what());
+  }
+}
+
 int tsg_ruleset_k1_literal(const tsg_ruleset* rs, uint32_t i, uint8_t* buf, uint32_t cap,
                            uint32_t* len, uint32_t* event) {
   if (!rs || (!buf && cap)) return fail(TSG_ERR_ARG, "bad argument");
diff --git a/trivy_amd/csrc/device.hpp b/trivy_amd/csrc/device.hpp
--- a/trivy_amd/csrc/device.hpp
+++ b/trivy_amd/csrc/device.hpp
@@ -123,6 +123,7 @@
 int batch_times(const HostOut* out, ScanTimes* t);
 int lane_kw(LaneState* l, uint32_t* kw, size_t n);
 int lane_events(LaneState* l, uint32_t* ev, size_t n);
+int lane_run_refine(LaneState* l, uint32_t* ref, size_t n);
 struct LaneItems {
   std::vector<uint32_t> entries, dentries, items;
   std::vector<uint8_t> gskip;
diff --git a/trivy_amd/csrc/internal.hpp b/trivy_amd/csrc/internal.hpp
--- a/trivy_amd/csrc/internal.hpp
+++ b/trivy_amd/csrc/internal.hpp
@@ -44,6 +44,7 @@
   std::atomic<int64_t> tar_range_kib{0}, piece_mib{0}, pike_only{0}, no_k1x{0}, emu_wordrec{0},
       x_step{0}, k1_automaton{0}, group_states{0}, group_table_kib{0}, k1f_grid{0},
       k1f_list{0}, k2_items_cap{0}, k2_max_dense{0}, k2_no_word_recs{0}, device_poison{0}, grid_cap{0};
+  std::atomic<int64_t> run_refine{1};
   std::mutex m;
   std::string emu_kw_unknown;
 };
diff --git a/trivy_amd/csrc/kernels.hip b/trivy_amd/csrc/kernels.hip
--- a/trivy_amd/csrc/kernels.hip
+++ b/trivy_amd/csrc/kernels.hip
@@ -1407,6 +1407,8 @@
   const uint64_t* off;
   const uint32_t* cf;
   const uint32_t* ev;
+  const uint32_t* ev_ref;
+  const uint32_t* gref;
   const uint32_t* evlist;
   const uint32_t* nev;
   uint32_t evcap;
@@ -1504,31 +1506,91 @@
   }
 }
 
-static inline size_t item_lds_host(uint32_t G, uint32_t GW) { return 256 * (size_t)GW + 8 * (size_t)G; }
+struct RefineArgs {
+  const uint8_t* data;
+  const uint32_t* ev;
+  const uint32_t* evlist;
+  const uint32_t* nev;
+  uint32_t evcap;
+  uint32_t chunk;
+  const uint32_t* bits;
+  uint32_t* ev_ref;
+};
+constexpr uint32_t kRefineRun = 32;
+static_assert(kBlock == 256, "refine_kernel stages a 256-entry table, an entry per thread");
+__global__ void __launch_bounds__(kBlock) refine_kernel(RefineArgs A) {
+  __shared__ uint32_t s_bits[256];
+  s_bits[threadIdx.x] = A.bits[threadIdx.x];
+  __syncthreads();
+  const uint32_t lane = threadIdx.x & 63, C = A.chunk;
+  const uint32_t WPC = C / 16, SEGW = min(WPC, 62u), LPS = SEGW + 2, CPW = 64 / LPS, S = (WPC + SEGW - 1) / SEGW;
+  const uint32_t sub = lane / LPS, li = lane - sub * LPS;
+  const uint32_t nev = min(*A.nev, A.evcap);
+  const uint64_t nwaves = (uint64_t)gridDim.x * (kBlock / 64);
+  for (uint64_t base = ((uint64_t)blockIdx.x * (kBlock / 64) + (threadIdx.x >> 6)) * CPW; base < nev; base += nwaves * CPW) {
+    const uint64_t i = base + sub;
+    const bool unit = sub < CPW && i < nev;
+    const uint32_t e = unit ? A.evlist[i] : 0u;
+    const bool runu = unit && (A.ev[e] & kEvRunU) != 0;
+    uint32_t acc = 0;
+    for (uint32_t s = 0; s < S; s++) {
+      const int32_t wi = (int32_t)(s * SEGW + li) - 2;
+      const bool in = runu && wi < (int32_t)WPC;
+      uint4 v = make_uint4(0, 0, 0, 0);
+      if (in) v = *(const uint4*)(A.data + ((int64_t)e * C + (int64_t)wi * 16));
+      const uint32_t d[4] = {v.x, v.y, v.z, v.w};
+      uint32_t pre[16], suf[16];
+#pragma unroll
+      for (int o = 0; o < 16; o++) pre[o] = suf[o] = s_bits[(d[o >> 2] >> (8 * (o & 3))) & 0xFFu];
+#pragma unroll
+      for (int o = 1; o < 16; o++) pre[o] &= pre[o - 1];
+#pragma unroll
+      for (int o = 14; o >= 0; o--) suf[o] &= suf[o + 1];
+      const uint32_t before = __shfl_up(pre[15], 1);
+      uint32_t h = pre[15];
+#pragma unroll
+      for (int o = 0; o < 15; o++) h |= pre[o] & __shfl_up(suf[o + 1], 2);
+      if (li >= 2 && in) acc |= h & before;
+    }
+    for (uint32_t dd = 1; dd < 64; dd <<= 1) {
+      const uint32_t t = __shfl_down(acc, dd);
+      if (li + dd < LPS) acc |= t;
+    }
+    if (runu && li == 0) A.ev_ref[e] = acc;
+  }
+}
+
+static inline size_t item_lds_host(uint32_t G, uint32_t GW) { return 256 * (size_t)GW + 8 * (size_t)G + 4 * (size_t)((G + 1) & ~1u); }
 constexpr uint32_t kItemKwgLdsMax = 16 * 1024;
 struct ItemLds {
   const unsigned long long* gofbit;
   const uint32_t* gback;
   const uint32_t* gevents;
+  const uint32_t* gref;
   const unsigned long long* kwg;
 };
-__device__ __forceinline__ uint32_t item_lds_bytes(const ItemArgs& A) { return 256 * A.GW + 8 * A.G + A.kwg_lds; }
+__device__ __forceinline__ uint32_t item_lds_bytes(const ItemArgs& A) {
+  return 256 * A.GW + 8 * A.G + 4 * ((A.G + 1) & ~1u) + A.kwg_lds;
+}
 __device__ __forceinline__ ItemLds item_lds_load(const ItemArgs& A, uint8_t* smem) {
   unsigned long long* gofbit = (unsigned long long*)smem;
   uint32_t* gback = (uint32_t*)(gofbit + 32 * A.GW);
   uint32_t* gevents = gback + A.G;
+  uint32_t* gref = gevents + A.G;
   for (uint32_t i = threadIdx.x; i < 32 * A.GW; i += blockDim.x) gofbit[i] = A.gofbit[i];
   for (uint32_t i = threadIdx.x; i < A.G; i += blockDim.x) {
     gback[i] = A.gback[i];
-    gevents[i] = A.gevents[i];
+    const uint32_t ge = A.gevents[i], gr = A.gref && (ge & kEvRunU) ? A.gref[i] : 0u;
+    gevents[i] = gr ? ge & ~kEvRunU : ge;
+    gref[i] = gr;
   }
   const unsigned long long* kwg = A.kwg;
   if (A.kwg_lds) {
-    unsigned long long* k = (unsigned long long*)(gevents + A.G);
+    unsigned long long* k = (unsigned long long*)(gref + ((A.G + 1) & ~1u));
     for (uint32_t i = threadIdx.x; i < A.kwg_lds / 8; i += blockDim.x) k[i] = A.kwg[i];
     kwg = k;
   }
-  return ItemLds{gofbit, gback, gevents, kwg};
+  return ItemLds{gofbit, gback, gevents, gref, kwg};
 }
 
 __device__ __forceinline__ unsigned long long file_gate(const ItemArgs& A, const ItemLds& T, uint32_t f, uint32_t w) {
@@ -1547,13 +1609,15 @@
   const uint32_t C = A.chunk;
   if (t < nev) {
     const uint64_t e = ev_t;
+    const uint32_t er_raw = A.ev_ref ? A.ev_ref[e] : 0u;
     const uint32_t evb = A.ev[e] & ~kEvAlways;
+    const uint32_t er = (evb & kEvRunU) ? er_raw : 0u;
     const uint64_t ce = (e + 1) * C;
-    uint32_t pw[kMaxBack];
+    uint32_t pw[kMaxBack], pr[kMaxBack];
     if (e >= (uint64_t)kMaxBack) {
       const uint64_t b0 = (e - kMaxBack) & ~3ull;
       const uint32_t sh = (uint32_t)(e - kMaxBack - b0);
-      uint32_t x[20];
+      uint32_t x[20], y[20];
 #pragma unroll
       for (int j = 0; j < 5; j++) {
         const uint4 q = *(const uint4*)(A.ev + b0 + 4 * j);
@@ -1563,14 +1627,28 @@
         x[4 * j + 3] = q.w;
       }
 #pragma unroll
+      for (int j = 0; j < 5; j++) {
+        const uint4 q = A.ev_ref ? *(const uint4*)(A.ev_ref + b0 + 4 * j) : make_uint4(0, 0, 0, 0);
+        y[4 * j] = q.x;
+        y[4 * j + 1] = q.y;
+        y[4 * j + 2] = q.z;
+        y[4 * j + 3] = q.w;
+      }
+#pragma unroll
       for (int i = 0; i < kMaxBack; i++) {
         const int k = kMaxBack - 1 - i;
         pw[i] = sh == 0 ? x[k] : sh == 1 ? x[k + 1] : sh == 2 ? x[k + 2] : x[k + 3];
+        pr[i] = sh == 0 ? y[k] : sh == 1 ? y[k + 1] : sh == 2 ? y[k + 2] : y[k + 3];
       }
     } else {
 #pragma unroll
-      for (int i = 0; i < kMaxBack; i++) pw[i] = e > (uint64_t)i ? A.ev[e - 1 - i] : 0u;
-    }
+      for (int i = 0; i < kMaxBack; i++) {
+        pw[i] = e > (uint64_t)i ? A.ev[e - 1 - i] : 0u;
+        pr[i] = e > (uint64_t)i && A.ev_ref ? A.ev_ref[e - 1 - i] : 0u;
+      }
+    }
+#pragma unroll
+    for (int i = 0; i < kMaxBack; i++) pr[i] = (pw[i] & kEvRunU) ? pr[i] : 0u;
     for (uint32_t f = file_of(A.cf, A.off, A.F, e * C); f < A.F && A.off[f] < ce; f++) {
       const uint64_t fs = A.off[f], fe = A.off[f + 1];
       if (fe == fs) continue;
@@ -1582,12 +1660,13 @@
         while (cand) {
           const uint32_t g = w * 64 + __builtin_ctzll(cand);
           cand &= cand - 1;
-          const uint32_t back = T.gback[g], gev = T.gevents[g];
+          const uint32_t back = T.gback[g], gev = T.gevents[g], gr = T.gref[g];
+          if (!((evb & gev) | (er & gr))) continue;
           const uint64_t lo0 = e > fc0 + back ? e - back : fc0;
           const uint32_t lim = (uint32_t)(e - lo0);
           uint32_t m = 0;
 #pragma unroll
-          for (int i = 0; i < kMaxBack; i++) m |= ((pw[i] & gev) != 0 && (uint32_t)i < lim ? 1u : 0u) << i;
+          for (int i = 0; i < kMaxBack; i++) m |= (((pw[i] & gev) | (pr[i] & gr)) != 0 && (uint32_t)i < lim ? 1u : 0u) << i;
           visit(f, g, m ? e - __builtin_ctz(m) : lo0, e);
         }
       }
@@ -2701,6 +2780,9 @@
   uint32_t* d_gevents = nullptr;
   uint32_t* d_gback = nullptr;
   unsigned long long* d_gofbit = nullptr;
+  uint32_t* d_gref = nullptr;
+  uint32_t* d_refbits = nullptr;
+  uint32_t nref = 0;
   std::vector<uint32_t> gback;
   uint32_t GW = 1, maxback = 0, max_lds = 0;
   ~DeviceRules() {
@@ -2718,6 +2800,8 @@
   const uint64_t* off = nullptr;
   DevBuf<uint32_t> cf;
   DevBuf<uint32_t> ev_bits;
+  DevBuf<uint32_t> ev_ref;
+  bool refined = false;
   DevBuf<uint2> xlist;
   DevBuf<uint32_t> xcount;
   DevBuf<uint32_t> evlist;
@@ -3060,6 +3144,14 @@
   if ((rc = upload_vec(r->gback, &r->d_gback, &r->tables))) return rc;
   if ((rc = upload_vec(gofbit, &r->d_gofbit, &r->tables))) return rc;
   {
+    std::vector<uint32_t> gref, refbits(p.ref_bits, p.ref_bits + 256);
+    for (uint32_t g = 0; g < G; g++) gref.push_back(p.groups[g].gref);
+    if (!p.ref_cls.empty() && (uint32_t)p.run_k[0] != kRefineRun) return fail(TSG_ERR_INTERNAL, "run classes for another run length");
+    r->nref = (uint32_t)p.ref_cls.size();
+    if ((rc = upload_vec(gref, &r->d_gref, &r->tables))) return rc;
+    if ((rc = upload_vec(refbits, &r->d_refbits, &r->tables))) return rc;
+  }
+  {
     const uint32_t nkw = (uint32_t)p.kw_words * 32;
     std::vector<unsigned long long> kwg((size_t)nkw * r->GW, 0), galw(r->GW, 0);
     for (uint32_t g = 0; g < G; g++) {
@@ -3207,6 +3299,7 @@
   bool work;
   uint32_t kwg_bytes;
   int64_t grid_cap;
+  bool refine;
 };
 
 static int batch_shape(const DeviceRules* r, const ScanInput& in, const HostOut* out, BatchShape* s) {
@@ -3243,6 +3336,7 @@
   s->work = s->F && s->G && s->nchunks;
   s->kwg_bytes = (uint32_t)(32ull * s->W * r->GW * 8);
   s->grid_cap = knobs().grid_cap.load();
+  s->refine = s->work && total && r->nref && knobs().run_refine.load() != 0;
   return TSG_OK;
 }
 
@@ -3265,6 +3359,8 @@
   }
   if ((rc = l->cf.ensure((size_t)s.ncf))) return rc;
   if ((rc = l->ev_bits.ensure((size_t)s.nchunks_pad + 4))) return rc;
+  if (s.refine && (rc = l->ev_ref.ensure((size_t)s.nchunks_pad + 4))) return rc;
+  l->refined = s.refine;
   if (r->has_k1x && (rc = l->xlist.ensure((size_t)(total / 256 + 65536)))) return rc;
   if (r->has_k1x && (rc = l->xcount.ensure((size_t)std::max(r->cus, 1)))) return rc;
   if ((rc = l->evlist.ensure((size_t)s.nchunks_pad))) return rc;
@@ -3400,6 +3496,8 @@
   IA.off = l->off;
   IA.cf = l->cf;
   IA.ev = l->ev_bits;
+  IA.ev_ref = s.refine ? l->ev_ref.p : nullptr;
+  IA.gref = s.refine ? r->d_gref : nullptr;
   IA.ggate = l->ggate;
   IA.gofbit = r->d_gofbit;
   IA.gevents = r->d_gevents;
@@ -3430,6 +3528,12 @@
     GateArgs GA{l->ev_bits, s.nchunks, l->evlist, l->counts + kCntEvChunks, cgrid, l->kw, s.F, s.W, r->GW, r->d_kwg, r->d_galw, l->ggate,
                 (unsigned long long*)(l->counts + kCntClk), s.kwg_bytes <= kKwgLdsMax ? s.kwg_bytes : 0u};
     gates_kernel<<<cgrid + (s.F + kBlock - 1) / kBlock, kBlock, GA.kwg_lds, st>>>(GA);
+    HIP_TRY(hipGetLastError());
+  }
+  if (s.refine) {
+    RefineArgs RA{data, l->ev_bits, l->evlist, l->counts + kCntEvChunks, IA.evcap, s.C, r->d_refbits, l->ev_ref};
+    const uint64_t blocks = (s.nchunks + kBlock / 64 - 1) / (kBlock / 64);
+    refine_kernel<<<capped_grid(std::max<uint64_t>(1, std::min<uint64_t>(blocks, (uint64_t)r->grid)), s.grid_cap), kBlock, 0, st>>>(RA);
     HIP_TRY(hipGetLastError());
   }
   if (s.work) {
@@ -3594,6 +3698,19 @@
   return TSG_OK;
 }
 
+int lane_run_refine(LaneState* l, uint32_t* ref, size_t n) {
+  if (int rc = lane_sync(l)) return rc;
+  const size_t m = (size_t)std::min<uint64_t>(n, l->nchunks);
+  std::fill(ref, ref + n, 0u);
+  if (!m || !l->refined) return TSG_OK;
+  std::vector<uint32_t> ev(m);
+  HIP_TRY(hipMemcpy(ev.data(), l->ev_bits, sizeof(uint32_t) * m, hipMemcpyDeviceToHost));
+  HIP_TRY(hipMemcpy(ref, l->ev_ref, sizeof(uint32_t) * m, hipMemcpyDeviceToHost));
+  for (size_t c = 0; c < m; c++)
+    if (!(ev[c] & kEvRunU)) ref[c] = 0;
+  return TSG_OK;
+}
+
 int lane_events(LaneState* l, uint32_t* ev, size_t n) {
   if (int rc = lane_sync(l)) return rc;
   if (n && l->nchunks)
diff --git a/trivy_amd/csrc/knobs.cpp b/trivy_amd/csrc/knobs.cpp
--- a/trivy_amd/csrc/knobs.cpp
+++ b/trivy_amd/csrc/knobs.cpp
@@ -42,6 +42,7 @@
     if (x < 0) return fail(TSG_ERR_ARG, "grid_cap must be >= 0");
     k.grid_cap = x;
   }
+  else if (!strcmp(name, "run_refine")) k.run_refine = v.empty() ? 1 : x;
   else if (!strcmp(name, "device_poison")) k.device_poison = x;
   else if (!strcmp(name, "k2_no_word_recs")) k.k2_no_word_recs = x;
   else if (!strcmp(name, "k2_items_cap")) {
diff --git a/trivy_amd/csrc/pipeline.cpp b/trivy_amd/csrc/pipeline.cpp
--- a/trivy_amd/csrc/pipeline.cpp
+++ b/trivy_amd/csrc/pipeline.cpp
@@ -1353,6 +1353,17 @@
     if (items) std::memcpy(items, li.items.data(), 8 * std::min<size_t>(items_cap, li.items.size() / 2));
     if (gskip) std::memcpy(gskip, li.gskip.data(), std::min(gskip_len, li.gskip.size()));
     return TSG_OK;
+  });
+}
+
+int tsg_batch_run_refine(tsg_ctx* c, uint32_t slot_id, uint32_t* ref, size_t ref_len) {
+  if (!c || (!ref && ref_len)) return fail(TSG_ERR_ARG, "bad argument");
+  return guard([&]() -> int {
+    std::lock_guard<std::mutex> g(c->m);
+    if (c->emulate) return fail(TSG_ERR_ARG, "an emulated context has no device side array");
+    if (!c->kernels_lane || c->kernels_slot != slot_id || c->kernels_seq != c->seq)
+      return fail(TSG_ERR_ARG, "tsg_batch_run_refine follows tsg_batch_kernels on the same slot");
+    return lane_run_refine(c->kernels_lane, ref, ref_len);
   });
 }
 
diff --git a/trivy_amd/csrc/plan.cpp b/trivy_amd/csrc/plan.cpp
--- a/trivy_amd/csrc/plan.cpp
+++ b/trivy_amd/csrc/plan.cpp
@@ -98,7 +98,31 @@
   int first_atom = 0;
   int64_t evdist = 0;
   std::string desc = "none";
+  uint64_t cls[2] = {0, 0};
 };
+
+std::string class_text(const uint64_t* set) {
+  std::string s = "[";
+  auto put = [&](int c) {
+    char buf[8];
+    if (c > 32 && c < 127 && c != '\\' && c != ']' && c != '-') s.push_back((char)c);
+    else if (c == '-' || c == '\\' || c == ']') s += std::string("\\") + (char)c;
+    else snprintf(buf, sizeof buf, "\\x%02x", c), s += buf;
+  };
+  for (int c = 0; c < 128;) {
+    if (!((set[c >> 6] >> (c & 63)) & 1)) {
+      c++;
+      continue;
+    }
+    int e = c;
+    while (e + 1 < 128 && ((set[(e + 1) >> 6] >> ((e + 1) & 63)) & 1)) e++;
+    put(c);
+    if (e > c + 1) s.push_back('-');
+    if (e > c) put(e);
+    c = e + 1;
+  }
+  return s + "]";
+}
 
 Anchor choose_anchor(const Regexp& re, const Plan& p, bool literal_first) {
   const std::vector<AtomInfo> at = re.Atoms();
@@ -163,7 +187,16 @@
       int j = i;
       int64_t run = 0;
       while (j < n && at[j].ascii_only && in_set(at[j].set, p.run_cls, bit)) run += at[j++].min_bytes;
-      if (run >= k) return take(bit == 0 ? kEvRunU : kEvRunD, i, k, "", bit == 0 ? "run U" : "run D");
+      if (run >= k) {
+        Anchor a = take(bit == 0 ? kEvRunU : kEvRunD, i, k, "", bit == 0 ? "run U" : "run D");
+        int64_t need = k;
+        for (int t = i; bit == 0 && t < j && need > 0; t++) {
+          a.cls[0] |= at[t].set[0];
+          a.cls[1] |= at[t].set[1];
+          need -= at[t].min_bytes;
+        }
+        return a;
+      }
       i = j;
     }
   }
@@ -325,6 +358,40 @@
     p->rule_anchor[r] = anchor[r].desc;
   }, 1);
 
+  p->rule_cls.assign(R, {0, 0});
+  p->rule_cls_id.assign(R, -1);
+  for (size_t r = 0; r < R; r++) {
+    if (!single[r] || p->rule_event[r] != kEvRunU || p->run_k[0] != 32) continue;
+    std::array<uint64_t, 2> c = {anchor[r].cls[0], anchor[r].cls[1]};
+    bool usable = (c[0] | c[1]) != 0;
+    for (int b = 0; b < 128 && usable; b++)
+      if (((c[b >> 6] >> (b & 63)) & 1) && !(p->run_cls[b] & 1)) usable = false;
+    if (!usable) {
+      c = {0, 0};
+      for (int b = 0; b < 128; b++)
+        if (p->run_cls[b] & 1) c[b >> 6] |= 1ull << (b & 63);
+    }
+    size_t id = std::find(p->ref_cls.begin(), p->ref_cls.end(), c) - p->ref_cls.begin();
+    if (id == p->ref_cls.size()) {
+      if (id < (size_t)kRefClasses) {
+        p->ref_cls.push_back(c);
+      } else {
+        id = kRefClasses - 1;
+        p->ref_cls[id][0] |= c[0];
+        p->ref_cls[id][1] |= c[1];
+      }
+    }
+    p->rule_cls_id[r] = (int)id;
+  }
+  for (size_t r = 0; r < R; r++) {
+    if (p->rule_cls_id[r] < 0) continue;
+    p->rule_cls[r] = p->ref_cls[p->rule_cls_id[r]];
+    p->rule_anchor[r] += " class " + std::to_string(p->rule_cls_id[r]) + " " + class_text(p->rule_cls[r].data());
+  }
+  for (size_t j = 0; j < p->ref_cls.size(); j++)
+    for (int b = 0; b < 128; b++)
+      if ((p->ref_cls[j][b >> 6] >> (b & 63)) & 1) p->ref_bits[b] |= 1u << j;
+
   const bool tprof = getenv("TSG_PROF") != nullptr;
   auto tnow = [] { return std::chrono::steady_clock::now(); };
   auto tms = [](std::chrono::steady_clock::time_point a) {
@@ -356,6 +423,7 @@
       for (uint32_t r : cur) {
         p->rule_group[r] = (int)p->groups.size();
         g.evdist = std::max(g.evdist, p->rule_evdist[r]);
+        if (p->rule_cls_id[r] >= 0) g.gref |= 1u << p->rule_cls_id[r];
       }
       p->groups.push_back(std::move(g));
       cur.clear();
@@ -1399,10 +1467,15 @@
                    const std::vector<uint32_t>& ev, uint32_t max_back,
                    const std::function<void(uint32_t g, uint32_t f, uint64_t c)>& visit) {
   const uint32_t F = bv.nfiles;
+  std::vector<uint32_t> ref;
+  const bool refine = knobs().run_refine.load() != 0 && !plan.ref_cls.empty();
+  if (refine) refined_events(plan, bv, chunk, ev, &ref);
   for (size_t gi = 0; gi < plan.groups.size(); gi++) {
     const GroupPlan& g = plan.groups[gi];
     const uint32_t back = group_back(g, chunk);
     const bool every = (g.events & kEvAlways) != 0 || back > max_back;
+    const bool own = refine && (g.events & kEvRunU) && g.gref;
+    const uint32_t gev = own ? g.events & ~kEvRunU : g.events, gref = own ? g.gref : 0u;
     for (uint32_t f = 0; f < F; f++) {
       const uint64_t fs = bv.offsets[f], fe = bv.offsets[f + 1];
       if (fe == fs) continue;
@@ -1413,10 +1486,33 @@
       const uint64_t c0 = fs / chunk, c1 = (fe - 1) / chunk;
       for (uint64_t c = c0; c <= c1; c++) {
         bool need = every;
-        for (uint64_t q = c; q <= std::min<uint64_t>(c + back, c1) && !need; q++) need = (ev[q] & g.events) != 0;
+        for (uint64_t q = c; q <= std::min<uint64_t>(c + back, c1) && !need; q++)
+          need = (ev[q] & gev) != 0 || (gref && (ref[q] & gref) != 0);
         if (need) visit((uint32_t)gi, f, c);
       }
     }
+  }
+}
+
+void refined_events(const Plan& plan, const BatchView& bv, uint32_t chunk, const std::vector<uint32_t>& ev,
+                    std::vector<uint32_t>* ref) {
+  const uint64_t total = bv.offsets[bv.nfiles];
+  const uint32_t k = (uint32_t)plan.run_k[0], nc = (uint32_t)plan.ref_cls.size();
+  ref->assign(ev.size(), 0);
+  std::vector<uint32_t> run(nc);
+  for (uint64_t c = 0; c < ev.size(); c++) {
+    if (!(ev[c] & kEvRunU)) continue;
+    const uint64_t c0 = c * chunk, lo = c0 >= k - 1 ? c0 - (k - 1) : 0, hi = std::min<uint64_t>(total, c0 + chunk);
+    std::fill(run.begin(), run.end(), 0);
+    uint32_t bits = 0;
+    for (uint64_t p = lo; p < hi; p++) {
+      const uint32_t in = plan.ref_bits[bv.data[p]];
+      for (uint32_t j = 0; j < nc; j++) {
+        run[j] = ((in >> j) & 1) ? run[j] + 1 : 0;
+        if (run[j] >= k && p >= c0) bits |= 1u << j;
+      }
+    }
+    (*ref)[c] = bits;
   }
 }
 
diff --git a/trivy_amd/csrc/plan.hpp b/trivy_amd/csrc/plan.hpp
--- a/trivy_amd/csrc/plan.hpp
+++ b/trivy_amd/csrc/plan.hpp
@@ -1,4 +1,5 @@
 #pragma once
+#include <array>
 #include <cstdint>
 #include <functional>
 #include <memory>
@@ -17,6 +18,7 @@
 constexpr int kEvLit0 = 2;
 constexpr int kEvLitBits = 29;
 constexpr uint32_t kEvAlways = 1u << 31;
+constexpr int kRefClasses = 32;
 
 struct GroupPlan {
   std::unique_ptr<DFA> dfa;
@@ -24,6 +26,7 @@
   std::vector<uint32_t> kwmask;
   bool always = false;
   uint32_t events = kEvAlways;
+  uint32_t gref = 0;
   int64_t evdist = 0;
 };
 
@@ -49,6 +52,10 @@
   std::vector<int64_t> rule_evdist;
   std::vector<int> rule_first_atom;
   std::vector<std::string> rule_anchor;
+  std::vector<std::array<uint64_t, 2>> rule_cls;
+  std::vector<int> rule_cls_id;
+  std::vector<std::array<uint64_t, 2>> ref_cls;
+  uint32_t ref_bits[256] = {0};
   std::vector<uint8_t> rule_kw_mode;
   std::vector<std::vector<uint32_t>> rule_kws;
   std::vector<GroupPlan> groups;
@@ -182,6 +189,9 @@
                    const std::vector<uint32_t>& ev, uint32_t max_back,
                    const std::function<void(uint32_t g, uint32_t f, uint64_t c)>& visit);
 
+void refined_events(const Plan& plan, const BatchView& b, uint32_t chunk, const std::vector<uint32_t>& ev,
+                    std::vector<uint32_t>* ref);
+
 void k1_reference(const Plan& plan, const BatchView& b, uint32_t chunk,
                   std::vector<uint32_t>* kw, std::vector<uint32_t>* ev);
 void k1x_reference(const Plan& plan, const BatchView& b, uint32_t chunk,
diff --git a/trivy_amd/secret.py b/trivy_amd/secret.py
--- a/trivy_amd/secret.py
+++ b/trivy_amd/secret.py
@@ -345,6 +345,20 @@
                                                  C.byref(rev)))
         return {"first_atom": fa.value, "rule_atoms": at.value, "rule_winback": wb.value,
                 "rule_rev": bool(rev.value)}
+
+    def rule_class(self, rule):
+        cls, cid, gm = (C.c_uint64 * 2)(), C.c_int32(), C.c_uint32()
+        N.check(N.lib().tsg_ruleset_rule_class(self.handle, rule, cls, C.byref(cid), C.byref(gm)))
+        bits = int(cls[0]) | int(cls[1]) << 64
+        return {"cls": frozenset(c for c in range(128) if (bits >> c) & 1), "id": cid.value,
+                "group_mask": gm.value}
+
+    def run_refine_reference(self, batch, chunk):
+        ref = np.zeros(max((int(batch.offsets[-1]) + chunk - 1) // chunk, 1), dtype=np.uint32)
+        N.check(N.lib().tsg_emulate_run_refine(
+            self.handle, C.c_void_p(batch.data.ctypes.data), batch.offsets.ctypes.data_as(C.POINTER(C.c_uint64)),
+            batch.nfiles, chunk, ref.ctypes.data_as(C.POINTER(C.c_uint32)), ref.size))
+        return ref[:(int(batch.offsets[-1]) + chunk - 1) // chunk]
 
     def k1_literals(self):
         out = []
@@ -557,6 +571,13 @@
         assert list(m) == list(n)
         return ent[:n[0]], dent[:n[1]], items[:n[2]], gskip[:G]
 
+    def batch_run_refine(self):
+        sid, b = self._upload
+        n = (int(b.offsets[-1]) + self.chunk - 1) // self.chunk
+        ref = np.zeros(max(n, 1), dtype=np.uint32)
+        N.check(N.lib().tsg_batch_run_refine(self._h, sid, ref.ctypes.data_as(C.POINTER(C.c_uint32)), n))
+        return ref[:n]
+
     def batch_candidates(self):
         sid, b = self._upload
         W = (self.scanner.info()["n_keywords"] + 31) // 32
```

Result: no change. 56.67 (-0.1%).
